# hzxie/GaussianCity

Hardware: AMD Instinct MI355X
Metric: rendered frames/sec (fwd) @ 5000000 Gaussians, 1920x1080 (higher is better)
Workload: dtype f32; 1 GPU; C3: s_city 5000000 Gaussians, 1920x1080, SH degree 3, forward, 24-pose orbit; exp=gcr-fp32-v2 (bit-exact vs oracle), tile_sort=lists beyond 1024 entries sorted lazily, as far as the blend walks (default), cull=stateless: every frame reads means, scales, rotations (default)

## Files before the change

### gaussiancity_amd/csrc/gcr_api.hip

```cpp
#include <atomic>
#include <chrono>
#include <condition_variable>
#include <cstdio>
#include <cstring>
#include <deque>
#include <map>
#include <mutex>
#include <string>
#include <thread>

#include <pthread.h>

#include "gcr_internal.h"
#define GC_ERR_HIP GCR_ERR_DEVICE
#include "gc_host.h"

namespace {

std::atomic<int> g_timing{0};
std::atomic<int> g_force_radix{0};
std::atomic<int> g_force_global_cursor{0};
std::atomic<int> g_lazy_sort{1};
std::atomic<int> g_sort_in_blend{0};
std::atomic<int> g_split_preprocess{0};
std::atomic<int> g_deterministic{0};
std::atomic<int> g_bwd_wave_units{0};
std::atomic<int> g_rescue_hold{0};
std::atomic<int> g_gate_polls{400000};
std::atomic<int> g_band_sort_min{GCR_BAND_SORT_MIN_DEFAULT};
std::atomic<int> g_bwd_piece{160};
std::atomic<int> g_stream_policy{-1};
std::atomic<int> g_sync_culls{0};
struct SyncCullGuard {
  const int others;
  SyncCullGuard() : others(g_sync_culls.fetch_add(1)) {}
  ~SyncCullGuard() { g_sync_culls.fetch_sub(1); }
  SyncCullGuard(const SyncCullGuard&) = delete;
  SyncCullGuard& operator=(const SyncCullGuard&) = delete;
};
#ifdef GCR_EXPERIMENTS
std::atomic<int> g_k7_skip_flush{0};
std::atomic<int> g_k6_debug{0};
std::atomic<unsigned long long*> g_clock_buf{nullptr};
#endif

struct Opts {
  int lazy_sort, sort_in_blend, bwd_piece, deterministic, split_preprocess, force_radix, force_global_cursor, bwd_wave_units;
  int band_sort_min;
  int stream_policy;
};

int opt_raw(int v) { return v; }
int opt_bool(int v) { return v != 0; }
int opt_piece(int v) { return v < GCR_PIECE_MIN ? GCR_PIECE_MIN : (v > GCR_PIECE_MAX ? GCR_PIECE_MAX : v); }
struct OptionRow {
  const char* name;
  std::atomic<int>* global;
  int (*normalize)(int);
  int Opts::*resolved;
  int32_t gcr_options::*per_call;
};
const OptionRow g_options[] = {
    {"timing", &g_timing, opt_raw, nullptr, nullptr},
    {"force_radix", &g_force_radix, opt_raw, &Opts::force_radix, &gcr_options::force_radix},
    {"force_global_cursor", &g_force_global_cursor, opt_raw, &Opts::force_global_cursor, &gcr_options::force_global_cursor},
    {"split_preprocess", &g_split_preprocess, opt_raw, &Opts::split_preprocess, &gcr_options::split_preprocess},
    {"sort_in_blend", &g_sort_in_blend, opt_raw, &Opts::sort_in_blend, &gcr_options::sort_in_blend},
    {"lazy_sort", &g_lazy_sort, opt_bool, &Opts::lazy_sort, &gcr_options::lazy_sort},
    {"deterministic_backward", &g_deterministic, opt_bool, &Opts::deterministic, &gcr_options::deterministic_backward},
    {"bwd_wave_units", &g_bwd_wave_units, opt_bool, &Opts::bwd_wave_units, &gcr_options::bwd_wave_units},
    {"bwd_piece", &g_bwd_piece, opt_piece, &Opts::bwd_piece, &gcr_options::bwd_piece},
    {"band_sort_min", &g_band_sort_min, [](int v) { return v < 0 ? -1 : v; }, &Opts::band_sort_min, nullptr},
    {"stream_policy", &g_stream_policy, [](int v) { return v < 0 ? -1 : (v != 0); }, &Opts::stream_policy, nullptr},
    {"rescue_hold", &g_rescue_hold, opt_bool, nullptr, nullptr},
    {"gate_polls", &g_gate_polls, [](int v) { return v < 1 ? 1 : v; }, nullptr, nullptr},
#ifdef GCR_EXPERIMENTS
    {"k7_skip_flush", &g_k7_skip_flush, opt_raw, nullptr, nullptr},
    {"k6_debug", &g_k6_debug, opt_raw, nullptr, nullptr},
#endif
};
const OptionRow* find_option(const char* name) {
  if (name)
    for (const OptionRow& o : g_options)
      if (!strcmp(name, o.name)) return &o;
  return nullptr;
}
Opts resolve_options(const gcr_options* o) {
  Opts r{};
  for (const OptionRow& row : g_options) {
    if (!row.resolved) continue;
    int v = row.global->load();
    if (o != nullptr && row.per_call != nullptr && o->*row.per_call >= 0)
      v = row.normalize == opt_piece ? opt_piece(o->*row.per_call) : opt_bool(o->*row.per_call);
    r.*row.resolved = v;
  }
  return r;
}

enum Stage { ST_PRE = 0, ST_SCAN, ST_EMIT, ST_SORT, ST_RANGES, ST_BLEND_FWD, ST_BLEND_BWD, ST_PRE_BWD, ST_COUNT };

int check_num_rendered(unsigned long long R) {
  if (R == GCR_PREFILTER_MARK)
    return fail(GCR_ERR_INVALID_ARGUMENT, "Point is filtered although prefiltered is set. This shouldn't happen!");
  if (R > 0x7fffffffull)
    return fail(GCR_ERR_OVERFLOW, "num_rendered exceeds 2^31-1 (32-bit instance index, as in the reference)");
  return 0;
}

inline size_t align_up(size_t v, size_t a = 256) { return (v + a - 1) / a * a; }

inline void gcr_cpu_relax() {
#if defined(__x86_64__) || defined(__i386__)
  __builtin_ia32_pause();
#elif defined(__aarch64__)
  __asm__ __volatile__("yield");
#endif
}

constexpr int64_t GCR_SORT_IN_BLEND_MAX = 384;

thread_local StageSlot g_slots[ST_COUNT];
StageSlot* stage_slot(int stage) { return g_timing.load() ? &g_slots[stage] : nullptr; }

int debug_sync(const gcr_camera* cam, hipStream_t s, const char* where) {
  if (cam->debug) {
    hipError_t e = hipStreamSynchronize(s);
    if (e != hipSuccess) return fail_hip(e, where);
  }
  return 0;
}

gcr_layout compute_layout(int32_t P, int32_t W, int32_t H, int64_t R) {
  gcr_layout L;
  const size_t p = (size_t)(P > 0 ? P : 0);
  const size_t nblk = (p + 255) / 256;
  size_t o = 0;
  L.geom_rec = o;            o = align_up(o + p * sizeof(float4) * GCR_REC_QUADS);
  L.geom_cov3D = o;          o = align_up(o + p * GCR_COV3D_FLOATS * sizeof(float));
  L.geom_clamped = o;        o = align_up(o + p);
  L.geom_tiles_touched = o;  o = align_up(o + p * sizeof(uint32_t));
  L.geom_block_sums = o;     o = align_up(o + (nblk + 1) * sizeof(uint32_t));
  L.geom_vis_list = o;       o = align_up(o + p * sizeof(uint32_t));
  L.geom_vis_count = o;      o = align_up(o + (nblk + 1) * sizeof(uint32_t));
  L.geom_num_rendered = o;   o = align_up(o + 16 * sizeof(uint64_t));
  L.geom_block_tiles = o;    o = align_up(o + GCR_K1_MAX_BLOCKS * sizeof(uint64_t));
  L.geom_vis_rec = o;        o = align_up(o + p * sizeof(uint4));
  L.geom_total = o;

  const size_t npix = (size_t)(W > 0 ? W : 0) * (size_t)(H > 0 ? H : 0);
  const size_t gx = (size_t)(W + GCR_BLOCK_X - 1) / GCR_BLOCK_X, gy = (size_t)(H + GCR_BLOCK_Y - 1) / GCR_BLOCK_Y;
  const size_t T = gx * gy;
  o = 0;
  L.img_final_T = o;    o = align_up(o + npix * sizeof(float));
  L.img_n_contrib = o;  o = align_up(o + npix * sizeof(uint32_t));
  L.img_ranges = o;       o = align_up(o + T * 2 * sizeof(uint32_t));
  L.img_tile_cursor = o;  o = align_up(o + T * GCR_CURSOR_STRIDE * sizeof(uint32_t));
  {
    int G = 1;
    const int ng = gcr_tile_table_groups((int)T, GCR_K1_MAX_BLOCKS, &G);
    L.img_tile_table = o;   o = align_up(o + (size_t)ng * T * sizeof(uint32_t));
  }
  L.img_tile_lazy = o;    o = align_up(o + T * 4 * sizeof(uint32_t));
  L.img_total = o;

  const size_t r = (size_t)(R > 0 ? R : 0);
  const int end_bit = 32 + (int)gcr_higher_msb((uint32_t)T);
  L.bin_sorted = (size_t)(gcr_sort_passes(end_bit) & 1);
  o = 0;
  L.bin_vals[L.bin_sorted] = o;      o = align_up(o + r * sizeof(uint32_t));
  L.bin_vals[1 - L.bin_sorted] = o;  o = align_up(o + r * sizeof(uint32_t));
  L.bin_keys[0] = o;  o = align_up(o + r * sizeof(uint64_t));
  L.bin_keys[1] = o;  o = align_up(o + r * sizeof(uint64_t));
  L.bin_hist = o;     o = align_up(o + gcr_sort_hist_bytes((int64_t)r, end_bit));
  const size_t slots = r ? (size_t)gcr_piece_slots(r, T, GCR_PIECE_MIN) : 0;
  L.bin_lean_total = o;
  L.bin_work = o;       o = align_up(o + slots * 16);
  L.bin_mask = o;       o = align_up(o + r * sizeof(uint16_t));
  L.bin_ckpt = o;       o = align_up(o + slots * (size_t)GCR_CKPT_BYTES);
  L.bin_staged = o;     o = align_up(o + r * 48);
  L.bin_total = o;
  return L;
}

int check_inputs(const gcr_camera* cam, const gcr_gaussians* g, bool need_opacity = true) {
  if (!cam || !g) return fail(GCR_ERR_INVALID_ARGUMENT, "null camera/gaussians record");
  if (g->P < 0) return fail(GCR_ERR_INVALID_ARGUMENT, "P must be >= 0");
  if (g->P > 700000000)
    return fail(GCR_ERR_INVALID_ARGUMENT, "P above 700 000 000 is not supported");
  if (cam->img_w <= 0 || cam->img_h <= 0) return fail(GCR_ERR_INVALID_ARGUMENT, "image size must be positive");
  if (cam->img_w > 16 * 65535 || cam->img_h > 16 * 65535)
    return fail(GCR_ERR_INVALID_ARGUMENT, "image too large for 16-bit tile coordinates");
  if (!cam->bg || !cam->view_matrix || !cam->proj_matrix || !cam->campos)
    return fail(GCR_ERR_INVALID_ARGUMENT, "bg/view_matrix/proj_matrix/campos must be non-null");
  if (cam->out_u8 != 0 && cam->backward == 1)
    return fail(GCR_ERR_INVALID_ARGUMENT, "out_u8 (uint8 video frames) is for inference frames: gcr_camera.backward must be 0");
  if (cam->win_w != 0 || cam->win_h != 0) {
    if (cam->win_w <= 0 || cam->win_h <= 0 || cam->win_x < 0 || cam->win_y < 0 || cam->win_x + cam->win_w > cam->img_w ||
        cam->win_y + cam->win_h > cam->img_h)
      return fail(GCR_ERR_INVALID_ARGUMENT, "the output window must lie inside the image");
  }
  if (g->P == 0) return 0;
  if (!g->means3D) return fail(GCR_ERR_INVALID_ARGUMENT, "means3D must have dimensions (num_points, 3)");
  if (need_opacity && !g->opacities) return fail(GCR_ERR_INVALID_ARGUMENT, "opacities must be non-null");
  if ((g->shs == nullptr) == (g->colors_precomp == nullptr))
    return fail(GCR_ERR_INVALID_ARGUMENT, "provide exactly one of SHs or precomputed colors");
  const bool has_sr = g->scales != nullptr && g->rotations != nullptr;
  if (has_sr == (g->cov3D_precomp != nullptr) || ((g->scales != nullptr) != (g->rotations != nullptr)))
    return fail(GCR_ERR_INVALID_ARGUMENT,
                "provide exactly one of scale/rotation pair or precomputed 3D covariance");
  if (g->cull_cache && ((uintptr_t)g->cull_cache & 127u))
    return fail(GCR_ERR_INVALID_ARGUMENT, "cull_cache must be 128-byte aligned (gcr_cull_cache_bytes(P) bytes filled by gcr_build_cull_cache)");
  if (g->shs) {
    if (cam->sh_degree < 0 || cam->sh_degree > 3) return fail(GCR_ERR_INVALID_ARGUMENT, "sh_degree must be 0..3");
    if (g->M < (cam->sh_degree + 1) * (cam->sh_degree + 1))
      return fail(GCR_ERR_INVALID_ARGUMENT, "sh has fewer coefficients than sh_degree needs");
  }
  return 0;
}

void fill_cam(GcrCamVals& c, const gcr_camera* cam) {
  memset(&c, 0, sizeof(c));
  if (!cam->host_camera) return;
  c.by_value = 1;
  memcpy(c.view, cam->view_matrix, sizeof(c.view));
  memcpy(c.proj, cam->proj_matrix, sizeof(c.proj));
  memcpy(c.campos, cam->campos, sizeof(c.campos));
  memcpy(c.bg, cam->bg, sizeof(c.bg));
}
inline int stride_or(int32_t s, int dense) { return s > 0 ? (int)s : dense; }

struct FrameSetup {
  gcr_layout L;
  int64_t R_layout;
  int gx, gy, T;
  int nblocks, chunk;
  int NG, G;
  float4* rec;
  float* cov3D;
  uint32_t *tiles_touched, *block_sums, *vis_list, *vis_count;
  uint4 *vis_rec, *banded;
  unsigned long long *frame, *block_tiles;
  float* final_T;
  uint32_t *n_contrib, *ranges, *cursor, *table;
  uint4* lazy;
  char* bin;
  uint64_t* keys[2];
  uint32_t *vals[2], *list, *hist;
};
template <class T>
T* at(const void* base, size_t off) {
  return base ? (T*)((char*)base + off) : nullptr;
}
FrameSetup frame_setup(const Opts& op, int32_t P, const gcr_camera* cam, int64_t R_layout, const void* geom,
                       const void* img, const void* binning) {
  FrameSetup f;
  f.L = compute_layout(P, cam->img_w, cam->img_h, R_layout);
  const gcr_layout& L = f.L;
  f.R_layout = R_layout;
  f.gx = (cam->img_w + GCR_BLOCK_X - 1) / GCR_BLOCK_X;
  f.gy = (cam->img_h + GCR_BLOCK_Y - 1) / GCR_BLOCK_Y;
  f.T = f.gx * f.gy;
  gcr_preprocess_grid(P, gcr_preprocess_resident_blocks(), &f.nblocks, &f.chunk);
  f.G = 1;
  f.NG = op.force_global_cursor ? 0 : gcr_tile_table_groups(f.T, f.nblocks, &f.G);
  f.rec = at<float4>(geom, L.geom_rec);
  f.cov3D = at<float>(geom, L.geom_cov3D);
  f.tiles_touched = at<uint32_t>(geom, L.geom_tiles_touched);
  f.block_sums = at<uint32_t>(geom, L.geom_block_sums);
  f.vis_list = at<uint32_t>(geom, L.geom_vis_list);
  f.vis_count = at<uint32_t>(geom, L.geom_vis_count);
  f.vis_rec = at<uint4>(geom, L.geom_vis_rec);
  f.frame = at<unsigned long long>(geom, L.geom_num_rendered);
  f.block_tiles = at<unsigned long long>(geom, L.geom_block_tiles);
  f.banded = gcr_band_sort_possible(f.T) ? at<uint4>(geom, L.geom_tiles_touched) : nullptr;
  f.final_T = at<float>(img, L.img_final_T);
  f.n_contrib = at<uint32_t>(img, L.img_n_contrib);
  f.ranges = at<uint32_t>(img, L.img_ranges);
  f.cursor = at<uint32_t>(img, L.img_tile_cursor);
  f.table = at<uint32_t>(img, L.img_tile_table);
  f.lazy = at<uint4>(img, L.img_tile_lazy);
  f.bin = at<char>(binning, 0);
  for (int k = 0; k < 2; k++) {
    f.keys[k] = at<uint64_t>(binning, L.bin_keys[k]);
    f.vals[k] = at<uint32_t>(binning, L.bin_vals[k]);
  }
  f.list = f.vals[L.bin_sorted];
  f.hist = at<uint32_t>(binning, L.bin_hist);
  return f;
}

int check_buffers(const FrameSetup& f, const gcr_camera* cam, size_t geom_bytes, size_t img_bytes, const void* binning,
                  size_t binning_bytes, const char* binning_msg) {
  if (geom_bytes < f.L.geom_total) return fail(GCR_ERR_BUFFER_TOO_SMALL, "geometry buffer too small");
  if (img_bytes < f.L.img_total) return fail(GCR_ERR_BUFFER_TOO_SMALL, "image buffer too small");
  if (f.R_layout > 0 && (!binning || binning_bytes < (cam->backward == 1 ? f.L.bin_total : f.L.bin_lean_total)))
    return fail(GCR_ERR_BUFFER_TOO_SMALL, binning_msg);
  return 0;
}

template <class A>
void set_gaussian_args(A& a, const gcr_gaussians* g) {
  a.P = g->P;
  a.means3D = g->means3D; a.scales = g->scales; a.rotations = g->rotations;
  a.s_mean = stride_or(g->stride_means3D, 3);
  a.s_scale = stride_or(g->stride_scales, 3);
  a.s_rot = stride_or(g->stride_rotations, 4);
}
template <class A>
void set_camera_args(A& a, const gcr_camera* cam, const gcr_gaussians* g) {
  set_gaussian_args(a, g);
  a.D = cam->sh_degree; a.M = g->M; a.W = cam->img_w; a.H = cam->img_h;
  a.tanfovx = cam->tanfovx; a.tanfovy = cam->tanfovy;
  a.focal_y = cam->img_h / (2.0f * cam->tanfovy);
  a.focal_x = cam->img_w / (2.0f * cam->tanfovx);
  a.scale_modifier = cam->scale_modifier;
  a.shs = g->shs;
  a.view = cam->view_matrix; a.proj = cam->proj_matrix; a.campos = cam->campos;
  fill_cam(a.cam, cam);
}

GcrBlendArgs blend_args(const FrameSetup& f, const gcr_camera* cam, const uint32_t* list) {
  GcrBlendArgs b;
  memset(&b, 0, sizeof(b));
  b.ranges = f.ranges;
  b.list = list;
  b.rec = f.rec;
  b.W = cam->img_w; b.H = cam->img_h; b.gx = f.gx; b.gy = f.gy;
  b.bg = cam->bg;
  b.flip_x = cam->flip_x != 0; b.flip_y = cam->flip_y != 0;
  b.win_x = cam->win_x; b.win_y = cam->win_y; b.win_w = cam->win_w; b.win_h = cam->win_h;
  b.out_u8 = cam->out_u8 != 0 && cam->backward != 1;
  b.image_only = cam->backward == GCR_BACKWARD_IMAGE_ONLY;
  fill_cam(b.cam, cam);
  b.final_T = f.final_T;
  b.n_contrib = f.n_contrib;
  return b;
}

}

extern "C" {

#ifdef GCR_EXPERIMENTS
void gcr_debug_set_clock_buffer(void* dev_ptr) { g_clock_buf.store((unsigned long long*)dev_ptr); }
#endif

int gcr_abi_version(void) { return GCR_ABI_VERSION; }
int gcr_grad_record_floats(void) { return g_deterministic.load() ? GCR_GRAD_REC_FLOATS_DET : GCR_GRAD_REC_FLOATS; }
int gcr_grad_record_floats_opt(const gcr_options* options) {
  return resolve_options(options).deterministic ? GCR_GRAD_REC_FLOATS_DET : GCR_GRAD_REC_FLOATS;
}
const char* gcr_last_error(void) { return g_err.c_str(); }

size_t gcr_geometry_bytes(int32_t P) { return compute_layout(P, 16, 16, 0).geom_total; }
size_t gcr_image_bytes(int32_t W, int32_t H) { return compute_layout(0, W, H, 0).img_total; }
size_t gcr_binning_bytes(int64_t R, int32_t W, int32_t H) { return compute_layout(0, W, H, R).bin_total; }
size_t gcr_binning_bytes_lean(int64_t R, int32_t W, int32_t H) { return compute_layout(0, W, H, R).bin_lean_total; }
int gcr_get_layout(int32_t P, int32_t W, int32_t H, int64_t R, gcr_layout* out) {
  if (!out) return fail(GCR_ERR_INVALID_ARGUMENT, "null layout");
  *out = compute_layout(P, W, H, R);
  return 0;
}

int gcr_set_option(const char* name, int value) {
  const OptionRow* o = find_option(name);
  return o ? o->global->exchange(o->normalize(value)) : -1;
}

int gcr_get_option(const char* name) {
  const OptionRow* o = find_option(name);
  return o ? o->global->load() : INT32_MIN;
}

int gcr_get_stage_ms(float* ms_out, int capacity) { return stage_report(g_slots, ST_COUNT, ms_out, capacity); }

static inline bool band_sort_slot_free(const Opts& op) {
  return !op.split_preprocess && !op.force_radix && !op.force_global_cursor;
}

static int enqueue_preprocess(const Opts& op, const gcr_camera* cam, const gcr_gaussians* g, const FrameSetup& f,
                              int32_t* radii, unsigned long long cap_instances, unsigned long long cap_list, hipStream_t s,
                              unsigned long long* host_R = nullptr, unsigned int seq = 0, bool nt_stream = false) {
  GcrPreprocessArgs a;
  set_camera_args(a, cam, g);
  a.gx = f.gx; a.gy = f.gy;
  a.opacities = g->opacities; a.cov3D_precomp = g->cov3D_precomp; a.colors_precomp = g->colors_precomp;
  a.s_opac = stride_or(g->stride_opacities, 1);
  a.s_col = stride_or(g->stride_colors, 3);
  a.prefiltered = cam->prefiltered != 0;
  a.cull_cache = op.split_preprocess ? nullptr : reinterpret_cast<const float4*>(g->cull_cache);
  a.cull_shape = a.cull_cache ? reinterpret_cast<const float4*>((const char*)g->cull_cache + gcr_cull_cache_offset_b(g->P)) : nullptr;
  a.nt_stream = nt_stream ? 1 : 0;
  a.radii = radii;
  a.rec = f.rec;
  a.cov3D = f.cov3D;
  a.tile_count = f.cursor;
  a.vis_list = f.vis_list;
  a.vis_count = f.vis_count;
  a.vis_rec = f.vis_rec;
  a.cand_list = f.tiles_touched;
  a.cand_count = f.block_sums;
  a.nblocks = f.nblocks; a.chunk = f.chunk;
  a.block_tiles = f.block_tiles;
  const int T = f.T;
  if (f.NG > 0) a.tile_count = nullptr;
  {
    StageTimer t(s, stage_slot(ST_PRE));
    if (f.NG == 0)
      HIP_TRY(hipMemsetAsync(a.tile_count, 0, sizeof(uint32_t) * GCR_CURSOR_STRIDE * (size_t)T, s), "tile count memset");
    HIP_TRY(gcr_launch_preprocess(a, op.split_preprocess != 0, s), "preprocess");
  }
  if (int rc = debug_sync(cam, s, "preprocess")) return rc;
  StageTimer t(s, stage_slot(ST_SCAN));
  if (f.NG > 0) {
    const bool band = f.banded && band_sort_slot_free(op) && op.band_sort_min >= 0 &&
                      (op.band_sort_min == 0 || (cap_instances != ~0ull && cap_instances >= (unsigned long long)op.band_sort_min));
    HIP_TRY(gcr_launch_tile_count(T, f.gx, f.NG, f.G, f.nblocks, f.chunk, f.vis_rec, f.vis_count, f.table, f.cursor,
                                  f.cursor + (size_t)T, f.cursor + 2 * (size_t)T, f.frame, f.block_tiles, host_R, seq,
                                  band ? f.banded : nullptr, g->P / 4, s),
            "tile count");
  } else {
    HIP_TRY(gcr_launch_scan_tiles(f.cursor, GCR_CURSOR_STRIDE, f.ranges, T, f.frame, cap_instances, cap_list, host_R, seq,
                                  f.block_tiles, f.nblocks, s),
            "tile scan");
  }
  return 0;
}

static void set_piece_args(const Opts& op, GcrBlendArgs& b, bool want_state, const FrameSetup& f) {
  const gcr_layout& L = f.L;
  char* bb = want_state && f.R_layout > 0 ? f.bin : nullptr;
  b.piece = want_state ? op.bwd_piece : GCR_PIECE_MAX;
#ifdef GCR_EXPERIMENTS
  if (!want_state)
    if (const char* e = getenv("GCR_INFER_PIECE")) b.piece = atoi(e) < GCR_PIECE_MIN ? GCR_PIECE_MIN : (atoi(e) > GCR_PIECE_MAX ? GCR_PIECE_MAX : atoi(e));
#endif
  b.ckpt = bb ? (float4*)(bb + L.bin_ckpt) : nullptr;
  b.work = bb ? (uint4*)(bb + L.bin_work) : nullptr;
  b.mask_out = bb ? (uint16_t*)(bb + L.bin_mask) : nullptr;
  b.staged_out = bb ? (float4*)(bb + L.bin_staged) : nullptr;
  b.staged_off = L.bin_staged;
  b.ckpt_off = L.bin_ckpt;
  b.work_off = L.bin_work;
  b.mask_off = L.bin_mask;
  b.carve_bytes = L.bin_total;
  b.frame_out = f.frame;
#ifdef GCR_EXPERIMENTS
  if (const char* e = getenv("GCR_K6_NOEXTRAS")) {
    if (strchr(e, 'w')) { b.ckpt = nullptr; b.work = nullptr; }
    if (strchr(e, 'm')) { b.mask_out = nullptr; b.staged_out = nullptr; }
  }
#endif
}

static int enqueue_render_lds(const Opts& op, const gcr_camera* cam, const gcr_gaussians* g, const FrameSetup& f,
                              int64_t list_length_hint, bool speculative, unsigned long long cap_instances,
                              unsigned long long cap_list, float* out_color, hipStream_t s,
                              unsigned long long* host_longest = nullptr, unsigned long long* gate_words = nullptr,
                              unsigned int gate_seq = 0, bool nt_out = false) {
  const int64_t R_layout = f.R_layout;
  uint64_t* pairs = f.keys[0];
  const unsigned long long* frame_guard = speculative ? f.frame : nullptr;
  {
    StageTimer t(s, stage_slot(ST_EMIT));
    if (f.NG > 0) {
      HIP_TRY(gcr_launch_tile_scatter(f.T, f.gx, f.NG, f.G, f.nblocks, f.chunk, f.vis_rec, f.vis_count, f.table, f.cursor,
                                      f.cursor + (size_t)f.T, f.cursor + 2 * (size_t)f.T, f.ranges, pairs, f.frame,
                                      cap_instances, cap_list, host_longest, f.banded, g->P / 4, s),
              "tile scatter");
    } else if (R_layout > 0) {
      HIP_TRY(gcr_launch_scatter_instances(f.nblocks, f.chunk, f.vis_list, f.vis_count, f.rec, f.gx, f.cursor, pairs,
                                           f.ranges, f.T, frame_guard, s),
              "scatter instances");
    }
  }
  if (int rc = debug_sync(cam, s, "scatter instances")) return rc;
  const bool sort_in_blend = R_layout > 0 && list_length_hint <= GCR_SORT_IN_BLEND_MAX && op.sort_in_blend != 0;
  uint4* lazy = (R_layout > 0 && !sort_in_blend && op.lazy_sort != 0) ? f.lazy : nullptr;
  if (R_layout > 0 && !sort_in_blend) {
    StageTimer t(s, stage_slot(ST_SORT));
    HIP_TRY(gcr_launch_tile_sort(f.ranges, f.T, pairs, f.keys[1], f.list, list_length_hint + list_length_hint / 2 + 64,
                                 frame_guard, lazy, s),
            "tile sort");
  }
  if (int rc = debug_sync(cam, s, "tile sort")) return rc;
  GcrBlendArgs b = blend_args(f, cam, f.list);
  b.nt_out = nt_out && cam->backward != 1;
  b.out_color = out_color;
  b.frame = frame_guard;
  b.pairs = pairs;
  b.list_out = f.list;
  b.lazy = lazy;
  set_piece_args(op, b, cam->backward == 1, f);
  b.gate_words = gate_words;
  b.gate_seq = gate_seq;
  b.gate_polls = (unsigned int)g_gate_polls.load();
#ifdef GCR_EXPERIMENTS
  b.debug_flags = g_k6_debug.load();
  b.clock_buf = g_clock_buf.load();
#endif
#ifdef GCR_EXPERIMENTS
  static const bool chain = getenv("GCR_CHAIN_BLEND") != nullptr && atoi(getenv("GCR_CHAIN_BLEND")) != 0;
  static std::mutex chain_mu;
  static hipEvent_t chain_ev[64] = {};
  static unsigned chain_n = 0;
  if (chain) {
    std::lock_guard<std::mutex> lk(chain_mu);
    if (chain_n > 0) (void)hipStreamWaitEvent(s, chain_ev[(chain_n - 1) % 64], 0);
  }
#endif
  {
    StageTimer t(s, stage_slot(ST_BLEND_FWD));
    HIP_TRY(gcr_launch_blend_fwd(b, sort_in_blend, s), "blend forward");
  }
#ifdef GCR_EXPERIMENTS
  if (chain) {
    std::lock_guard<std::mutex> lk(chain_mu);
    hipEvent_t& e = chain_ev[chain_n % 64];
    if (!e) (void)hipEventCreateWithFlags(&e, hipEventDisableTiming);
    (void)hipEventRecord(e, s);
    chain_n++;
  }
#endif
  return debug_sync(cam, s, "blend forward");
}

static unsigned long long* host_words_alloc(size_t n) {
  unsigned long long* p = nullptr;
  if (n == 0 || hipHostMalloc((void**)&p, n * sizeof(unsigned long long),
                              hipHostMallocCoherent | hipHostMallocMapped | hipHostMallocPortable) != hipSuccess)
    return nullptr;
  for (size_t i = 0; i < n; i++) p[i] = 0ull;
  return p;
}
struct FrameReadback {
  unsigned long long* pinned = nullptr;
  unsigned int seq = 0;
  int ensure() {
    if (!pinned) {
      pinned = host_words_alloc(8);
      if (!pinned) return fail(GCR_ERR_DEVICE, "hipHostMalloc for the frame read-back failed");
    }
    return 0;
  }
};
thread_local FrameReadback g_readback;

static std::mutex g_words_mu;
static std::map<unsigned long long*, size_t> g_words_blocks;
static void rescue_forget_words(const unsigned long long* base, size_t n);

unsigned long long* gcr_host_words_alloc(size_t n_words) {
  unsigned long long* p = host_words_alloc(n_words);
  if (p) {
    std::lock_guard<std::mutex> lk(g_words_mu);
    g_words_blocks[p] = n_words;
  }
  return p;
}
void gcr_host_words_free(unsigned long long* words) {
  if (!words) return;
  size_t n = 0;
  {
    std::lock_guard<std::mutex> lk(g_words_mu);
    auto it = g_words_blocks.find(words);
    if (it != g_words_blocks.end()) {
      n = it->second;
      g_words_blocks.erase(it);
    }
  }
  if (n) rescue_forget_words(words, n);
  (void)hipHostFree(words);
}

int gcr_forward_preprocess(const gcr_camera* cam, const gcr_gaussians* g, void* geom,
                           size_t geom_bytes, void* img, size_t img_bytes, int32_t* radii,
                           gcr_frame_info* info_host, void* hip_stream) {
  if (int rc = check_inputs(cam, g)) return rc;
  if (!info_host) return fail(GCR_ERR_INVALID_ARGUMENT, "info_host is null");
  info_host->num_rendered = 0;
  info_host->max_tile_instances = 0;
  if (g->P == 0) return 0;
  if (!geom || !radii || !img) return fail(GCR_ERR_INVALID_ARGUMENT, "geom/img/radii must be non-null");
  const Opts op = resolve_options(cam->options);
  const FrameSetup f = frame_setup(op, g->P, cam, 0, geom, img, nullptr);
  if (int rc = check_buffers(f, cam, geom_bytes, img_bytes, nullptr, 0, nullptr)) return rc;
  hipStream_t s = (hipStream_t)hip_stream;
  const SyncCullGuard sync_cull;
  const bool nt = op.stream_policy > 0 || (op.stream_policy < 0 && sync_cull.others == 0);
  if (int rc = enqueue_preprocess(op, cam, g, f, radii, ~0ull, ~0ull, s, nullptr, 0, nt)) return rc;
  unsigned long long r[2] = {0, 0};
  HIP_TRY(hipMemcpyAsync(r, f.frame, sizeof(r), hipMemcpyDeviceToHost, s), "num_rendered copy");
  HIP_TRY(hipStreamSynchronize(s), "num_rendered sync");
  if (int rc = check_num_rendered(r[0])) return rc;
  info_host->num_rendered = (int64_t)r[0];
  info_host->max_tile_instances = (int64_t)r[1];
  return 0;
}

int gcr_forward(const gcr_camera* cam, const gcr_gaussians* g, void* geom, size_t geom_bytes, void* binning,
                size_t binning_bytes, int64_t binning_capacity, int64_t tile_list_capacity, void* img,
                size_t img_bytes, int32_t* radii, float* out_color, gcr_frame_info* info_host, void* hip_stream) {
  if (int rc = check_inputs(cam, g)) return rc;
  if (!info_host) return fail(GCR_ERR_INVALID_ARGUMENT, "info_host is null");
  info_host->num_rendered = 0;
  info_host->max_tile_instances = 0;
  if (g->P == 0) return 0;
  if (!out_color) return fail(GCR_ERR_INVALID_ARGUMENT, "out_color is null");
  if (binning_capacity < 0 || binning_capacity > 0x7fffffffll)
    return fail(GCR_ERR_INVALID_ARGUMENT, "binning_capacity out of range");
  if (!geom || !radii || !img) return fail(GCR_ERR_INVALID_ARGUMENT, "geom/img/radii must be non-null");
  const Opts op = resolve_options(cam->options);
  const FrameSetup f = frame_setup(op, g->P, cam, binning_capacity, geom, img, binning);
  if (int rc = check_buffers(f, cam, geom_bytes, img_bytes, binning, binning_bytes,
                               "binning buffer smaller than gcr_binning_bytes(binning_capacity)"))
    return rc;
  if (int rc = g_readback.ensure()) return rc;
  hipStream_t s = (hipStream_t)hip_stream;
  const bool speculate = binning_capacity > 0 && !op.force_radix && !cam->debug;
  const int64_t list_hint = tile_list_capacity > 0 ? tile_list_capacity : (int64_t)gcr_tile_sort_capacity();
  FrameReadback& rb = g_readback;
  const unsigned int seq = ++rb.seq ? rb.seq : ++rb.seq;
  const SyncCullGuard sync_cull;
  const bool nt = op.stream_policy > 0 || (op.stream_policy < 0 && sync_cull.others == 0);
  if (int rc = enqueue_preprocess(op, cam, g, f, radii, speculate ? (unsigned long long)binning_capacity : 0ull, ~0ull, s,
                                  rb.pinned, seq, nt))
    return rc;
  if (speculate) {
    if (int rc = enqueue_render_lds(op, cam, g, f, list_hint, true, (unsigned long long)binning_capacity, ~0ull, out_color,
                                    s, rb.pinned + 1, nullptr, 0, nt))
      return rc;
  }
  volatile unsigned long long* word = rb.pinned;
  unsigned long long v = *word;
  for (unsigned long spins = 0; (unsigned int)(v >> 32) != seq; v = *word) {
    gcr_cpu_relax();
    if ((++spins & 0xffffu) == 0) {
      const hipError_t q = hipStreamQuery(s);
      if (q != hipSuccess && q != hipErrorNotReady) return fail_hip(q, "frame info wait");
      if (q == hipSuccess && (unsigned int)(*word >> 32) != seq)
        return fail(GCR_ERR_DEVICE, "the stream finished without publishing num_rendered");
    }
  }
  const unsigned long long R = v & 0xffffffffull;
  const bool go = R <= (unsigned long long)binning_capacity;
  if (int rc = check_num_rendered(R)) return rc;
  info_host->num_rendered = (int64_t)R;
  if (speculate && go) {
    const unsigned long long seen = ((volatile unsigned long long*)rb.pinned)[1];
    info_host->max_tile_instances = seen ? (int64_t)seen : tile_list_capacity;
    return 0;
  }
  unsigned long long mx = 0;
  HIP_TRY(hipMemcpyAsync(&mx, f.frame + 1, sizeof(mx), hipMemcpyDeviceToHost, s), "longest list copy");
  HIP_TRY(hipStreamSynchronize(s), "longest list sync");
  info_host->max_tile_instances = (int64_t)mx;
  return 1;
}

struct AsyncFrame {
  unsigned long long* words;
  unsigned int seq;
  int device;
  gcr_camera cam;
  gcr_options opt;
  bool has_opt;
  float camvals[38];
  gcr_gaussians g;
  void* geom;
  size_t geom_bytes;
  void* img;
  size_t img_bytes;
  float* out_color;
  int64_t capacity;
  std::chrono::steady_clock::time_point born;
};

class RescueService {
  std::mutex mu_;
  std::condition_variable cv_;
  std::deque<AsyncFrame> frames_;
  bool started_ = false;
  hipStream_t streams_[64] = {};
  void* scratch_[64] = {};
  size_t scratch_bytes_[64] = {};
  std::atomic<long> rescued_{0};
  std::atomic<long> dropped_{0};
  const unsigned long long* rescuing_ = nullptr;
  std::condition_variable idle_cv_;

  static void publish(unsigned long long* w, int idx, unsigned int seq) {
    std::atomic_thread_fence(std::memory_order_seq_cst);
    ((volatile unsigned long long*)w)[idx] = (unsigned long long)seq;
    std::atomic_thread_fence(std::memory_order_seq_cst);
  }

  void rescue(AsyncFrame& f) {
    volatile unsigned long long* w = f.words;
    publish(f.words, 7, f.seq);
    if ((unsigned int)w[4] == f.seq) {
      publish(f.words, 5, f.seq);
      publish(f.words, 2, f.seq);
      dropped_.fetch_add(1);
      return;
    }
    const unsigned long long R = w[0] & 0xffffffffull;
    bool ok = false;
    void* stale = nullptr;
    do {
      if (check_num_rendered(R)) break;
      if (hipSetDevice(f.device) != hipSuccess) break;
      const int d = f.device & 63;
      if (!streams_[d]) {
        int lo = 0, hi = 0;
        if (hipDeviceGetStreamPriorityRange(&lo, &hi) != hipSuccess) lo = hi = 0;
        if (hipStreamCreateWithPriority(&streams_[d], hipStreamNonBlocking, hi) != hipSuccess &&
            hipStreamCreateWithFlags(&streams_[d], hipStreamNonBlocking) != hipSuccess)
          break;
      }
      hipStream_t s = streams_[d];
      gcr_camera cam = f.cam;
      if (cam.backward == 1) cam.backward = 0;
      cam.options = f.has_opt ? &f.opt : nullptr;
      if (cam.host_camera) {
        cam.view_matrix = f.camvals;
        cam.proj_matrix = f.camvals + 16;
        cam.campos = f.camvals + 32;
        cam.bg = f.camvals + 35;
      }
      const FrameSetup fs = frame_setup(resolve_options(cam.options), f.g.P, &cam, 0, f.geom, f.img, nullptr);
      gcr_frame_info info;
      info.num_rendered = (int64_t)R;
      unsigned long long longest = 0;
      if (hipMemcpyAsync(&longest, fs.frame + 1, 8, hipMemcpyDeviceToHost, s) != hipSuccess) break;
      if (hipStreamSynchronize(s) != hipSuccess) break;
      info.max_tile_instances = (int64_t)longest;
      const size_t bytes = gcr_binning_bytes_lean((int64_t)R, cam.img_w, cam.img_h);
      if (scratch_bytes_[d] < bytes) {
        stale = scratch_[d];
        scratch_[d] = nullptr;
        scratch_bytes_[d] = 0;
        if (hipMalloc(&scratch_[d], bytes + bytes / 2) != hipSuccess) {
          scratch_[d] = nullptr;
          break;
        }
        scratch_bytes_[d] = bytes + bytes / 2;
      }
      if (gcr_forward_render(&cam, &f.g, f.geom, f.geom_bytes, scratch_[d], scratch_bytes_[d], f.img, f.img_bytes, &info,
                             f.out_color, s) < 0)
        break;
      if (hipStreamSynchronize(s) != hipSuccess) break;
      ok = true;
    } while (false);
    if (!ok) publish(f.words, 5, f.seq);
    publish(f.words, 6, f.seq);
    publish(f.words, 2, f.seq);
    rescued_.fetch_add(1);
    if (stale) (void)hipFree(stale);
  }

  void run() {
    for (;;) {
      std::unique_lock<std::mutex> lk(mu_);
      cv_.wait(lk, [&] { return !frames_.empty(); });
      const auto now = std::chrono::steady_clock::now();
      const bool hold = g_rescue_hold.load() != 0;
      for (auto it = frames_.begin(); it != frames_.end();) {
        volatile unsigned long long* w = it->words;
        const unsigned long long v = w[0];
        if ((unsigned int)(v >> 32) == it->seq) {
          if ((v & 0xffffffffull) <= (unsigned long long)it->capacity) {
            it = frames_.erase(it);
            continue;
          }
          if ((unsigned int)w[4] == it->seq) {
            dropped_.fetch_add(1);
            it = frames_.erase(it);
            continue;
          }
          if (!hold && (unsigned int)w[3] == it->seq) {
            AsyncFrame f = *it;
            frames_.erase(it);
            rescuing_ = f.words;
            lk.unlock();
            rescue(f);
            lk.lock();
            rescuing_ = nullptr;
            idle_cv_.notify_all();
            break;
          }
        }
        if (now - it->born > std::chrono::seconds(120)) {
          it = frames_.erase(it);
          continue;
        }
        ++it;
      }
      lk.unlock();
      std::this_thread::sleep_for(std::chrono::microseconds(100));
    }
  }

 public:
  void add(const AsyncFrame& f) {
    std::lock_guard<std::mutex> lk(mu_);
    for (auto it = frames_.begin(); it != frames_.end();) it = it->words == f.words ? frames_.erase(it) : it + 1;
    const bool was_empty = frames_.empty();
    frames_.push_back(f);
    if (!started_) {
      started_ = true;
      std::thread([this] { run(); }).detach();
    }
    if (was_empty) cv_.notify_one();
  }
  void forget(const unsigned long long* base, size_t n) {
    std::unique_lock<std::mutex> lk(mu_);
    for (auto it = frames_.begin(); it != frames_.end();) it = (it->words >= base && it->words < base + n) ? frames_.erase(it) : it + 1;
    idle_cv_.wait(lk, [&] { return !(rescuing_ != nullptr && rescuing_ >= base && rescuing_ < base + n); });
  }
  void remove(const unsigned long long* words, unsigned int seq) {
    std::lock_guard<std::mutex> lk(mu_);
    for (auto it = frames_.begin(); it != frames_.end();) it = (it->words == words && it->seq == seq) ? frames_.erase(it) : it + 1;
  }
  long rescued() const { return rescued_.load(); }
  long dropped() const { return dropped_.load(); }
  void reset_after_fork() {
    new (&mu_) std::mutex();
    new (&cv_) std::condition_variable();
    new (&idle_cv_) std::condition_variable();
    rescuing_ = nullptr;
    new (&frames_) std::deque<AsyncFrame>();
    started_ = false;
    for (int i = 0; i < 64; i++) {
      streams_[i] = nullptr;
      scratch_[i] = nullptr;
      scratch_bytes_[i] = 0;
    }
  }
};
static RescueService& rescue_service() {
  static RescueService* r = [] {
    RescueService* p = new RescueService();
    (void)pthread_atfork(nullptr, nullptr, [] { rescue_service().reset_after_fork(); });
    return p;
  }();
  return *r;
}

static void rescue_forget_words(const unsigned long long* base, size_t n) { rescue_service().forget(base, n); }

long gcr_rescue_count(void) { return rescue_service().rescued(); }
long gcr_rescue_dropped_count(void) { return rescue_service().dropped(); }

int gcr_forward_async(const gcr_camera* cam, const gcr_gaussians* g, void* geom, size_t geom_bytes, void* binning,
                      size_t binning_bytes, int64_t binning_capacity, int64_t tile_list_capacity, void* img,
                      size_t img_bytes, int32_t* radii, float* out_color, unsigned long long* words_host, uint32_t seq,
                      void* hip_stream) {
  if (int rc = check_inputs(cam, g)) return rc;
  if (!words_host || seq == 0u) return fail(GCR_ERR_INVALID_ARGUMENT, "words_host must be non-null and seq non-zero");
  if (g->P == 0) {
    ((volatile unsigned long long*)words_host)[1] = 0ull;
    ((volatile unsigned long long*)words_host)[0] = (unsigned long long)seq << 32;
    return 0;
  }
  if (!out_color) return fail(GCR_ERR_INVALID_ARGUMENT, "out_color is null");
  const Opts op = resolve_options(cam->options);
  if (binning_capacity <= 0 || binning_capacity > 0x7fffffffll || op.force_radix || cam->debug)
    return fail(GCR_ERR_INVALID_ARGUMENT,
                "gcr_forward_async needs a capacity guess > 0 and neither force_radix nor debug: use gcr_forward");
  if (!geom || !radii || !img) return fail(GCR_ERR_INVALID_ARGUMENT, "geom/img/radii must be non-null");
  const FrameSetup fr = frame_setup(op, g->P, cam, binning_capacity, geom, img, binning);
  if (int rc = check_buffers(fr, cam, geom_bytes, img_bytes, binning, binning_bytes,
                               "binning buffer smaller than gcr_binning_bytes(binning_capacity)"))
    return rc;
  hipStream_t s = (hipStream_t)hip_stream;
  const int64_t list_hint = tile_list_capacity > 0 ? tile_list_capacity : (int64_t)gcr_tile_sort_capacity();
  if (int rc = enqueue_preprocess(op, cam, g, fr, radii, (unsigned long long)binning_capacity, ~0ull, s, words_host, seq,
                                  op.stream_policy > 0))
    return rc;
  AsyncFrame f;
  memset((void*)&f, 0, sizeof(f));
  f.words = words_host;
  f.seq = seq;
  if (hipGetDevice(&f.device) != hipSuccess) f.device = 0;
  f.cam = *cam;
  f.has_opt = cam->options != nullptr;
  if (f.has_opt) f.opt = *cam->options;
  f.cam.options = nullptr;
  if (cam->host_camera) {
    memcpy(f.camvals, cam->view_matrix, 16 * sizeof(float));
    memcpy(f.camvals + 16, cam->proj_matrix, 16 * sizeof(float));
    memcpy(f.camvals + 32, cam->campos, 3 * sizeof(float));
    memcpy(f.camvals + 35, cam->bg, 3 * sizeof(float));
  }
  f.g = *g;
  f.geom = geom;
  f.geom_bytes = geom_bytes;
  f.img = img;
  f.img_bytes = img_bytes;
  f.out_color = out_color;
  f.capacity = binning_capacity;
  f.born = std::chrono::steady_clock::now();
  rescue_service().add(f);
  const int rc = enqueue_render_lds(op, cam, g, fr, list_hint, true, (unsigned long long)binning_capacity, ~0ull, out_color, s,
                                    words_host + 1, words_host, seq, op.stream_policy > 0);
  if (rc < 0) rescue_service().remove(words_host, seq);
  return rc;
}

static int ticket_state(const unsigned long long* words_host, uint32_t seq, int64_t capacity, gcr_frame_info* info) {
  volatile const unsigned long long* w = words_host;
  const unsigned long long v = w[0];
  if ((unsigned int)(v >> 32) != seq) return 1;
  const unsigned long long R = v & 0xffffffffull;
  if (int rc = check_num_rendered(R)) return rc;
  if (R > (unsigned long long)capacity) {
    if ((unsigned int)w[5] == seq) return fail(GCR_ERR_DEVICE, "the overflow rescue of an asynchronous frame failed");
    if ((unsigned int)w[2] != seq) {
      if ((unsigned int)w[4] == seq && (unsigned int)w[7] != seq)
        return fail(GCR_ERR_DEVICE, "an asynchronous frame overflowed its binning buffer and was not rescued in time");
      return 1;
    }
  }
  if (info) {
    info->num_rendered = (int64_t)R;
    info->max_tile_instances = (int64_t)w[1];
  }
  return 0;
}

int gcr_ticket_poll(const unsigned long long* words_host, uint32_t seq, int64_t binning_capacity,
                    gcr_frame_info* info_host) {
  if (!words_host || seq == 0u) return fail(GCR_ERR_INVALID_ARGUMENT, "words_host must be non-null and seq non-zero");
  return ticket_state(words_host, seq, binning_capacity, info_host);
}

int gcr_ticket_wait(const unsigned long long* words_host, uint32_t seq, int64_t binning_capacity, void* hip_stream,
                    gcr_frame_info* info_host) {
  if (!words_host || seq == 0u) return fail(GCR_ERR_INVALID_ARGUMENT, "words_host must be non-null and seq non-zero");
  hipStream_t s = (hipStream_t)hip_stream;
  for (unsigned long spins = 0;; ) {
    const int st = ticket_state(words_host, seq, binning_capacity, info_host);
    if (st != 1) return st;
    gcr_cpu_relax();
    if ((++spins & 0xfffffu) == 0 && hip_stream != nullptr) {
      const hipError_t q = hipStreamQuery(s);
      if (q != hipSuccess && q != hipErrorNotReady) return fail_hip(q, "ticket wait");
      if (q == hipSuccess && ticket_state(words_host, seq, binning_capacity, info_host) == 1)
        return fail(GCR_ERR_DEVICE, "the stream finished without publishing num_rendered");
    }
  }
}

int gcr_forward_render(const gcr_camera* cam, const gcr_gaussians* g, void* geom, size_t geom_bytes,
                       void* binning, size_t binning_bytes, void* img, size_t img_bytes,
                       const gcr_frame_info* info, float* out_color, void* hip_stream) {
  if (int rc = check_inputs(cam, g, false)) return rc;
  if (g->P == 0) return 0;
  if (!geom || !img || !info) return fail(GCR_ERR_INVALID_ARGUMENT, "geom/img/info must be non-null");
  if (!out_color && cam->backward != 1)
    return fail(GCR_ERR_INVALID_ARGUMENT, "out_color may only be NULL for a state-only pass (gcr_camera.backward == 1)");
  const int64_t R = info->num_rendered;
  if (R < 0 || R > 0x7fffffffll) return fail(GCR_ERR_INVALID_ARGUMENT, "R out of range");
  if (R > 0 && !binning) return fail(GCR_ERR_INVALID_ARGUMENT, "binning buffer is null");
  const Opts op = resolve_options(cam->options);
  const FrameSetup f = frame_setup(op, g->P, cam, R, geom, img, binning);
  if (int rc = check_buffers(f, cam, geom_bytes, img_bytes, binning, binning_bytes, "binning buffer too small")) return rc;
  hipStream_t s = (hipStream_t)hip_stream;
  if (R == 0 || !op.force_radix)
    return enqueue_render_lds(op, cam, g, f, info->max_tile_instances, false, ~0ull, ~0ull, out_color, s, nullptr, nullptr, 0,
                              op.stream_policy > 0);

  int half = (int)f.L.bin_sorted;
  {
    StageTimer t(s, stage_slot(ST_EMIT));
    HIP_TRY(gcr_launch_tiles_touched(g->P, f.nblocks, f.chunk, f.vis_list, f.vis_count, f.rec, f.tiles_touched, f.block_sums, s),
            "tiles touched");
    HIP_TRY(gcr_launch_scan_block_sums(f.block_sums, (g->P + 255) / 256, (unsigned long long*)f.hist, s), "scan");
    HIP_TRY(gcr_launch_emit(g->P, f.tiles_touched, f.block_sums, f.rec, f.gx, f.keys[0], f.vals[0], s), "emit");
  }
  if (int rc = debug_sync(cam, s, "emit")) return rc;
  {
    StageTimer t(s, stage_slot(ST_SORT));
    const int end_bit = 32 + (int)gcr_higher_msb((uint32_t)f.T);
    HIP_TRY(gcr_launch_sort(f.keys[0], f.vals[0], f.keys[1], f.vals[1], R, end_bit, f.hist, &half, s), "sort");
  }
  if (int rc = debug_sync(cam, s, "sort")) return rc;
  {
    StageTimer t(s, stage_slot(ST_RANGES));
    HIP_TRY(gcr_launch_tile_ranges(f.keys[half], R, f.ranges, f.T, s), "tile ranges");
  }
  if (int rc = debug_sync(cam, s, "tile ranges")) return rc;
  GcrBlendArgs b = blend_args(f, cam, f.vals[half]);
  b.out_color = out_color;
  set_piece_args(op, b, cam->backward == 1, f);
  {
    StageTimer t(s, stage_slot(ST_BLEND_FWD));
    HIP_TRY(gcr_launch_blend_fwd(b, false, s), "blend forward");
  }
  return debug_sync(cam, s, "blend forward");
}

int gcr_backward(const gcr_camera* cam, const gcr_gaussians* g, const int32_t* radii, const void* geom,
                 size_t geom_bytes, const void* binning, size_t binning_bytes, const void* img,
                 size_t img_bytes, int64_t R, const float* dL_dpix, const gcr_grads* gr,
                 void* hip_stream) {
  if (int rc = check_inputs(cam, g, false)) return rc;
  if (g->P == 0) return 0;
  if (!gr || !dL_dpix || !radii || !geom || !img)
    return fail(GCR_ERR_INVALID_ARGUMENT, "grads/dL_dpix/radii/geom/img must be non-null");
  if (!gr->dL_dmeans2D || !gr->dL_dconic || !gr->dL_dopacity || !gr->dL_dcolors || !gr->dL_dmeans3D ||
      !gr->dL_dcov3D || (g->shs && !gr->dL_dsh) || (g->scales && (!gr->dL_dscales || !gr->dL_drotations)))
    return fail(GCR_ERR_INVALID_ARGUMENT, "a required gradient output is null");
  if ((uintptr_t)gr->dL_dconic & 63u)
    return fail(GCR_ERR_INVALID_ARGUMENT, "dL_dconic (the gradient records) must be 64-byte aligned");
  if (g->scales && stride_or(gr->stride_rotations, 4) == 4 && ((uintptr_t)gr->dL_drotations & 15u))
    return fail(GCR_ERR_INVALID_ARGUMENT, "dL_drotations must be 16-byte aligned");
  if (g->rotations && stride_or(g->stride_rotations, 4) == 4 && ((uintptr_t)g->rotations & 15u))
    return fail(GCR_ERR_INVALID_ARGUMENT, "rotations must be 16-byte aligned when dense");
  const bool any_grad_stride = gr->stride_means3D > 0 || gr->stride_opacity > 0 || gr->stride_colors > 0 ||
                               gr->stride_scales > 0 || gr->stride_rotations > 0;
  if (any_grad_stride && (!gr->packed || gr->packed_floats <= 0))
    return fail(GCR_ERR_INVALID_ARGUMENT, "strided gradient outputs need the block they live in (gcr_grads.packed)");
  if (R < 0 || R > 0x7fffffffll) return fail(GCR_ERR_INVALID_ARGUMENT, "R out of range");
  if (cam->backward != 1)
    return fail(GCR_ERR_INVALID_ARGUMENT,
                "gcr_backward needs a frame rendered with gcr_camera.backward == 1 (pass the same value here); for a frame "
                "rendered without it call gcr_forward_render(out_color = NULL, backward = 1) first");
  const Opts op = resolve_options(cam->options);
  const FrameSetup f = frame_setup(op, g->P, cam, R, geom, img, binning);
  if (int rc = check_buffers(f, cam, geom_bytes, img_bytes, binning, binning_bytes, "binning buffer too small")) return rc;
  hipStream_t s = (hipStream_t)hip_stream;

  const int det = op.deterministic;

  GcrFillArgs fill;
  memset(&fill, 0, sizeof(fill));
  {
    const unsigned long long P = (unsigned long long)g->P;
    auto seg = [&](float* p, unsigned long long n) {
      if (p != nullptr && n != 0) {
        fill.ptr[fill.nseg] = p;
        fill.n[fill.nseg++] = n;
      }
    };
    seg(gr->dL_dmeans2D, 3 * P);
    seg(gr->stride_colors > 0 ? nullptr : gr->dL_dcolors, (unsigned long long)GCR_NUM_CHANNELS * P);
    seg(gr->stride_opacity > 0 ? nullptr : gr->dL_dopacity, P);
    seg(gr->stride_means3D > 0 ? nullptr : gr->dL_dmeans3D, 3 * P);
    seg(gr->dL_dcov3D, 6 * P);
    seg(gr->dL_dsh, g->shs ? 3ull * (unsigned long long)g->M * P : 0ull);
    seg(gr->stride_scales > 0 ? nullptr : gr->dL_dscales, 3 * P);
    seg(gr->stride_rotations > 0 ? nullptr : gr->dL_drotations, 4 * P);
    if (any_grad_stride) seg(gr->packed, (unsigned long long)gr->packed_floats);
    unsigned long long total = 0;
    for (int i = 0; i < fill.nseg; i++) total += fill.n[i];
    const unsigned long long want = (total + 1023ull) / 1024ull;
    unsigned long long cap = 256ull;
#ifdef GCR_EXPERIMENTS
    if (const char* e = getenv("GCR_FILL_BLOCKS")) cap = (unsigned long long)atoi(e);
#endif
    fill.blocks = (int)(want < cap ? (want ? want : 1ull) : cap);
  }

  if (R > 0) {
    StageTimer t(s, stage_slot(ST_BLEND_BWD));
    HIP_TRY(gcr_launch_zero_grad_records(f.nblocks, f.chunk, f.vis_list, f.vis_count, (float4*)gr->dL_dconic,
                                         (det ? GCR_GRAD_REC_FLOATS_DET : GCR_GRAD_REC_FLOATS) / 4, s),
            "zero gradient records");
    GcrBlendArgs b = blend_args(f, cam, f.list);
    b.fill = fill;
    b.dL_dpix = dL_dpix;
    b.grad_rec = gr->dL_dconic;
    b.deterministic = det;
    b.binning_base = f.bin;
    b.frame_in = f.frame;
    b.R = (unsigned long long)R;
    b.piece = op.bwd_piece;
    b.binning_bytes = (unsigned long long)binning_bytes;
#ifdef GCR_EXPERIMENTS
    b.debug_flags = g_k7_skip_flush.load();
    b.clock_buf = g_clock_buf.load();
#endif
    HIP_TRY(gcr_launch_blend_bwd(b, op.bwd_wave_units != 0, s), "blend backward");
  } else {
    HIP_TRY(gcr_launch_fill(fill, s), "gradient zero fill");
  }
  if (int rc = debug_sync(cam, s, "blend backward")) return rc;

  GcrPreprocessBwdArgs a;
  set_camera_args(a, cam, g);
  a.cov3D = g->cov3D_precomp ? g->cov3D_precomp : f.cov3D;
  a.s_cov3d = g->cov3D_precomp ? 6 : GCR_COV3D_FLOATS;
  a.radii = radii;
  a.vis_list = f.vis_list;
  a.vis_count = f.vis_count;
  a.nblocks = f.nblocks; a.chunk = f.chunk;
  a.frame = R > 0 ? f.frame : nullptr;
  a.binning_bytes = (unsigned long long)binning_bytes;
  a.grad_rec = (const float4*)gr->dL_dconic;
  a.rec = f.rec;
  a.deterministic = det;
  a.dL_dmean2D = gr->dL_dmeans2D; a.dL_dcolor = gr->dL_dcolors; a.dL_dopacity = gr->dL_dopacity;
  a.dL_dmean3D = gr->dL_dmeans3D; a.dL_dcov3D = gr->dL_dcov3D; a.dL_dsh = gr->dL_dsh;
  a.dL_dscale = gr->dL_dscales; a.dL_drot = gr->dL_drotations;
  a.g_mean = stride_or(gr->stride_means3D, 3);
  a.g_opac = stride_or(gr->stride_opacity, 1);
  a.g_col = stride_or(gr->stride_colors, 3);
  a.g_scale = stride_or(gr->stride_scales, 3);
  a.g_rot = stride_or(gr->stride_rotations, 4);
  {
    StageTimer t(s, stage_slot(ST_PRE_BWD));
    HIP_TRY(gcr_launch_preprocess_bwd(a, s), "preprocess backward");
  }
  return debug_sync(cam, s, "preprocess backward");
}

size_t gcr_cull_cache_bytes(int32_t P) { return P > 0 ? gcr_cull_cache_offset_b(P) + (size_t)P * 32 : 0; }

int gcr_build_cull_cache(const gcr_gaussians* g, float scale_modifier, void* cull_cache_out, void* hip_stream) {
  if (!g) return fail(GCR_ERR_INVALID_ARGUMENT, "null gaussians record");
  if (g->P < 0 || g->P > 700000000) return fail(GCR_ERR_INVALID_ARGUMENT, "P must be 0 .. 700 000 000");
  if (g->P == 0) return 0;
  if (!g->means3D) return fail(GCR_ERR_INVALID_ARGUMENT, "means3D must have dimensions (num_points, 3)");
  if (!g->opacities) return fail(GCR_ERR_INVALID_ARGUMENT, "opacities must be non-null");
  const bool has_sr = g->scales != nullptr && g->rotations != nullptr;
  if (has_sr == (g->cov3D_precomp != nullptr) || ((g->scales != nullptr) != (g->rotations != nullptr)))
    return fail(GCR_ERR_INVALID_ARGUMENT, "provide exactly one of scale/rotation pair or precomputed 3D covariance");
  if (!cull_cache_out || ((uintptr_t)cull_cache_out & 127u))
    return fail(GCR_ERR_INVALID_ARGUMENT, "cull_cache_out must be a 128-byte aligned buffer of gcr_cull_cache_bytes(P) bytes");
  GcrPreprocessArgs a;
  memset(&a, 0, sizeof(a));
  set_gaussian_args(a, g);
  a.scale_modifier = scale_modifier;
  a.cov3D_precomp = g->cov3D_precomp;
  a.opacities = g->opacities;
  a.s_opac = stride_or(g->stride_opacities, 1);
  HIP_TRY(gcr_launch_build_cull_cache(a, reinterpret_cast<float4*>(cull_cache_out),
                                      reinterpret_cast<float4*>((char*)cull_cache_out + gcr_cull_cache_offset_b(g->P)),
                                      (hipStream_t)hip_stream),
          "build cull cache");
  return 0;
}

int gcr_mark_visible(int32_t P, const float* means3D, const float* view_matrix,
                     const float* proj_matrix, uint8_t* present, void* hip_stream) {
  (void)proj_matrix;
  if (P < 0) return fail(GCR_ERR_INVALID_ARGUMENT, "P must be >= 0");
  if (P == 0) return 0;
  if (!means3D || !view_matrix || !present) return fail(GCR_ERR_INVALID_ARGUMENT, "null pointer");
  HIP_TRY(gcr_launch_mark_visible(P, means3D, view_matrix, present, (hipStream_t)hip_stream), "mark_visible");
  return 0;
}

int64_t gcr_rasterize_forward(gcr_resize_fn geometry_buffer, void* geometry_user,
                              gcr_resize_fn binning_buffer, void* binning_user,
                              gcr_resize_fn image_buffer, void* image_user, const gcr_camera* cam,
                              const gcr_gaussians* g, float* out_color, int32_t* radii,
                              void* hip_stream) {
  if (int rc = check_inputs(cam, g)) return rc;
  if (!geometry_buffer || !binning_buffer || !image_buffer)
    return fail(GCR_ERR_INVALID_ARGUMENT, "resize callbacks must be non-null");
  if (g->P == 0) return 0;
  const size_t gbytes = gcr_geometry_bytes(g->P);
  void* geom = geometry_buffer(geometry_user, gbytes);
  if (!geom) return fail(GCR_ERR_ALLOC, "geometry resize callback returned null");
  const size_t ibytes = gcr_image_bytes(cam->img_w, cam->img_h);
  void* img = image_buffer(image_user, ibytes);
  if (!img) return fail(GCR_ERR_ALLOC, "image resize callback returned null");
  gcr_camera cam1 = *cam;
  cam1.backward = 1;
  gcr_frame_info info;
  if (int rc = gcr_forward_preprocess(&cam1, g, geom, gbytes, img, ibytes, radii, &info, hip_stream)) return rc;
  const size_t bbytes = gcr_binning_bytes(info.num_rendered, cam->img_w, cam->img_h);
  void* bin = binning_buffer(binning_user, bbytes);
  if (!bin && info.num_rendered > 0) return fail(GCR_ERR_ALLOC, "binning resize callback returned null");
  if (int rc = gcr_forward_render(&cam1, g, geom, gbytes, bin, bbytes, img, ibytes, &info, out_color, hip_stream))
    return rc;
  return info.num_rendered;
}

}
```

### gaussiancity_amd/csrc/gcr_binning.hip

```cpp
#include <stdlib.h>
#include "gcr_device.h"
#include "gcr_internal.h"
#include "gcr_sort.h"

namespace {

constexpr int SORT_THREADS = 256;
constexpr int SORT_ITEMS = 16;
constexpr int SORT_TILE = SORT_THREADS * SORT_ITEMS;
constexpr int RADIX_BITS = 8;
constexpr int RADIX = 1 << RADIX_BITS;

__global__ __launch_bounds__(256) void k_emit(int P, const uint32_t* __restrict__ tiles_touched,
                                              const uint32_t* __restrict__ block_offsets,
                                              const float4* __restrict__ rec, int gx,
                                              uint64_t* __restrict__ keys,
                                              uint32_t* __restrict__ vals) {
  __shared__ uint32_t lds4[4];
  const int idx = blockIdx.x * 256 + threadIdx.x;
  const uint32_t t = idx < P ? tiles_touched[idx] : 0u;
  uint32_t total;
  uint32_t off = gcr_block_excl_scan_256(t, lds4, &total);
  if (t == 0) return;
  off += block_offsets[blockIdx.x];
  const float4 q2 = rec[(size_t)idx * GCR_REC_QUADS + 2];
  const uint32_t dbits = __float_as_uint(q2.y);
  const uint32_t rx = __float_as_uint(q2.z), ry = __float_as_uint(q2.w);
  const uint32_t minx = rx & 0xffffu, maxx = rx >> 16, miny = ry & 0xffffu, maxy = ry >> 16;
  for (uint32_t y = miny; y < maxy; y++)
    for (uint32_t x = minx; x < maxx; x++) {
      const uint64_t key = ((uint64_t)(y * (uint32_t)gx + x) << 32) | dbits;
      keys[off] = key;
      vals[off] = (uint32_t)idx;
      off++;
    }
}

constexpr int RANK_MERGE_MAX = 1024;
constexpr int TT_MAX_TBLOCKS = 640;

template <int THREADS>
struct TtPrefix {
  static constexpr int PER = (GCR_K1_MAX_BLOCKS + THREADS) / THREADS;
  uint32_t vc[PER];
  GCR_DEV void load(const uint32_t* __restrict__ vis_count, int nblocks, int tid) {
#pragma unroll
    for (int u = 0; u < PER; u++) {
      const int bi = tid * PER + u;
      vc[u] = bi < nblocks ? vis_count[bi] : 0u;
    }
  }
  GCR_DEV void scan(uint32_t* pre, uint32_t* wtot, int nblocks, int tid) const {
    const int lane = tid & 63, w = tid >> 6;
    uint32_t mine = 0;
#pragma unroll
    for (int u = 0; u < PER; u++) mine += vc[u];
    const uint32_t incl = gcr_wave_incl_scan_u32(mine, lane);
    __syncthreads();
    if (lane == 63) wtot[w] = incl;
    __syncthreads();
    uint32_t run = incl - mine;
#pragma unroll
    for (int k = 0; k < THREADS / 64; k++)
      if (k < w) run += wtot[k];
#pragma unroll
    for (int u = 0; u < PER; u++) {
      const int bi = tid * PER + u;
      if (bi <= nblocks) pre[bi] = run;
      run += vc[u];
    }
    __syncthreads();
  }
};
GCR_DEV uint32_t tt_position(const uint32_t* pre, int nblocks, int chunk, uint32_t f) {
  int lo = 0, hi = nblocks;
  while (hi - lo > 1) {
    const int mid = (lo + hi) >> 1;
    if (pre[mid] <= f)
      lo = mid;
    else
      hi = mid;
  }
  return (uint32_t)lo * (uint32_t)chunk + (f - pre[lo]);
}
GCR_DEV uint4 tt_survivor(const uint32_t* pre, int nblocks, const uint4* __restrict__ vis_rec, int chunk, uint32_t f) {
  return vis_rec[tt_position(pre, nblocks, chunk, f)];
}

template <bool SCATTER, int TT_THREADS>
__global__ __launch_bounds__(TT_THREADS) void k_tile_table(int T, int gx, int G, int nblocks_k1, int chunk,
                                                           const uint4* __restrict__ vis_rec,
                                                           const uint32_t* __restrict__ vis_count,
                                                           uint32_t* __restrict__ table,
                                                           const uint32_t* __restrict__ tile_total,
                                                           const uint32_t* __restrict__ tile_local,
                                                           const uint32_t* __restrict__ blk_total,
                                                           uint32_t* __restrict__ ranges,
                                                           uint64_t* __restrict__ pairs,
                                                           unsigned long long* __restrict__ frame,
                                                           unsigned long long cap_instances,
                                                           unsigned long long cap_list,
                                                           unsigned long long* __restrict__ host_word,
                                                           unsigned int seq,
                                                           const unsigned long long* __restrict__ block_tiles,
                                                           const uint4* __restrict__ banded, int banded_capacity) {
  extern __shared__ __attribute__((aligned(16))) unsigned char gcr_smem[];
  uint32_t* cnt = reinterpret_cast<uint32_t*>(gcr_smem);
  __shared__ uint32_t pre[GCR_K1_MAX_BLOCKS + 1];
  __shared__ uint32_t blk_base[TT_MAX_TBLOCKS];
  __shared__ uint32_t wtot[TT_THREADS / 64];
  const int tid = threadIdx.x, lane = tid & 63, w = tid >> 6;
#ifdef GCR_EXPERIMENTS
  const uint32_t my_row = G < 0 ? blockIdx.x : gcr_tt_row(blockIdx.x, gridDim.x);
#else
  const uint32_t my_row = gcr_tt_row(blockIdx.x, gridDim.x);
#endif
  uint32_t* __restrict__ row = table + (size_t)my_row * T;
  TtPrefix<TT_THREADS> blocks;
  blocks.load(vis_count, nblocks_k1, tid);
  if (!SCATTER) {
    if (blockIdx.x == 0) {
      unsigned long long part = 0ull, pf = 0ull;
      for (int b = tid; b < nblocks_k1; b += TT_THREADS) {
        const unsigned long long v = block_tiles[b];
        part += v & ~GCR_PREFILTER_FLAG;
        pf |= v & GCR_PREFILTER_FLAG;
      }
#pragma unroll
      for (int o = 32; o > 0; o >>= 1) part += __shfl_xor(part, o, 64);
      __shared__ unsigned long long wpart[TT_THREADS / 64];
      if (lane == 0) wpart[w] = part;
      const int prefilter_violation = __syncthreads_or(pf != 0ull ? 1 : 0);
      if (tid == 0) {
        unsigned long long total = 0ull;
#pragma unroll
        for (int k = 0; k < TT_THREADS / 64; k++) total += wpart[k];
        if (prefilter_violation) total = GCR_PREFILTER_MARK;
        frame[0] = total;
        frame[1] = 0ull;
        frame[2] = 0ull;
        frame[GCR_FRAME_PIECE] = 0ull;
        frame[GCR_FRAME_BANDED] = banded != nullptr ? 1ull : 0ull;
        if (host_word != nullptr)
          gcr_store_to_host(host_word, ((unsigned long long)seq << 32) | (total > 0xffffffffull ? 0xffffffffull : total));
      }
    }
    for (int t = tid; t < T; t += TT_THREADS) cnt[t] = 0u;
  } else {
    const bool go = frame[0] <= cap_instances && frame[1] <= cap_list;
    if (blockIdx.x == 0 && tid == 0) {
      frame[2] = go ? 1ull : 0ull;
      if (host_word != nullptr) gcr_store_to_host(host_word, frame[1]);
    }
    if (!go) return;
    const int ntb = (T + 63) / 64;
    uint32_t running = 0;
    for (int b0 = 0; b0 < ntb; b0 += TT_THREADS) {
      const int bi = b0 + tid;
      const uint32_t v = bi < ntb ? blk_total[bi] : 0u;
      const uint32_t incl = gcr_wave_incl_scan_u32(v, lane);
      if (lane == 63) wtot[w] = incl;
      __syncthreads();
      uint32_t before = 0, all = 0;
#pragma unroll
      for (int k = 0; k < TT_THREADS / 64; k++) {
        const uint32_t x = wtot[k];
        if (k < w) before += x;
        all += x;
      }
      if (bi < ntb) blk_base[bi] = running + before + incl - v;
      running += all;
      __syncthreads();
    }
    const int slice = (T + (int)gridDim.x - 1) / (int)gridDim.x;
    const int t_lo = blockIdx.x * slice, t_hi = min(T, t_lo + slice);
    for (int t = tid; t < T; t += TT_THREADS) {
      const uint32_t start = blk_base[t >> 6] + tile_local[t];
      cnt[t] = start + row[t];
      if (t >= t_lo && t < t_hi) {
        ranges[2 * t] = start;
        ranges[2 * t + 1] = start + tile_total[t];
      }
    }
  }
  (void)G;
  blocks.scan(pre, wtot, nblocks_k1, tid);
  const uint32_t survivors = pre[nblocks_k1];
  const uint32_t f_lo = (uint32_t)(((uint64_t)survivors * blockIdx.x) / gridDim.x);
  const uint32_t f_hi = (uint32_t)(((uint64_t)survivors * (blockIdx.x + 1u)) / gridDim.x);
  const bool use_band = banded != nullptr && (SCATTER ? frame[GCR_FRAME_BANDED] != 0ull : true);
  const bool band_recs = survivors <= (uint32_t)banded_capacity;
  const uint32_t* __restrict__ banded_pos = reinterpret_cast<const uint32_t*>(banded);
  for (uint32_t f = f_lo + (uint32_t)tid; f < f_hi; f += TT_THREADS) {
    const uint4 sv = !use_band ? tt_survivor(pre, nblocks_k1, vis_rec, chunk, f)
                               : (band_recs ? banded[f] : vis_rec[banded_pos[f]]);
    const uint32_t rx = sv.z, ry = sv.w;
    const uint32_t minx = rx & 0xffffu, maxx = rx >> 16, miny = ry & 0xffffu, maxy = ry >> 16;
    const uint64_t key = ((uint64_t)sv.y << 32) | sv.x;
    for (uint32_t y = miny; y < maxy; y++)
      for (uint32_t x = minx; x < maxx; x++) {
        const uint32_t t = y * (uint32_t)gx + x;
        if (SCATTER) {
          const uint32_t pos = atomicAdd(&cnt[t], 1u);
          pairs[pos] = key;
        } else {
          atomicAdd(&cnt[t], 1u);
        }
      }
  }
  if (!SCATTER) {
    __syncthreads();
    for (int t = tid; t < T; t += TT_THREADS) row[t] = cnt[t];
  }
}

constexpr int GCR_BANDS = 256;
constexpr int BAND_CUTS = 128;
GCR_DEV uint32_t band_of(uint32_t rx, uint32_t ry, uint32_t gx, uint32_t band_mul) {
  const uint32_t t0 = (ry & 0xffffu) * gx + (rx & 0xffffu);
  const uint32_t b = (uint32_t)(((uint64_t)t0 * band_mul) >> 32);
  return b < (uint32_t)GCR_BANDS ? b : (uint32_t)GCR_BANDS - 1u;
}

constexpr int BAND_THREADS = 1024;
constexpr int BAND_ILP = 4;
template <bool PERMUTE>
__global__ __launch_bounds__(BAND_THREADS) void k_band(int gx, uint32_t band_mul, int nblocks_k1, int chunk,
                                                       const uint4* __restrict__ vis_rec,
                                                       const uint32_t* __restrict__ vis_count,
                                                       uint32_t* __restrict__ hist, uint4* __restrict__ banded,
                                                       int banded_capacity) {
  __shared__ uint32_t pre[GCR_K1_MAX_BLOCKS + 1];
  __shared__ uint32_t wtot[BAND_THREADS / 64];
  __shared__ uint32_t cur[GCR_BANDS];
  __shared__ uint32_t part[2][BAND_THREADS / GCR_BANDS][GCR_BANDS];
  const int tid = threadIdx.x, lane = tid & 63, w = tid >> 6;
  TtPrefix<BAND_THREADS> blocks;
  blocks.load(vis_count, nblocks_k1, tid);
  if (PERMUTE) {
    constexpr int Q = BAND_THREADS / GCR_BANDS, ROWS = BAND_CUTS / Q;
    const int b = tid & (GCR_BANDS - 1), q = tid / GCR_BANDS;
    uint32_t total = 0, before = 0;
#pragma unroll 16
    for (int r = 0; r < ROWS; r++) {
      const int g = q * ROWS + r;
      const uint32_t v = hist[(size_t)g * GCR_BANDS + b];
      total += v;
      before += g < (int)blockIdx.x ? v : 0u;
    }
    part[0][q][b] = total;
    part[1][q][b] = before;
    __syncthreads();
    if (tid < GCR_BANDS) {
      total = 0;
      before = 0;
#pragma unroll
      for (int k = 0; k < Q; k++) {
        total += part[0][k][tid];
        before += part[1][k][tid];
      }
      const uint32_t incl = gcr_wave_incl_scan_u32(total, lane);
      if (lane == 63) wtot[w] = incl;
      part[0][0][tid] = incl - total + before;
    }
    __syncthreads();
    if (tid < GCR_BANDS) {
      uint32_t start = part[0][0][tid];
#pragma unroll
      for (int k = 0; k < GCR_BANDS / 64; k++)
        if (k < w) start += wtot[k];
      cur[tid] = start;
    }
  } else {
    if (tid < GCR_BANDS) cur[tid] = 0u;
  }
  blocks.scan(pre, wtot, nblocks_k1, tid);
  const uint32_t survivors = pre[nblocks_k1];
  const uint32_t f_lo = (uint32_t)(((uint64_t)survivors * blockIdx.x) / gridDim.x);
  const uint32_t f_hi = (uint32_t)(((uint64_t)survivors * (blockIdx.x + 1u)) / gridDim.x);
  const bool band_recs = survivors <= (uint32_t)banded_capacity;
  uint32_t* __restrict__ banded_pos = reinterpret_cast<uint32_t*>(banded);
  for (uint32_t f0 = f_lo + (uint32_t)tid; f0 < f_hi; f0 += BAND_THREADS * BAND_ILP) {
    uint32_t pos[BAND_ILP];
    uint4 sv[BAND_ILP];
#pragma unroll
    for (int u = 0; u < BAND_ILP; u++) {
      const uint32_t f = f0 + (uint32_t)u * BAND_THREADS;
      pos[u] = f < f_hi ? tt_position(pre, nblocks_k1, chunk, f) : 0xffffffffu;
    }
#pragma unroll
    for (int u = 0; u < BAND_ILP; u++)
      if (pos[u] != 0xffffffffu) sv[u] = vis_rec[pos[u]];
#pragma unroll
    for (int u = 0; u < BAND_ILP; u++)
      if (pos[u] != 0xffffffffu) {
        const uint32_t b = band_of(sv[u].z, sv[u].w, (uint32_t)gx, band_mul);
        if (PERMUTE) {
          const uint32_t slot = atomicAdd(&cur[b], 1u);
          if (band_recs)
            banded[slot] = sv[u];
          else
            banded_pos[slot] = pos[u];
        } else {
          atomicAdd(&cur[b], 1u);
        }
      }
  }
  if (!PERMUTE) {
    __syncthreads();
    if (tid < GCR_BANDS) hist[(size_t)blockIdx.x * GCR_BANDS + tid] = cur[tid];
  }
}

__global__ __launch_bounds__(1024) void k_table_colscan(uint32_t* __restrict__ table, int NG, int T,
                                                        uint32_t* __restrict__ tile_total,
                                                        uint32_t* __restrict__ tile_local,
                                                        uint32_t* __restrict__ blk_total,
                                                        unsigned long long* __restrict__ frame) {
  __shared__ uint32_t part[16][64];
  const int lane = threadIdx.x & 63, grp = threadIdx.x >> 6;
  const int t = blockIdx.x * 64 + lane;
  const int rpg = (NG + 15) / 16;
  const int r0 = grp * rpg;
  uint32_t v[32];
  uint32_t sum = 0;
#pragma unroll
  for (int r = 0; r < 32; r++) {
    const int g = r0 + r;
    v[r] = (r < rpg && g < NG && t < T) ? table[(size_t)g * T + t] : 0u;
  }
#pragma unroll
  for (int r = 0; r < 32; r++) sum += v[r];
  part[grp][lane] = sum;
  __syncthreads();
  uint32_t before = 0, all = 0;
#pragma unroll
  for (int k = 0; k < 16; k++) {
    const uint32_t p = part[k][lane];
    if (k < grp) before += p;
    all += p;
  }
  if (t < T) {
    uint32_t run = before;
#pragma unroll
    for (int r = 0; r < 32; r++) {
      const int g = r0 + r;
      if (r < rpg && g < NG) {
        table[(size_t)g * T + t] = run;
        run += v[r];
      }
    }
  }
  if (grp == 0) {
    const uint32_t mine = t < T ? all : 0u;
    const uint32_t incl = gcr_wave_incl_scan_u32(mine, lane);
    const uint32_t mx = gcr_wave_max_u32(mine);
    if (t < T) {
      tile_total[t] = mine;
      tile_local[t] = incl - mine;
    }
    if (lane == 63) {
      blk_total[blockIdx.x] = incl;
      if (mx) atomicMax(&frame[1], (unsigned long long)mx);
    }
  }
}

__global__ __launch_bounds__(256) void k_scatter_instances(int chunk, const uint32_t* __restrict__ vis_list,
                                                           const uint32_t* __restrict__ vis_count,
                                                           const float4* __restrict__ rec, int gx,
                                                           uint32_t* __restrict__ cursor,
                                                           uint64_t* __restrict__ pairs,
                                                           const unsigned long long* __restrict__ frame) {
  if (frame != nullptr && frame[2] == 0ull) return;
  const uint32_t nvis = vis_count[blockIdx.x];
  const uint32_t* __restrict__ my_list = vis_list + (size_t)blockIdx.x * chunk;
  for (uint32_t it = threadIdx.x; it < nvis; it += 256) {
    const int idx = (int)my_list[it];
    const float4 q2 = rec[(size_t)idx * GCR_REC_QUADS + 2];
    const uint64_t key = ((uint64_t)__float_as_uint(q2.y) << 32) | (uint32_t)idx;
    const uint32_t rx = __float_as_uint(q2.z), ry = __float_as_uint(q2.w);
    const uint32_t minx = rx & 0xffffu, maxx = rx >> 16, miny = ry & 0xffffu, maxy = ry >> 16;
    const uint32_t w = maxx - minx, n = w * (maxy - miny);
    for (uint32_t k0 = 0; k0 < n; k0 += 8) {
      uint32_t pos[8];
#pragma unroll
      for (uint32_t u = 0; u < 8; u++) {
        const uint32_t k = k0 + u;
        if (k < n) {
          const uint32_t t = (miny + k / w) * (uint32_t)gx + minx + k % w;
          pos[u] = atomicAdd(&cursor[(size_t)t * GCR_CURSOR_STRIDE], 1u);
        }
      }
#pragma unroll
      for (uint32_t u = 0; u < 8; u++)
        if (k0 + u < n) pairs[pos[u]] = key;
    }
  }
}

__global__ __launch_bounds__(256) void k_tile_sort(const uint32_t* __restrict__ ranges,
                                                   uint64_t* __restrict__ pairs, uint64_t* __restrict__ pairs_spare,
                                                   uint32_t* __restrict__ list,
                                                   const unsigned long long* __restrict__ frame, int lds_capacity,
                                                   uint4* __restrict__ lazy) {
  extern __shared__ __attribute__((aligned(16))) unsigned char gcr_smem[];
  uint64_t* s = reinterpret_cast<uint64_t*>(gcr_smem);
  if (frame != nullptr && frame[2] == 0ull) return;
  const int tid = threadIdx.x;
  const uint32_t r0 = ranges[2 * blockIdx.x], r1 = ranges[2 * blockIdx.x + 1];
  const int n = (int)(r1 - r0);
  if (lazy != nullptr) {
    if (n > GCR_LAZY_MIN) {
      uint32_t n_sorted = 0;
      uint64_t L = 0;
      gcr_lazy_extend<GCR_LAZY_CAP_K4>(s, pairs + r0, (uint32_t)n, n_sorted, L, list + r0, tid);
      if (tid == 0) lazy[blockIdx.x] = make_uint4(n_sorted, 0u, (uint32_t)L, (uint32_t)(L >> 32));
      return;
    }
    if (tid == 0) lazy[blockIdx.x] = make_uint4((uint32_t)max(n, 0), 0u, ~0u, ~0u);
  }
  if (n <= 0) return;
  if (n > lds_capacity) {
    gcr_tile_sort_long(s, (uint32_t)lds_capacity, pairs + r0, pairs_spare + r0, list + r0, (uint32_t)n, tid);
    return;
  }
  if (n == 1) {
    if (tid == 0) list[r0] = (uint32_t)pairs[r0];
    return;
  }
  if (n <= RANK_MERGE_MAX) {
    const int nchunks = (n + 63) >> 6, npad = nchunks << 6;
    uint64_t* sb = s + npad;
    for (int i = tid; i < npad; i += 256) s[i] = i < n ? pairs[r0 + i] : ~0ull;
    __syncthreads();
    const ulonglong2* s2 = reinterpret_cast<const ulonglong2*>(s);
    uint64_t mine[RANK_MERGE_MAX / 256];
    uint32_t rank[RANK_MERGE_MAX / 256];
#pragma unroll
    for (int e = 0; e < RANK_MERGE_MAX / 256; e++) {
      const int i = tid + e * 256;
      if (i < npad) {
        const int c = i >> 6;
        const uint64_t key = s[i];
        uint32_t r = 0;
#pragma unroll 8
        for (int j = 0; j < 32; j++) {
          const ulonglong2 kk = s2[c * 32 + j];
          r += (kk.x < key ? 1u : 0u) + (kk.y < key ? 1u : 0u);
        }
        mine[e] = key;
        rank[e] = r;
        if (i < n) sb[c * 64 + r] = key;
      }
    }
    __syncthreads();
    const int last_real = n - (nchunks - 1) * 64;
#pragma unroll
    for (int e = 0; e < RANK_MERGE_MAX / 256; e++) {
      const int i = tid + e * 256;
      if (i < n) {
        const int c = i >> 6;
        const uint64_t key = mine[e];
        uint32_t pos = rank[e];
        for (int c2 = 0; c2 < nchunks; c2++) {
          if (c2 == c) continue;
          const uint64_t* chunk = sb + c2 * 64;
          const int len = c2 == nchunks - 1 ? last_real : 64;
          int lo = 0, hi = len;
#pragma unroll
          for (int step = 0; step < 7; step++) {
            if (lo < hi) {
              const int mid = (lo + hi) >> 1;
              if (chunk[mid] < key)
                lo = mid + 1;
              else
                hi = mid;
            }
          }
          pos += (uint32_t)lo;
        }
        list[r0 + pos] = (uint32_t)key;
      }
    }
    return;
  }
  int N2 = 2;
  while (N2 < n) N2 <<= 1;
  for (int i = tid; i < N2; i += 256) s[i] = i < n ? pairs[r0 + i] : ~0ull;
  __syncthreads();
  gcr_bitonic_sort_lds(s, N2, tid);
  for (int i = tid; i < n; i += 256) list[r0 + i] = (uint32_t)s[i];
}


__global__ __launch_bounds__(SORT_THREADS) void k_radix_hist(const uint64_t* __restrict__ keys,
                                                             int64_t R, int shift, int nb,
                                                             uint32_t* __restrict__ table,
                                                             uint32_t* __restrict__ ghist) {
  __shared__ uint32_t h[RADIX];
  const int tid = threadIdx.x;
  h[tid] = 0;
  __syncthreads();
  const int64_t base = (int64_t)blockIdx.x * SORT_TILE;
#pragma unroll 4
  for (int i = 0; i < SORT_ITEMS; i++) {
    const int64_t idx = base + (int64_t)i * SORT_THREADS + tid;
    if (idx < R) atomicAdd(&h[(uint32_t)(keys[idx] >> shift) & (RADIX - 1)], 1u);
  }
  __syncthreads();
  const uint32_t c = h[tid];
  table[(size_t)tid * nb + blockIdx.x] = c;
  if (c) atomicAdd(&ghist[tid], c);
}

__global__ __launch_bounds__(256) void k_radix_scan(uint32_t* __restrict__ table, int nb) {
  __shared__ uint32_t lds4[4];
  uint32_t* row = table + (size_t)blockIdx.x * nb;
  uint32_t running = 0;
  for (int base = 0; base < nb; base += 256) {
    const int i = base + threadIdx.x;
    const uint32_t v = i < nb ? row[i] : 0u;
    uint32_t total;
    const uint32_t ex = gcr_block_excl_scan_256(v, lds4, &total);
    if (i < nb) row[i] = running + ex;
    running += total;
  }
}

__global__ __launch_bounds__(SORT_THREADS) void k_radix_scatter(
    const uint64_t* __restrict__ kin, const uint32_t* __restrict__ vin, uint64_t* __restrict__ kout,
    uint32_t* __restrict__ vout, int64_t R, int shift, int nb, const uint32_t* __restrict__ table,
    const uint32_t* __restrict__ ghist) {
  __shared__ uint32_t cnt[4][RADIX];
  __shared__ uint32_t dbase[RADIX];
  __shared__ uint32_t lds4[4];
  const int tid = threadIdx.x, lane = tid & 63, w = tid >> 6;
#pragma unroll
  for (int i = 0; i < 4; i++) cnt[i][tid] = 0;
  {
    uint32_t total;
    const uint32_t gb = gcr_block_excl_scan_256(ghist[tid], lds4, &total);
    dbase[tid] = gb + table[(size_t)tid * nb + blockIdx.x];
  }
  __syncthreads();

  const int64_t wbase = (int64_t)blockIdx.x * SORT_TILE + (int64_t)w * (64 * SORT_ITEMS);
  uint64_t key[SORT_ITEMS];
  uint32_t lrank[SORT_ITEMS];
  const uint64_t lt_mask = (1ull << lane) - 1ull;
#pragma unroll
  for (int i = 0; i < SORT_ITEMS; i++) {
    const int64_t idx = wbase + i * 64 + lane;
    const bool valid = idx < R;
    key[i] = valid ? kin[idx] : ~0ull;
    const uint32_t d = (uint32_t)(key[i] >> shift) & (RADIX - 1);
    uint64_t m = __ballot(valid);
#pragma unroll
    for (int b = 0; b < RADIX_BITS; b++) {
      const bool bit = (d >> b) & 1u;
      const uint64_t bb = __ballot(bit);
      m &= bit ? bb : ~bb;
    }
    const uint32_t rank_in = (uint32_t)__popcll(m & lt_mask);
    const uint32_t old = cnt[w][d];
    __builtin_amdgcn_wave_barrier();
    if (valid && rank_in == 0) cnt[w][d] = old + (uint32_t)__popcll(m);
    __builtin_amdgcn_wave_barrier();
    lrank[i] = old + rank_in;
  }
  __syncthreads();
  {
    uint32_t run = 0;
#pragma unroll
    for (int i = 0; i < 4; i++) {
      const uint32_t t = cnt[i][tid];
      cnt[i][tid] = run;
      run += t;
    }
  }
  __syncthreads();
#pragma unroll
  for (int i = 0; i < SORT_ITEMS; i++) {
    const int64_t idx = wbase + i * 64 + lane;
    if (idx < R) {
      const uint32_t d = (uint32_t)(key[i] >> shift) & (RADIX - 1);
      const uint32_t pos = dbase[d] + cnt[w][d] + lrank[i];
      kout[pos] = key[i];
      vout[pos] = vin[idx];
    }
  }
}

__global__ __launch_bounds__(256) void k_tile_ranges(const uint64_t* __restrict__ keys, int64_t R,
                                                     uint32_t* __restrict__ ranges) {
  const int64_t idx = (int64_t)blockIdx.x * 256 + threadIdx.x;
  if (idx >= R) return;
  const uint32_t currtile = (uint32_t)(keys[idx] >> 32);
  if (idx == 0)
    ranges[2 * currtile + 0] = 0;
  else {
    const uint32_t prevtile = (uint32_t)(keys[idx - 1] >> 32);
    if (currtile != prevtile) {
      ranges[2 * prevtile + 1] = (uint32_t)idx;
      ranges[2 * currtile + 0] = (uint32_t)idx;
    }
  }
  if (idx == R - 1) ranges[2 * currtile + 1] = (uint32_t)R;
}

__global__ __launch_bounds__(256) void k_ranges_make_contiguous(uint32_t* __restrict__ ranges, int T) {
  __shared__ uint32_t wmax[4];
  __shared__ uint32_t carry_s;
  const int tid = threadIdx.x, lane = tid & 63, w = tid >> 6;
  if (tid == 0) carry_s = 0u;
  __syncthreads();
  for (int t0 = 0; t0 < T; t0 += 256) {
    const int t = t0 + tid;
    const uint32_t r0 = t < T ? ranges[2 * t] : 0u, r1 = t < T ? ranges[2 * t + 1] : 0u;
    uint32_t v = r1;
#pragma unroll
    for (int o = 1; o < 64; o <<= 1) {
      const uint32_t u = __shfl_up(v, o, 64);
      if (lane >= o) v = u > v ? u : v;
    }
    if (lane == 63) wmax[w] = v;
    __syncthreads();
    uint32_t before = carry_s;
#pragma unroll
    for (int k = 0; k < 4; k++)
      if (k < w) before = wmax[k] > before ? wmax[k] : before;
    const uint32_t incl = v > before ? v : before;
    uint32_t prev = __shfl_up(incl, 1, 64);
    if (lane == 0) prev = before;
    if (t < T && r0 == r1) {
      ranges[2 * t] = prev;
      ranges[2 * t + 1] = prev;
    }
    __syncthreads();
    if (tid == 255) carry_s = incl;
    __syncthreads();
  }
}

}

hipError_t gcr_launch_emit(int P, const uint32_t* tiles_touched, const uint32_t* block_offsets,
                           const float4* rec, int gx, uint64_t* keys, uint32_t* vals,
                           hipStream_t s) {
  if (P <= 0) return hipSuccess;
  k_emit<<<(P + 255) / 256, 256, 0, s>>>(P, tiles_touched, block_offsets, rec, gx, keys, vals);
  return hipGetLastError();
}

bool gcr_band_sort_possible(int T) { return T >= GCR_BANDS; }

int gcr_tile_table_groups(int T, int nblocks_k1, int* G_out) {
  const size_t lds = (size_t)T * sizeof(uint32_t);
  if (lds > 148 * 1024 || (T + 63) / 64 > TT_MAX_TBLOCKS) return 0;
  int ng = 128;
#ifdef GCR_EXPERIMENTS
  if (const char* e = getenv("GCR_TT_GROUPS")) ng = atoi(e);
#endif
  if (ng > nblocks_k1) ng = nblocks_k1;
  if (ng < 1) ng = 1;
  int G = (nblocks_k1 + ng - 1) / ng;
  *G_out = G;
  return (nblocks_k1 + G - 1) / G;
}

static hipError_t tile_table_attr() {
  static hipError_t done = [] {
    const void* fns[4] = {(const void*)k_tile_table<false, 512>, (const void*)k_tile_table<true, 512>,
                          (const void*)k_tile_table<false, 1024>, (const void*)k_tile_table<true, 1024>};
    for (const void* f : fns) {
      const hipError_t e = hipFuncSetAttribute(f, hipFuncAttributeMaxDynamicSharedMemorySize, 148 * 1024);
      if (e != hipSuccess) return e;
    }
    return hipSuccess;
  }();
  return done;
}
static inline bool tile_table_wide(int) { return true; }
static inline int tile_table_G(int G) {
#ifdef GCR_EXPERIMENTS
  static const bool numeric = getenv("GCR_TT_ROWS_NUMERIC") != nullptr && atoi(getenv("GCR_TT_ROWS_NUMERIC")) != 0;
  if (numeric) return -1;
#endif
  return G;
}

hipError_t gcr_launch_tile_count(int T, int gx, int NG, int G, int nblocks_k1, int chunk, const uint4* vis_rec,
                                 const uint32_t* vis_count, uint32_t* table,
                                 uint32_t* tile_total, uint32_t* tile_local, uint32_t* blk_total,
                                 unsigned long long* frame, const unsigned long long* block_tiles,
                                 unsigned long long* host_R, unsigned int seq, uint4* banded, int banded_capacity,
                                 hipStream_t s) {
  hipError_t e = tile_table_attr();
  if (e != hipSuccess) return e;
  if (banded != nullptr) {
    const uint32_t band_mul = (uint32_t)((((uint64_t)GCR_BANDS << 32) + (uint64_t)T - 1) / (uint64_t)T);
    k_band<false><<<BAND_CUTS, BAND_THREADS, 0, s>>>(gx, band_mul, nblocks_k1, chunk, vis_rec, vis_count, table, nullptr,
                                                      banded_capacity);
    k_band<true><<<BAND_CUTS, BAND_THREADS, 0, s>>>(gx, band_mul, nblocks_k1, chunk, vis_rec, vis_count, table, banded,
                                                     banded_capacity);
  }
  if (tile_table_wide(T))
    k_tile_table<false, 1024><<<NG, 1024, (size_t)T * sizeof(uint32_t), s>>>(
        T, gx, tile_table_G(G), nblocks_k1, chunk, vis_rec, vis_count, table, nullptr, nullptr, nullptr, nullptr, nullptr,
        frame, 0ull, 0ull, host_R, seq, block_tiles, banded, banded_capacity);
  else
    k_tile_table<false, 512><<<NG, 512, (size_t)T * sizeof(uint32_t), s>>>(
        T, gx, tile_table_G(G), nblocks_k1, chunk, vis_rec, vis_count, table, nullptr, nullptr, nullptr, nullptr, nullptr,
        frame, 0ull, 0ull, host_R, seq, block_tiles, banded, banded_capacity);
  k_table_colscan<<<(T + 63) / 64, 1024, 0, s>>>(table, NG, T, tile_total, tile_local, blk_total, frame);
  return hipGetLastError();
}

hipError_t gcr_launch_tile_scatter(int T, int gx, int NG, int G, int nblocks_k1, int chunk, const uint4* vis_rec,
                                   const uint32_t* vis_count, uint32_t* table,
                                   const uint32_t* tile_total, const uint32_t* tile_local,
                                   const uint32_t* blk_total, uint32_t* ranges, uint64_t* pairs,
                                   unsigned long long* frame, unsigned long long cap_instances,
                                   unsigned long long cap_list, unsigned long long* host_longest,
                                   const uint4* banded, int banded_capacity, hipStream_t s) {
  hipError_t e = tile_table_attr();
  if (e != hipSuccess) return e;
  if (tile_table_wide(T))
    k_tile_table<true, 1024><<<NG, 1024, (size_t)T * sizeof(uint32_t), s>>>(
        T, gx, tile_table_G(G), nblocks_k1, chunk, vis_rec, vis_count, table, tile_total, tile_local, blk_total, ranges, pairs,
        frame, cap_instances, cap_list, host_longest, 0u, nullptr, banded, banded_capacity);
  else
    k_tile_table<true, 512><<<NG, 512, (size_t)T * sizeof(uint32_t), s>>>(
        T, gx, tile_table_G(G), nblocks_k1, chunk, vis_rec, vis_count, table, tile_total, tile_local, blk_total, ranges, pairs,
        frame, cap_instances, cap_list, host_longest, 0u, nullptr, banded, banded_capacity);
  return hipGetLastError();
}

__global__ __launch_bounds__(256) void k_restore_cursors(const uint32_t* __restrict__ ranges,
                                                         uint32_t* __restrict__ cursor, int T) {
  const int t = blockIdx.x * 256 + threadIdx.x;
  if (t < T) cursor[(size_t)t * GCR_CURSOR_STRIDE] = ranges[2 * t];
}

hipError_t gcr_launch_scatter_instances(int nblocks, int chunk, const uint32_t* vis_list,
                                        const uint32_t* vis_count, const float4* rec, int gx,
                                        uint32_t* tile_cursor, uint64_t* pairs, const uint32_t* ranges, int T,
                                        const unsigned long long* frame, hipStream_t s) {
  if (nblocks <= 0) return hipSuccess;
  if (frame == nullptr)
    k_restore_cursors<<<(T + 255) / 256, 256, 0, s>>>(ranges, tile_cursor, T);
  k_scatter_instances<<<nblocks, 256, 0, s>>>(chunk, vis_list, vis_count, rec, gx, tile_cursor, pairs, frame);
  return hipGetLastError();
}

__global__ __launch_bounds__(256) void k_fill_tiles_touched(int chunk, const uint32_t* __restrict__ vis_list,
                                                            const uint32_t* __restrict__ vis_count,
                                                            const float4* __restrict__ rec,
                                                            uint32_t* __restrict__ tiles_touched) {
  const uint32_t nvis = vis_count[blockIdx.x];
  const uint32_t* __restrict__ my_list = vis_list + (size_t)blockIdx.x * chunk;
  for (uint32_t it = threadIdx.x; it < nvis; it += 256) {
    const uint32_t idx = my_list[it];
    const float4 q2 = rec[(size_t)idx * GCR_REC_QUADS + 2];
    const uint32_t rx = __float_as_uint(q2.z), ry = __float_as_uint(q2.w);
    tiles_touched[idx] = ((rx >> 16) - (rx & 0xffffu)) * ((ry >> 16) - (ry & 0xffffu));
  }
}

__global__ __launch_bounds__(256) void k_block_sums(int P, const uint32_t* __restrict__ tiles_touched,
                                                    uint32_t* __restrict__ block_sums) {
  __shared__ uint32_t wsum[4];
  const int idx = blockIdx.x * 256 + threadIdx.x;
  const uint32_t t = idx < P ? tiles_touched[idx] : 0u;
  const uint32_t ws = gcr_wave_sum_u32(t);
  if ((threadIdx.x & 63) == 0) wsum[threadIdx.x >> 6] = ws;
  __syncthreads();
  if (threadIdx.x == 0) block_sums[blockIdx.x] = wsum[0] + wsum[1] + wsum[2] + wsum[3];
}

hipError_t gcr_launch_tiles_touched(int P, int nblocks, int chunk, const uint32_t* vis_list,
                                    const uint32_t* vis_count, const float4* rec, uint32_t* tiles_touched,
                                    uint32_t* block_sums, hipStream_t s) {
  if (P <= 0) return hipSuccess;
  hipError_t e = hipMemsetAsync(tiles_touched, 0, sizeof(uint32_t) * (size_t)P, s);
  if (e != hipSuccess) return e;
  k_fill_tiles_touched<<<nblocks, 256, 0, s>>>(chunk, vis_list, vis_count, rec, tiles_touched);
  k_block_sums<<<(P + 255) / 256, 256, 0, s>>>(P, tiles_touched, block_sums);
  return hipGetLastError();
}

int gcr_tile_sort_capacity(void) { return 4096; }

hipError_t gcr_launch_tile_sort(const uint32_t* ranges, int T, uint64_t* pairs, uint64_t* pairs_spare,
                                uint32_t* list, int64_t list_length_hint, const unsigned long long* frame,
                                uint4* lazy, hipStream_t s) {
  if (T <= 0) return hipSuccess;
  static_assert(GCR_LAZY_MIN == RANK_MERGE_MAX, "lists the lazy path leaves to this kernel take the rank + merge path");
  const int cap = lazy != nullptr ? GCR_LAZY_MIN : gcr_tile_sort_capacity();
  size_t n2 = 64;
  while ((int64_t)n2 < list_length_hint && n2 < (size_t)cap) n2 <<= 1;
  size_t lds = n2 <= (size_t)RANK_MERGE_MAX ? 2 * n2 * sizeof(uint64_t) : n2 * sizeof(uint64_t);
  if (lazy != nullptr && lds < gcr_lazy_lds_keys(GCR_LAZY_CAP_K4) * sizeof(uint64_t))
    lds = gcr_lazy_lds_keys(GCR_LAZY_CAP_K4) * sizeof(uint64_t);
  k_tile_sort<<<T, 256, lds, s>>>(ranges, pairs, pairs_spare, list, frame, (int)n2, lazy);
  return hipGetLastError();
}

int gcr_sort_passes(int end_bit) { return (end_bit + RADIX_BITS - 1) / RADIX_BITS; }

static inline int sort_num_blocks(int64_t R) { return (int)((R + SORT_TILE - 1) / SORT_TILE); }

size_t gcr_sort_hist_bytes(int64_t R, int end_bit) {
  const size_t nb = (size_t)(R > 0 ? sort_num_blocks(R) : 1);
  return sizeof(uint32_t) * (RADIX * nb + (size_t)RADIX * gcr_sort_passes(end_bit));
}

hipError_t gcr_launch_sort(uint64_t* k0, uint32_t* v0, uint64_t* k1, uint32_t* v1, int64_t R,
                           int end_bit, uint32_t* hist, int* sorted_half, hipStream_t s) {
  const int passes = gcr_sort_passes(end_bit);
  *sorted_half = passes & 1;
  if (R <= 0) return hipSuccess;
  const int nb = sort_num_blocks(R);
  uint32_t* table = hist;
  uint32_t* ghist = hist + (size_t)RADIX * nb;
  hipError_t e = hipMemsetAsync(ghist, 0, sizeof(uint32_t) * RADIX * passes, s);
  if (e != hipSuccess) return e;
  uint64_t* kin = k0;
  uint32_t* vin = v0;
  uint64_t* kout = k1;
  uint32_t* vout = v1;
  for (int p = 0; p < passes; p++) {
    const int shift = p * RADIX_BITS;
    uint32_t* gh = ghist + (size_t)p * RADIX;
    k_radix_hist<<<nb, SORT_THREADS, 0, s>>>(kin, R, shift, nb, table, gh);
    k_radix_scan<<<RADIX, 256, 0, s>>>(table, nb);
    k_radix_scatter<<<nb, SORT_THREADS, 0, s>>>(kin, vin, kout, vout, R, shift, nb, table, gh);
    uint64_t* tk = kin; kin = kout; kout = tk;
    uint32_t* tv = vin; vin = vout; vout = tv;
  }
  return hipGetLastError();
}

hipError_t gcr_launch_tile_ranges(const uint64_t* keys, int64_t R, uint32_t* ranges, int T,
                                  hipStream_t s) {
  hipError_t e = hipMemsetAsync(ranges, 0, sizeof(uint32_t) * 2 * (size_t)T, s);
  if (e != hipSuccess) return e;
  if (R <= 0) return hipSuccess;
  k_tile_ranges<<<(unsigned)((R + 255) / 256), 256, 0, s>>>(keys, R, ranges);
  k_ranges_make_contiguous<<<1, 256, 0, s>>>(ranges, T);
  return hipGetLastError();
}
```

### gaussiancity_amd/csrc/gcr_blend.hip

```cpp
#include "gcr_cull.h"
#include "gcr_device.h"
#include "gcr_internal.h"
#include "gcr_sort.h"

namespace {

constexpr int CHUNK = 256;
constexpr uint32_t ENTRY_BYTES = 48;
constexpr int K6_SENT_SLOT = 223;
constexpr int K6_LIST_STRIDE = 232;
static_assert(GCR_PIECE_MAX <= K6_SENT_SLOT, "a K6 chunk must leave slot 255 to the sentinel");
constexpr uint32_t NO_ENTRY = 0xFFFFFFFFu;

struct __attribute__((aligned(16))) StagedEntry {
  float4 a, b, c;
};
static_assert(sizeof(StagedEntry) == ENTRY_BYTES, "StagedEntry must be 48 bytes");

GCR_DEV float gcr_alpha_skip_bound(float opacity) {
  if (!(opacity > 0.0f)) return __builtin_inff();
  return gcr_max(-87.0f, -__builtin_logf(255.0f * opacity) - 1.0e-3f);
}

GCR_DEV float blend_exp(float x) { return gcr_expf_noguard(x); }

struct LaneGeom {
  int lane, w, row, pxi, pyi;
  int bit[4];
};
GCR_DEV LaneGeom lane_geom(int tid, int tx, int ty) {
  LaneGeom g;
  g.lane = tid & 63;
  g.w = tid >> 6;
  g.row = g.lane >> 4;
  const int li = g.lane & 15;
  const int bx = (g.w & 1) * 2 + (g.row & 1), by = (g.w >> 1) * 2 + (g.row >> 1);
  g.pxi = tx * GCR_TILE_X + bx * 4 + (li & 3);
  g.pyi = ty * GCR_TILE_Y + by * 4 + (li >> 2);
#pragma unroll
  for (int rr = 0; rr < 4; rr++) g.bit[rr] = ((g.w >> 1) * 2 + (rr >> 1)) * 4 + (g.w & 1) * 2 + (rr & 1);
  return g;
}

struct LaneGeom6 {
  int lane, w, sub, pxi, pyi;
};
GCR_DEV LaneGeom6 lane_geom6(int tid, int tx, int ty) {
  LaneGeom6 g;
  g.lane = tid & 63;
  g.w = tid >> 6;
  g.sub = g.lane >> 3;
  const int li = g.lane & 7;
  g.pxi = tx * GCR_TILE_X + (g.w & 1) * 8 + (g.sub & 3) * 2 + (li & 1);
  g.pyi = ty * GCR_TILE_Y + (g.w >> 1) * 8 + (g.sub >> 2) * 4 + (li >> 1);
  return g;
}
GCR_DEV uint32_t lane6_to_k7_thread(uint32_t tid) {
  const uint32_t lane = tid & 63u, sub = lane >> 3, li = lane & 7u;
  const uint32_t row4 = (sub >> 2) * 2u + ((sub & 3u) >> 1);
  const uint32_t li4 = (li >> 1) * 4u + (sub & 1u) * 2u + (li & 1u);
  return (tid & ~63u) + row4 * 16u + li4;
}

GCR_DEV long long gcr_out_index(const GcrBlendArgs& a, int px, int py, size_t* plane) {
  const int ox = a.flip_x ? a.W - 1 - px : px, oy = a.flip_y ? a.H - 1 - py : py;
  if (a.win_w == 0) {
    *plane = (size_t)a.H * a.W;
    return (long long)a.W * oy + ox;
  }
  *plane = (size_t)a.win_h * a.win_w;
  const int wx = ox - a.win_x, wy = oy - a.win_y;
  return (wx >= 0 && wx < a.win_w && wy >= 0 && wy < a.win_h) ? (long long)a.win_w * wy + wx : -1ll;
}
GCR_DEV bool gcr_tile_in_window(const GcrBlendArgs& a, int tx, int ty) {
  if (a.win_w == 0) return true;
  int x0 = tx * GCR_TILE_X, x1 = min(a.W, x0 + GCR_TILE_X) - 1, y0 = ty * GCR_TILE_Y, y1 = min(a.H, y0 + GCR_TILE_Y) - 1;
  if (a.flip_x) { const int t = a.W - 1 - x1; x1 = a.W - 1 - x0; x0 = t; }
  if (a.flip_y) { const int t = a.H - 1 - y1; y1 = a.H - 1 - y0; y0 = t; }
  return x1 >= a.win_x && x0 < a.win_x + a.win_w && y1 >= a.win_y && y0 < a.win_y + a.win_h;
}

GCR_DEV uint8_t gcr_video_byte(float c) {
  float t = c < -1.0f ? -1.0f : (c > 1.0f ? 1.0f : c);
  t = t / 2.0f;
  t = t + 0.5f;
  t = t * 255.0f;
  return (uint8_t)(t == t ? (int)t : 0);
}

GCR_DEV uint32_t slot_of_offset(uint32_t off) { return (off * 1366u) >> 16; }

struct K7Behind {
  float T, s0, s1, s2;
};
GCR_DEV K7Behind k7_behind(const float4* __restrict__ ckpt, uint32_t sbase, uint32_t kpiece, uint32_t npieces, uint32_t cs,
                           uint32_t last_contributor, uint32_t thread) {
  K7Behind r = {0.0f, 0.0f, 0.0f, 0.0f};
  if (kpiece + 1u >= npieces) return r;
  r.T = ckpt[(size_t)(sbase + kpiece) * 256u + thread].x;
  const uint32_t my_last = last_contributor > 0u ? (last_contributor - 1u) / cs : 0u;
  for (uint32_t m = npieces - 1u; m > kpiece; m--) {
    const float4 d = ckpt[(size_t)(sbase + m) * 256u + thread];
    const bool mine = m <= my_last;
    r.s0 += mine ? d.y : 0.0f;
    r.s1 += mine ? d.z : 0.0f;
    r.s2 += mine ? d.w : 0.0f;
  }
  return r;
}

#ifndef GCR_K6_SKIP_BRANCH
#define GCR_K6_SKIP_BRANCH 0
#endif
#if GCR_K6_SKIP_BRANCH
#define GCR_K6_WAVE_SKIP(x) (__ballot(x) != 0ull)
#else
#define GCR_K6_WAVE_SKIP(x) true
#endif
#ifndef GCR_K7_ADD_SENTINEL
#define GCR_K7_ADD_SENTINEL 0
#endif
#ifdef GCR_EXPERIMENTS
#define GCR_K6_STEP_ON !(a.debug_flags & 1)
#define GCR_K6_LOOP_ON !(a.debug_flags & 2)
#else
#define GCR_K6_STEP_ON true
#define GCR_K6_LOOP_ON true
#endif
__device__ __noinline__ uint32_t k6_lazy_extend(uint64_t* s, const uint64_t* keys, uint32_t n, uint32_t* out, uint4* state) {
  const int tid = threadIdx.x;
  uint32_t* w = reinterpret_cast<uint32_t*>(state);
  uint32_t ns = __hip_atomic_load(w, __ATOMIC_RELAXED, __HIP_MEMORY_SCOPE_AGENT);
  uint64_t l = (uint64_t)__hip_atomic_load(w + 2, __ATOMIC_RELAXED, __HIP_MEMORY_SCOPE_AGENT) |
               ((uint64_t)__hip_atomic_load(w + 3, __ATOMIC_RELAXED, __HIP_MEMORY_SCOPE_AGENT) << 32);
  gcr_lazy_extend<GCR_LAZY_CAP_K6>(s, keys, n, ns, l, out, tid);
  if (tid == 0) {
    __hip_atomic_store(w, ns, __ATOMIC_RELAXED, __HIP_MEMORY_SCOPE_AGENT);
    __hip_atomic_store(w + 2, (uint32_t)l, __ATOMIC_RELAXED, __HIP_MEMORY_SCOPE_AGENT);
    __hip_atomic_store(w + 3, (uint32_t)(l >> 32), __ATOMIC_RELAXED, __HIP_MEMORY_SCOPE_AGENT);
  }
  __syncthreads();
  return ns;
}

__device__ __noinline__ void k6_frame_gate(unsigned long long* words, unsigned int seq, unsigned int max_polls) {
  gcr_store_to_host(words + 3, (unsigned long long)seq);
  for (unsigned int i = 0; i < max_polls; i++) {
    const unsigned long long v = __hip_atomic_load(words + 2, __ATOMIC_RELAXED, __HIP_MEMORY_SCOPE_SYSTEM);
    if ((unsigned int)v == seq) return;
    __builtin_amdgcn_s_sleep(127);
    __builtin_amdgcn_s_sleep(127);
  }
  gcr_store_to_host(words + 4, (unsigned long long)seq);
  asm volatile("s_waitcnt vmcnt(0)" ::: "memory");
  const unsigned long long st = __hip_atomic_load(words + 7, __ATOMIC_RELAXED, __HIP_MEMORY_SCOPE_SYSTEM);
  if ((unsigned int)st != seq) return;
  for (unsigned long long i = 0; i < 16ull * max_polls; i++) {
    const unsigned long long v = __hip_atomic_load(words + 2, __ATOMIC_RELAXED, __HIP_MEMORY_SCOPE_SYSTEM);
    if ((unsigned int)v == seq) return;
    __builtin_amdgcn_s_sleep(127);
    __builtin_amdgcn_s_sleep(127);
  }
}

template <bool SORT, bool STATE, bool PIXSTATE>
__global__ __launch_bounds__(256) __attribute__((amdgpu_waves_per_eu(8, 8))) void k_blend_fwd(const GcrBlendArgs a) {
  __shared__ StagedEntry sE[K6_SENT_SLOT + 1];
  __shared__ uint32_t sMask[CHUNK];
  __shared__ __attribute__((aligned(16))) uint8_t sList[4][8][K6_LIST_STRIDE];

  if (a.frame != nullptr && a.frame[2] == 0ull) {
    if (a.gate_words != nullptr && blockIdx.x == 0 && threadIdx.x == 0) k6_frame_gate(a.gate_words, a.gate_seq, a.gate_polls);
    return;
  }
  const int tile = blockIdx.x;
  const int tx = tile % a.gx, ty = tile / a.gx;
  const int tid = threadIdx.x;
  const float tile_x0 = (float)(tx * GCR_TILE_X), tile_y0 = (float)(ty * GCR_TILE_Y);
  const uint32_t r0 = a.ranges[2 * tile], r1 = a.ranges[2 * tile + 1];
  if (!gcr_tile_in_window(a, tx, ty)) {
    if (STATE && a.work != nullptr) {
      const uint32_t P0 = (uint32_t)a.piece, sb = r0 / P0 + (uint32_t)tile, ns = r1 / P0 + 1u - r0 / P0;
      for (uint32_t k = tid; k < ns; k += 256u) a.work[sb + k] = make_uint4(GCR_NO_TILE, 0u, 0u, 0u);
      if (tile == 0 && tid == 0) {
        a.frame_out[GCR_FRAME_PIECE] = P0;
        a.frame_out[GCR_FRAME_CKPT_OFF] = a.ckpt_off;
        a.frame_out[GCR_FRAME_WORK_OFF] = a.work_off;
        a.frame_out[GCR_FRAME_MASK_OFF] = a.mask_off;
        a.frame_out[GCR_FRAME_STAGED_OFF] = a.staged_off;
        a.frame_out[GCR_FRAME_CARVE] = a.carve_bytes;
      }
    }
    return;
  }
  const int total = (int)(r1 - r0);
  const char* const sEb = reinterpret_cast<const char*>(sE);
#ifdef GCR_EXPERIMENTS
  if (a.clock_buf != nullptr && tid == 0) {
    unsigned long long* o = a.clock_buf + (size_t)tile * 16;
    o[0] = (unsigned long long)__builtin_amdgcn_s_getreg(63492) | ((unsigned long long)__builtin_amdgcn_s_getreg(63508) << 32);
    o[1] = __builtin_readcyclecounter();
    o[3] = (unsigned long long)total;
    o[10] = __builtin_readcyclecounter();
  }
#endif
  if (tid == 0) {
    sE[K6_SENT_SLOT].a = make_float4(0.0f, 0.0f, 0.0f, 0.0f);
    sE[K6_SENT_SLOT].b = make_float4(0.0f, 0.0f, 0.0f, 0.0f);
    sE[K6_SENT_SLOT].c = make_float4(0.0f, __builtin_inff(), 0.0f, 0.0f);
  }
  static_assert(gcr_lazy_lds_keys(GCR_LAZY_CAP_K6) * 8 <= K6_SENT_SLOT * (int)ENTRY_BYTES, "the lazy sort's scratch must end below the sentinel");

  float Tw;
  {
    const LaneGeom6 g0 = lane_geom6(tid, tx, ty);
    Tw = (g0.pxi < a.W && g0.pyi < a.H) ? 1.0f : -1.0f;
  }
  float C0 = 0.0f, C1 = 0.0f, C2 = 0.0f;
  float D0 = 0.0f, D1 = 0.0f, D2 = 0.0f;
  uint32_t last_contributor = 0;
  const uint32_t piece_P = (uint32_t)a.piece;
  const int cs = (int)gcr_piece_size((uint32_t)total, piece_P);
  const uint32_t sbase = r0 / piece_P + (uint32_t)tile;
  uint32_t entered = 0;

  uint32_t lz_sorted = (uint32_t)max(total, 0);
  if (!SORT && a.lazy != nullptr) lz_sorted = a.lazy[tile].x;

  uint32_t sorted_id = 0;
  if (SORT && total > 0) {
    const uint64_t* __restrict__ seg = a.pairs + r0;
    uint32_t* __restrict__ out = a.list_out + r0;
    if (total <= K6_SENT_SLOT) {
      uint64_t* sKey = reinterpret_cast<uint64_t*>(sE);
      const uint64_t mine = tid < total ? seg[tid] : ~0ull;
      sKey[tid] = mine;
      __syncthreads();
      const ulonglong2* k2 = reinterpret_cast<const ulonglong2*>(sKey);
      uint32_t rank = 0;
      for (int j = 0; j < (total + 1) / 2; j++) {
        const ulonglong2 kk = k2[j];
        rank += (kk.x < mine ? 1u : 0u) + (kk.y < mine ? 1u : 0u);
      }
      __syncthreads();
      if (tid < total) {
        sMask[rank] = (uint32_t)mine;
        out[rank] = (uint32_t)mine;
      }
      __syncthreads();
      sorted_id = tid < total ? sMask[tid] : 0u;
      __syncthreads();
    } else {
      for (int i = tid; i < total; i += 256) {
        const uint64_t mine = seg[i];
        uint32_t rank = 0;
        for (int j = 0; j < total; j++) rank += seg[j] < mine ? 1u : 0u;
        out[rank] = (uint32_t)mine;
      }
      __syncthreads();
    }
  }

#define GCR_BLEND_STEP(QA, QB, QC, OFF)                                                      \
  {                                                                                          \
    const float dx = QA.x - pixx, dy = QA.y - pixy;                                          \
    const float power = __builtin_fmaf(QA.w * dx, dy, __builtin_fmaf(QB.x * dy, dy, (QA.z * dx) * dx)); \
    const bool in_range = !(power > 0.0f) && !(power < QC.y);                                \
    if (GCR_K6_WAVE_SKIP(in_range) && GCR_K6_STEP_ON) {                     \
        \
      const float araw = __builtin_fminf(0.99f, QB.y * blend_exp(power));          \
      const bool valid = in_range && !(araw < 1.0f / 255.0f);                                \
      const float a_eff = valid ? araw : 0.0f;                                               \
      const float test_T = Tw * (1 - a_eff);                                                 \
      const bool keep = !(test_T < 0.0001f);                                                 \
      const float wgt = keep ? a_eff : 0.0f;                                                 \
      C0 = __builtin_fmaf(QB.z * wgt, Tw, C0);                                               \
      C1 = __builtin_fmaf(QB.w * wgt, Tw, C1);                                               \
      C2 = __builtin_fmaf(QC.x * wgt, Tw, C2);                                               \
      if (STATE) {     \
        D0 = __builtin_fmaf(QB.z * wgt, Tw, D0);                                             \
        D1 = __builtin_fmaf(QB.w * wgt, Tw, D1);                                             \
        D2 = __builtin_fmaf(QC.x * wgt, Tw, D2);                                             \
      }                                                                                      \
      if (PIXSTATE) last_off = (keep && valid) ? (OFF) : last_off;                           \
      Tw = keep ? test_T : -__builtin_fabsf(Tw);                                             \
    }                                                                                        \
  }
#define GCR_BLEND_LOAD(QA, QB, QC, OFF)                            \
  QA = *reinterpret_cast<const float4*>(sEb + (OFF));             \
  QB = *reinterpret_cast<const float4*>(sEb + (OFF) + 16);         \
  QC = *reinterpret_cast<const float2*>(sEb + (OFF) + 32);

  int base = 0;
  bool finished = false;
  while (base < total && !finished && GCR_K6_LOOP_ON) {
  if (!SORT) {
    const uint32_t need = (uint32_t)(base + min(cs, total - base));
    while (lz_sorted < need) {
      const uint32_t ns = k6_lazy_extend(reinterpret_cast<uint64_t*>(sE), a.pairs + r0, (uint32_t)total,
                                         a.list_out + r0, a.lazy + tile);
      lz_sorted = (uint32_t)__builtin_amdgcn_readfirstlane((int)ns);
    }
  }
  int tid_op = threadIdx.x;
  asm volatile("" : "+v"(tid_op));
  const LaneGeom6 g = lane_geom6(tid_op, tx, ty);
  const int lane = g.lane;
  const float pixx = (float)g.pxi, pixy = (float)g.pyi;
  const int w_u = __builtin_amdgcn_readfirstlane(g.w);
  const int mask_sh = (w_u >> 1) * 16 + (w_u & 1) * 4;
  uint8_t* const lw = &sList[w_u][0][0];
  for (; base < total; base += cs) {
    if (__syncthreads_count(!(Tw > 0.0f)) == 256) {
      finished = true;
      break;
    }
    if (!SORT && lz_sorted < (uint32_t)(base + min(cs, total - base))) break;
    if (STATE && entered > 0u && a.ckpt != nullptr) {
      uint32_t t_op = threadIdx.x;
      asm volatile("" : "+v"(t_op));
      a.ckpt[(size_t)(sbase + entered - 1u) * 256u + lane6_to_k7_thread(t_op)] = make_float4(__builtin_fabsf(Tw), D0, D1, D2);
      D0 = D1 = D2 = 0.0f;
    }
    entered++;
    const int n = min(cs, total - base);
    uint32_t my_mask = 0;
    if (tid < n) {
      const uint32_t id = !SORT ? a.list[r0 + base + tid]
                                : ((total <= K6_SENT_SLOT && cs == total) ? sorted_id : a.list_out[r0 + base + tid]);
      const float4* __restrict__ rec = a.rec + (size_t)id * GCR_REC_QUADS;
#ifdef GCR_EXPERIMENTS
      if (a.clock_buf != nullptr && tid == 0 && base == 0) {
        asm volatile("s_waitcnt vmcnt(0)" ::: "memory");
        a.clock_buf[(size_t)tile * 16 + 8] = __builtin_readcyclecounter();
      }
#endif
      const float4 q0 = rec[0], q1 = rec[1], q2 = rec[2];
#ifdef GCR_EXPERIMENTS
      if (a.clock_buf != nullptr && tid == 0 && base == 0) {
        asm volatile("s_waitcnt vmcnt(0)" ::: "memory");
        a.clock_buf[(size_t)tile * 16 + 9] = __builtin_readcyclecounter();
      }
#endif
      const float pmin = gcr_alpha_skip_bound(q1.y);
      my_mask = gcr_block_mask_2x4(q0.x, q0.y, q0.z, q0.w, q1.x, pmin, tile_x0, tile_y0);
      const float4 sa = make_float4(q0.x, q0.y, -0.5f * q0.z, -q0.w), sb = make_float4(-0.5f * q1.x, q1.y, q1.z, q1.w);
      const float4 sc = make_float4(q2.x, pmin, 0.0f, 0.0f);
      sE[tid].a = sa;
      sE[tid].b = sb;
      sE[tid].c = sc;
      if (STATE && a.staged_out != nullptr) {
        float4* __restrict__ so = a.staged_out + (size_t)(r0 + (uint32_t)base + (uint32_t)tid) * 3;
        so[0] = sa;
        so[1] = sb;
        so[2] = sc;
      }
    }
    sMask[tid] = my_mask;
    if (STATE && tid < n && a.mask_out != nullptr)
      a.mask_out[r0 + base + tid] = (uint16_t)gcr_block_mask_4x4_of_2x4(my_mask);
    __syncthreads();
#ifdef GCR_EXPERIMENTS
    if (a.clock_buf != nullptr && tid == 0 && base == 0) a.clock_buf[(size_t)tile * 16 + 4] = __builtin_readcyclecounter();
#endif
    if (__ballot(Tw > 0.0f) == 0ull) continue;
    {
      constexpr int NQ = 8 * K6_LIST_STRIDE / 16;
      static_assert(8 * K6_LIST_STRIDE % 16 == 0 && NQ > 64 && NQ <= 128, "list fill: two stores per lane");
      uint4* const f = reinterpret_cast<uint4*>(lw);
      const uint32_t sb = 0x01010101u * (uint32_t)K6_SENT_SLOT;
      const uint4 ff = make_uint4(sb, sb, sb, sb);
      f[lane] = ff;
      if (64 + lane < NQ) f[64 + lane] = ff;
    }
    int cnt[8] = {0, 0, 0, 0, 0, 0, 0, 0};
#pragma unroll
    for (int k = 0; k < 4; k++) {
      if (k * 64 < n) {
        const int jj = k * 64 + lane;
        const uint32_t m = sMask[jj] >> mask_sh;
#pragma unroll
        for (int s = 0; s < 8; s++) {
          uint32_t bit = m & (1u << (s < 4 ? s : s + 4));
          asm volatile("" : "+v"(bit));
          const bool rel = bit != 0u;
          const uint64_t bal = __ballot(rel);
          const uint32_t before = __builtin_amdgcn_mbcnt_hi((uint32_t)(bal >> 32), __builtin_amdgcn_mbcnt_lo((uint32_t)bal, 0u));
          if (rel) lw[s * K6_LIST_STRIDE + cnt[s] + (int)before] = (uint8_t)jj;
          cnt[s] += __popcll(bal);
        }
      }
    }
    const int maxcnt = __builtin_amdgcn_readfirstlane(
        max(max(max(cnt[0], cnt[1]), max(cnt[2], cnt[3])), max(max(cnt[4], cnt[5]), max(cnt[6], cnt[7]))));
    __builtin_amdgcn_wave_barrier();
#ifdef GCR_EXPERIMENTS
    if (a.clock_buf != nullptr && tid == 0 && base == 0) {
      a.clock_buf[(size_t)tile * 16 + 5] = __builtin_readcyclecounter();
      a.clock_buf[(size_t)tile * 16 + 7] = (unsigned long long)maxcnt;
    }
#endif
    const uint8_t* lp = &sList[w_u][g.sub][0];
    float4 qa0, qb0, qa1, qb1;
    float2 qc0, qc1;
    uint32_t e0 = (uint32_t)lp[0] * ENTRY_BYTES, e1 = (uint32_t)lp[1] * ENTRY_BYTES;
    uint32_t last_off = NO_ENTRY;
    GCR_BLEND_LOAD(qa0, qb0, qc0, e0)
    for (int i = 0; i < maxcnt; i += 2, lp += 2) {
      GCR_BLEND_LOAD(qa1, qb1, qc1, e1)
      const uint32_t cur0 = e0;
      e0 = (uint32_t)lp[2] * ENTRY_BYTES;
      GCR_BLEND_STEP(qa0, qb0, qc0, cur0)
      if (i + 1 >= maxcnt) break;
      GCR_BLEND_LOAD(qa0, qb0, qc0, e0)
      const uint32_t cur1 = e1;
      e1 = (uint32_t)lp[3] * ENTRY_BYTES;
      GCR_BLEND_STEP(qa1, qb1, qc1, cur1)
      if (__ballot(Tw > 0.0f) == 0ull) break;
    }
#ifdef GCR_EXPERIMENTS
    if (a.clock_buf != nullptr && tid == 0 && base == 0) a.clock_buf[(size_t)tile * 16 + 6] = __builtin_readcyclecounter();
#endif
    if (PIXSTATE && last_off != NO_ENTRY) last_contributor = (uint32_t)base + slot_of_offset(last_off) + 1u;
  }
  }
#undef GCR_BLEND_STEP
#undef GCR_BLEND_LOAD
  int tid_end = threadIdx.x;
  asm volatile("" : "+v"(tid_end));
  const LaneGeom6 g = lane_geom6(tid_end, tx, ty);
  static_assert(PIXSTATE || !STATE, "the backward reads final_T / n_contrib");
  if (g.pxi < a.W && g.pyi < a.H) {
    const float Tout = __builtin_fabsf(Tw);
    const size_t pix_id = (size_t)a.W * g.pyi + g.pxi;
    const bool nt_out = !STATE && a.nt_out != 0;
    if (!PIXSTATE) {
    } else if (nt_out) {
      __builtin_nontemporal_store(Tout, a.final_T + pix_id);
      __builtin_nontemporal_store(last_contributor, a.n_contrib + pix_id);
    } else {
      a.final_T[pix_id] = Tout;
      a.n_contrib[pix_id] = last_contributor;
    }
    size_t oplane = 0;
    int px_op = g.pxi, py_op = g.pyi;
    asm volatile("" : "+v"(px_op), "+v"(py_op));
    const long long out_id = (!STATE || a.out_color != nullptr) ? gcr_out_index(a, px_op, py_op, &oplane) : -1;
    if (out_id >= 0) {
      const float c0 = C0 + Tout * GCR_CAM(a, bg, a.bg, 0);
      const float c1 = C1 + Tout * GCR_CAM(a, bg, a.bg, 1);
      const float c2 = C2 + Tout * GCR_CAM(a, bg, a.bg, 2);
      if (!STATE && a.out_u8) {
        uint8_t* o = reinterpret_cast<uint8_t*>(a.out_color) + 3 * (size_t)out_id;
        o[0] = gcr_video_byte(c0);
        o[1] = gcr_video_byte(c1);
        o[2] = gcr_video_byte(c2);
      } else if (nt_out) {
        __builtin_nontemporal_store(c0, a.out_color + out_id);
        __builtin_nontemporal_store(c1, a.out_color + oplane + out_id);
        __builtin_nontemporal_store(c2, a.out_color + 2 * oplane + out_id);
      } else {
        a.out_color[out_id] = c0;
        a.out_color[oplane + out_id] = c1;
        a.out_color[2 * oplane + out_id] = c2;
      }
    }
  }
#ifdef GCR_EXPERIMENTS
  if (a.clock_buf != nullptr && tid == 0) a.clock_buf[(size_t)tile * 16 + 2] = __builtin_readcyclecounter();
#endif
  if (STATE && a.work != nullptr) {
    if (entered >= 2u)
      a.ckpt[(size_t)(sbase + entered - 1u) * 256u + lane6_to_k7_thread((uint32_t)tid)] =
          make_float4(__builtin_fabsf(Tw), D0, D1, D2);
    const uint32_t nslots = r1 / piece_P + 1u - r0 / piece_P;
    for (uint32_t k = tid; k < nslots; k += 256u)
      a.work[sbase + k] = k < entered ? make_uint4((uint32_t)tile, r0, (uint32_t)total, k) : make_uint4(GCR_NO_TILE, 0u, 0u, 0u);
  }
  if (STATE && a.work != nullptr && tile == 0 && tid == 0) {
    a.frame_out[GCR_FRAME_PIECE] = piece_P;
    a.frame_out[GCR_FRAME_CKPT_OFF] = a.ckpt_off;
    a.frame_out[GCR_FRAME_WORK_OFF] = a.work_off;
    a.frame_out[GCR_FRAME_MASK_OFF] = a.mask_off;
    a.frame_out[GCR_FRAME_STAGED_OFF] = a.staged_off;
    a.frame_out[GCR_FRAME_CARVE] = a.carve_bytes;
  }
}

#ifdef GCR_EXPERIMENTS
#define GCR_K7_NCLK 8
#define GCR_K7_CLK(i) \
  if (clk_on) clk[i] = __builtin_readcyclecounter();
#define GCR_FLUSH_ON !(a.debug_flags & 1)
#define GCR_LDS_ADD_ON !(a.debug_flags & 4)
#define GCR_STEP_ON !(a.debug_flags & 16)
#define GCR_K7_IEEE_DIV (a.debug_flags & 64)
#define GCR_PASSES_ON !(a.debug_flags & 32)
#else
#define GCR_K7_IEEE_DIV false
#define GCR_STEP_ON true
#define GCR_PASSES_ON true
#define GCR_K7_CLK(i)
#define GCR_FLUSH_ON true
#define GCR_LDS_ADD_ON true
#endif

constexpr int WPASS = 64;
constexpr int WLIST_STRIDE = WPASS + 8;
constexpr uint32_t WSENT_OFF = WPASS * ENTRY_BYTES;

#ifndef GCR_K7_RS_ASM
#define GCR_K7_RS_ASM 1
#endif
#if GCR_K7_RS_ASM
#define GCR_K7_ROW_SLOT gcr_row_reduce_scatter9_b_slot(lane)
#define GCR_K7_ROW_SUMS                                                                                        \
  float rs_r;                                                                                                  \
  const float rs_8 = gcr_row_reduce_scatter9_b(v[0], v[1], v[2], v[3], v[4], v[5], v[6], v[7], v[8], rs_r);    \
  const float rsum = acc_slot == 8 ? rs_8 : rs_r;
#else
#define GCR_K7_ROW_SLOT ((lane & 15) <= 8 ? (lane & 15) : -1)
#define GCR_K7_ROW_SUMS const float rsum = gcr_row_reduce_scatter9(v, lane);
#endif
#define GCR_BWD_STEP(QA, QB, QC)                                                               \
  {                                                                                            \
    const float dx = QA.x - pixx, dy = QA.y - pixy;                                            \
    const float power_raw = __builtin_fmaf(QA.w * dx, dy, __builtin_fmaf(QB.x * dy, dy, (QA.z * dx) * dx)); \
    const bool in_range = __float_as_uint(QC.z) < last_contributor && !(power_raw > 0.0f) &&   \
                          !(power_raw < QC.y);                                                 \
    if (GCR_K7_WAVE_SKIP(in_range) && GCR_STEP_ON) {    \
      const float power = in_range ? power_raw : 0.0f;                                         \
      const float G = blend_exp(power);                                                        \
      const float alpha = __builtin_fminf(0.99f, QB.y * G);                                    \
      const bool use = in_range && !(alpha < 1.0f / 255.0f);                                   \
      const float a_eff = use ? alpha : 0.0f;                                                  \
      const float om = 1.f - a_eff;                                                            \
      const float rc0 = __builtin_amdgcn_rcpf(om);                                             \
      const float rcp = __builtin_fmaf(rc0, __builtin_fmaf(-om, rc0, 1.0f), rc0);              \
      T = GCR_K7_IEEE_DIV ? T / om : T * rcp;                                                  \
      const float dchannel_dcolor = a_eff * T;                                                 \
      const float oml = 1.f - last_alpha;                                                      \
      acc0 = __builtin_fmaf(last_alpha, lc0, oml * acc0);                                      \
      acc1 = __builtin_fmaf(last_alpha, lc1, oml * acc1);                                      \
      acc2 = __builtin_fmaf(last_alpha, lc2, oml * acc2);                                      \
      lc0 = QB.z;                                                                              \
      lc1 = QB.w;                                                                              \
      lc2 = QC.x;                                                                              \
      last_alpha = a_eff;                                                                      \
      float dL_dalpha = (lc0 - acc0) * dLp0;                                                   \
      dL_dalpha = __builtin_fmaf(lc1 - acc1, dLp1, dL_dalpha);                                 \
      dL_dalpha = __builtin_fmaf(lc2 - acc2, dLp2, dL_dalpha);                                 \
      dL_dalpha = GCR_K7_IEEE_DIV ? dL_dalpha * T + nbg / om : __builtin_fmaf(nbg, rcp, dL_dalpha * T); \
      dL_dalpha = use ? dL_dalpha : 0.0f;                                                      \
      const float u = G * dL_dalpha;                                                           \
      const float ux = u * dx, uy = u * dy;                                                    \
      float v[9];                                                                              \
      v[0] = dchannel_dcolor * dLp0;                                                           \
      v[1] = dchannel_dcolor * dLp1;                                                           \
      v[2] = dchannel_dcolor * dLp2;                                                           \
      v[3] = ux;                                                                               \
      v[4] = uy;                                                                               \
      v[5] = ux * dx;                                                                          \
      v[6] = ux * dy;                                                                          \
      v[7] = uy * dy;                                                                          \
      v[8] = u;                                                                                \
       \
       \
      GCR_K7_ROW_SUMS                                                                          \
      if (acc_slot >= 0 && GCR_LDS_ADD_ON && (GCR_K7_ADD_SENTINEL || __float_as_uint(QC.z) != NO_ENTRY))                 \
        atomicAdd(reinterpret_cast<double*>(acc_base + __float_as_uint(QC.w)), (double)rsum);                             \
    }                                                                                          \
  }
#ifndef GCR_K7_SKIP_BRANCH
#define GCR_K7_SKIP_BRANCH 0
#endif
#ifndef GCR_K7_XCD_MAP
#define GCR_K7_XCD_MAP 1
#endif
#if GCR_K7_SKIP_BRANCH
#define GCR_K7_WAVE_SKIP(x) (__ballot(x) != 0ull)
#else
#define GCR_K7_WAVE_SKIP(x) true
#endif
#ifdef GCR_EXPERIMENTS
#define GCR_BWD_LOAD(QA, QB, QC, OFF)                              \
  QA = *reinterpret_cast<const float4*>(sEb + (OFF));             \
  if (!(a.debug_flags & 8)) {                                      \
    QB = *reinterpret_cast<const float4*>(sEb + (OFF) + 16);       \
    QC = *reinterpret_cast<const float4*>(sEb + (OFF) + 32);       \
  } else {                                                         \
    QB = make_float4(QA.z, 0.5f, QA.x, QA.y);                      \
    QC = make_float4(QA.w, -5.0f, __uint_as_float(0u), __uint_as_float(0u)); \
  }
#else
#define GCR_BWD_LOAD(QA, QB, QC, OFF)                              \
  QA = *reinterpret_cast<const float4*>(sEb + (OFF));             \
  QB = *reinterpret_cast<const float4*>(sEb + (OFF) + 16);         \
  QC = *reinterpret_cast<const float4*>(sEb + (OFF) + 32);
#endif



#ifdef GCR_K7_WAVES_PER_EU
#define GCR_K7_OCC __attribute__((amdgpu_waves_per_eu(GCR_K7_WAVES_PER_EU, 8)))
#else
#define GCR_K7_OCC
#endif
__global__ __launch_bounds__(64) GCR_K7_OCC void k_blend_bwd(const GcrBlendArgs a) {
  __shared__ StagedEntry sE[WPASS + 1];
  __shared__ uint32_t sId[WPASS];
  __shared__ uint16_t sList[4][WLIST_STRIDE];
  __shared__ uint16_t sRel[WPASS];
  __shared__ double sAcc[WPASS * 9];

  const int lane = threadIdx.x;
  if ((int)blockIdx.x < a.fill.blocks) {
    for (int sgi = 0; sgi < a.fill.nseg; sgi++)
      gcr_fill_zero_segment<64>(a.fill.ptr[sgi], a.fill.n[sgi], (int)blockIdx.x, a.fill.blocks, lane);
    return;
  }
#ifdef GCR_EXPERIMENTS
  bool clk_on = a.clock_buf != nullptr;
  unsigned long long clk[GCR_K7_NCLK] = {};
#endif
  GCR_K7_CLK(0)
  if (!gcr_frame_has_state(a.frame_in, a.binning_bytes)) return;
  const uint32_t piece_P = (uint32_t)a.frame_in[GCR_FRAME_PIECE];
  const unsigned long long nunits = 4ull * gcr_piece_slots(a.R, (unsigned long long)(a.gx * a.gy), piece_P);
  const float4* __restrict__ ckpt = reinterpret_cast<const float4*>(a.binning_base + a.frame_in[GCR_FRAME_CKPT_OFF]);
  const uint4* __restrict__ work = reinterpret_cast<const uint4*>(a.binning_base + a.frame_in[GCR_FRAME_WORK_OFF]);
  const uint16_t* __restrict__ masks = reinterpret_cast<const uint16_t*>(a.binning_base + a.frame_in[GCR_FRAME_MASK_OFF]);
  const float4* __restrict__ staged = reinterpret_cast<const float4*>(a.binning_base + a.frame_in[GCR_FRAME_STAGED_OFF]);
  const uint64_t lt_mask = (1ull << lane) - 1ull;
  const int acc_slot = GCR_K7_ROW_SLOT;
  const float bg0 = GCR_CAM(a, bg, a.bg, 0), bg1 = GCR_CAM(a, bg, a.bg, 1), bg2 = GCR_CAM(a, bg, a.bg, 2);
  const char* const sEb = reinterpret_cast<const char*>(sE);
  char* const acc_base = reinterpret_cast<char*>(&sAcc[acc_slot >= 0 ? acc_slot : 0]);
  if (lane == 0) {
    sE[WPASS].a = make_float4(0.0f, 0.0f, 0.0f, 0.0f);
    sE[WPASS].b = make_float4(0.0f, 0.0f, 0.0f, 0.0f);
    sE[WPASS].c = make_float4(0.0f, __builtin_inff(), __uint_as_float(NO_ENTRY), 0.0f);
  }
#pragma unroll
  for (int k = 0; k < 9; k++) sAcc[k * WPASS + lane] = 0.0;

  const unsigned long long nvirt = (nunits + 31ull) & ~31ull;
  for (unsigned long long v = (unsigned long long)blockIdx.x - (unsigned long long)a.fill.blocks; v < nvirt;
       v += (unsigned long long)gridDim.x - (unsigned long long)a.fill.blocks) {
#if GCR_K7_XCD_MAP
    const unsigned long long item = (v >> 5) * 8ull + (v & 7ull);
    const int q = (int)((v >> 3) & 3ull);
#else
    const unsigned long long item = v >> 2;
    const int q = (int)(v & 3ull);
#endif
    if (4ull * item >= nunits) continue;
    uint4 d = work[item];
    asm volatile("" : "+v"(d.x), "+v"(d.y), "+v"(d.z), "+v"(d.w));
    if (d.x == GCR_NO_TILE) continue;
    const int tile = (int)d.x;
    const uint32_t r0 = d.y, len = d.z, kpiece = d.w;
    const uint32_t npieces = gcr_piece_count(len, piece_P), cs = gcr_piece_size(len, piece_P);
    const uint32_t lo = kpiece * cs, hi = min(len, lo + cs);
    const uint32_t sbase = r0 / piece_P + (uint32_t)tile;
    const int tx = tile % a.gx, ty = tile / a.gx;
    const LaneGeom g = lane_geom(q * 64 + lane, tx, ty);
    const uint32_t quad_bits = (1u << g.bit[0]) | (1u << g.bit[1]) | (1u << g.bit[2]) | (1u << g.bit[3]);
    const bool inside = g.pxi < a.W && g.pyi < a.H;
    const float pixx = (float)g.pxi, pixy = (float)g.pyi;
    const size_t pix_id = (size_t)a.W * g.pyi + g.pxi;

    const float T_final = inside ? a.final_T[pix_id] : 0.0f;
    const uint32_t last_contributor = inside ? a.n_contrib[pix_id] : 0u;
    float dLp0 = 0.0f, dLp1 = 0.0f, dLp2 = 0.0f;
    if (inside) {
      size_t iplane;
      const long long in_id = gcr_out_index(a, g.pxi, g.pyi, &iplane);
      if (in_id >= 0) {
        dLp0 = a.dL_dpix[in_id];
        dLp1 = a.dL_dpix[iplane + in_id];
        dLp2 = a.dL_dpix[2 * iplane + in_id];
      }
    }
    const K7Behind ck = k7_behind(ckpt, sbase, kpiece, npieces, cs, last_contributor, (uint32_t)(q * 64 + lane));
    float bg_dot_dpixel = 0;
    bg_dot_dpixel += bg0 * dLp0;
    bg_dot_dpixel += bg1 * dLp1;
    bg_dot_dpixel += bg2 * dLp2;
    uint32_t row_max = last_contributor;
#pragma unroll
    for (int o = 8; o > 0; o >>= 1) {
      const uint32_t t = __shfl_xor(row_max, o, 64);
      row_max = t > row_max ? t : row_max;
    }
    uint32_t rmax[4];
#pragma unroll
    for (int rr = 0; rr < 4; rr++) rmax[rr] = __shfl(row_max, rr * 16, 64);
    const uint32_t wave_max = max(max(rmax[0], rmax[1]), max(rmax[2], rmax[3]));
    GCR_K7_CLK(1)
    if (wave_max <= lo || !GCR_PASSES_ON) continue;
    const int top = (int)min(hi, wave_max);

    float T = T_final;
    float acc0 = 0.0f, acc1 = 0.0f, acc2 = 0.0f;
    if (last_contributor > hi) {
      T = ck.T;
      acc0 = ck.s0 / ck.T;
      acc1 = ck.s1 / ck.T;
      acc2 = ck.s2 / ck.T;
    }
    const float nbg = -T_final * bg_dot_dpixel;
    float last_alpha = 0.0f, lc0 = 0.0f, lc1 = 0.0f, lc2 = 0.0f;

    const int npass = (top - (int)lo + WPASS - 1) / WPASS;
    uint32_t wm0, wm1, wm2, wm3, wi0, wi1, wi2, wi3;
#define GCR_K7_WINDOW(K, M, I)                                         \
  {                                                                    \
    const int e = top - 1 - (K) * WPASS - lane;                        \
    const bool hv = (K) < npass && e >= (int)lo;                       \
    M = hv ? (uint32_t)masks[r0 + (uint32_t)(hv ? e : 0)] : 0u;        \
    I = hv ? a.list[r0 + (uint32_t)(hv ? e : 0)] : 0u;                 \
  }
    GCR_K7_WINDOW(0, wm0, wi0)
    GCR_K7_WINDOW(1, wm1, wi1)
    GCR_K7_WINDOW(2, wm2, wi2)
    GCR_K7_WINDOW(3, wm3, wi3)
#undef GCR_K7_WINDOW
    bool rel_n = (wm0 & quad_bits) != 0u;
    float4 n0 = make_float4(0.0f, 0.0f, 0.0f, 0.0f), n1 = n0, n2 = n0;
    if (rel_n) {
      const float4* __restrict__ rec = staged + (size_t)(r0 + (uint32_t)(top - 1 - lane)) * 3;
      n0 = rec[0];
      n1 = rec[1];
      n2 = rec[2];
    }
    for (int k = 0; k < npass; k++) {
      const int e_l = top - 1 - k * WPASS - lane;
      const uint32_t m16 = wm0, id = wi0;
      const bool any_rel = rel_n;
      const float4 q0 = n0, q1 = n1, q2 = n2;
      wm0 = wm1; wm1 = wm2; wm2 = wm3; wm3 = 0u;
      wi0 = wi1; wi1 = wi2; wi2 = wi3; wi3 = 0u;
      rel_n = k + 1 < npass && (wm0 & quad_bits) != 0u;
      if (rel_n) {
        const float4* __restrict__ rec = staged + (size_t)(r0 + (uint32_t)(top - 1 - (k + 1) * WPASS - lane)) * 3;
        n0 = rec[0];
        n1 = rec[1];
        n2 = rec[2];
      }
      const uint64_t rel_bal = __ballot(any_rel);
      if (rel_bal == 0ull) continue;
      if (any_rel) {
        sE[lane].a = q0;
        sE[lane].b = q1;
        sE[lane].c = make_float4(q2.x, q2.y, __uint_as_float((uint32_t)e_l), __uint_as_float((uint32_t)lane * 72u));
        sId[lane] = id;
        sRel[__popcll(rel_bal & lt_mask)] = (uint16_t)lane;
      }
      const int nrel = __popcll(rel_bal);
      int maxcnt = 0;
      int cnt[4];
#pragma unroll
      for (int rr = 0; rr < 4; rr++) {
        const bool rel = ((m16 >> g.bit[rr]) & 1u) && (uint32_t)e_l < rmax[rr];
        const uint64_t bal = __ballot(rel);
        if (rel) sList[rr][__popcll(bal & lt_mask)] = (uint16_t)(lane * (int)ENTRY_BYTES);
        cnt[rr] = __popcll(bal);
        maxcnt = max(maxcnt, cnt[rr]);
      }
#pragma unroll
      for (int rr = 0; rr < 4; rr++)
        for (int s = cnt[rr] + lane; s < maxcnt + 3; s += 64) sList[rr][s] = (uint16_t)WSENT_OFF;
      __builtin_amdgcn_wave_barrier();
      GCR_K7_CLK(2)

      const uint16_t* lp = &sList[g.row][0];
      float4 qa0, qb0, qc0, qa1, qb1, qc1;
      uint32_t e0 = lp[0], e1 = lp[1];
      GCR_BWD_LOAD(qa0, qb0, qc0, e0)
      for (int i = 0; i < maxcnt; i += 2, lp += 2) {
        GCR_BWD_LOAD(qa1, qb1, qc1, e1)
        e0 = lp[2];
        GCR_BWD_STEP(qa0, qb0, qc0)
        if (i + 1 >= maxcnt) break;
        GCR_BWD_LOAD(qa0, qb0, qc0, e0)
        e1 = lp[3];
        GCR_BWD_STEP(qa1, qb1, qc1)
      }
      __builtin_amdgcn_wave_barrier();
      GCR_K7_CLK(3)
      {
        const int comp = lane & 15;
        const int rec_idx = comp < 3 ? comp : (comp == 8 ? 3 : comp + 1);
        if (comp < 9) {
          for (int i = lane >> 4; i < nrel; i += 4) {
            const int slot = (int)sRel[i];
            const float v = (float)sAcc[slot * 9 + comp];
            if (v != 0.0f) {
              sAcc[slot * 9 + comp] = 0.0;
              if (!GCR_FLUSH_ON) continue;
              if (!a.deterministic) {
                atomicAdd(&a.grad_rec[(size_t)sId[slot] * GCR_GRAD_REC_FLOATS + rec_idx], v);
              } else {
                const uint32_t gid = sId[slot];
                const float4 q2 = a.rec[(size_t)gid * GCR_REC_QUADS + 2];
                const int kc = gcr_det_frac_bits(sE[slot].a.x, sE[slot].a.y, __float_as_uint(q2.z), __float_as_uint(q2.w), 2);
                const int ko = gcr_det_frac_bits(sE[slot].a.x, sE[slot].a.y, __float_as_uint(q2.z), __float_as_uint(q2.w), 0);
                const int k1 = gcr_det_frac_bits(sE[slot].a.x, sE[slot].a.y, __float_as_uint(q2.z), __float_as_uint(q2.w), 1);
                const int cls = gcr_det_class(rec_idx);
                const int kf = cls == 2 ? kc : (cls == 1 ? k1 : ko);
                const float sc = __builtin_ldexpf(v, kf);
                const long long q = sc >= 9.2e18f ? 0x7fffffffffffffffll : (sc <= -9.2e18f ? -0x7fffffffffffffffll : __float2ll_rn(sc));
                unsigned long long* const r64 = reinterpret_cast<unsigned long long*>(a.grad_rec) + (size_t)gid * (GCR_GRAD_REC_FLOATS_DET / 2);
                atomicAdd(r64 + rec_idx, (unsigned long long)q);
                r64[GCR_DET_K_SLOT] = (unsigned long long)(kc + 64) | ((unsigned long long)(ko + 64) << 8) |
                                      ((unsigned long long)(k1 + 64) << 16);
              }
            }
          }
        }
      }
      __builtin_amdgcn_wave_barrier();
    }
#ifdef GCR_EXPERIMENTS
    if (clk_on) {
      clk[4] = __builtin_readcyclecounter();
      if (lane == 0) {
        unsigned long long* o = a.clock_buf + (size_t)blockIdx.x * (GCR_K7_NCLK + 2);
        o[0] = (unsigned long long)__builtin_amdgcn_s_getreg(63492) |
               ((unsigned long long)__builtin_amdgcn_s_getreg(63508) << 32);
        o[1] = (unsigned long long)(top - (int)lo);
        for (int i = 0; i < GCR_K7_NCLK; i++) o[2 + i] = clk[i];
      }
      clk_on = false;
    }
#endif
  }
}

#ifndef GCR_K7_IPASS
#define GCR_K7_IPASS GCR_PIECE_MAX
#endif
#ifdef GCR_K7_ITEM_WAVES
#define GCR_K7_ITEM_OCC __attribute__((amdgpu_waves_per_eu(GCR_K7_ITEM_WAVES, GCR_K7_ITEM_WAVES)))
#else
#define GCR_K7_ITEM_OCC
#endif
constexpr int IPASS = GCR_K7_IPASS;
constexpr int ILIST_STRIDE = IPASS + 9;
static_assert(IPASS < 256, "one thread per piece entry, byte list slots (slot IPASS = the sentinel)");

__global__ __launch_bounds__(256) GCR_K7_ITEM_OCC void k_blend_bwd_item(const GcrBlendArgs a) {
  __shared__ StagedEntry sE[IPASS + 1];
  __shared__ uint32_t sId[IPASS + 1];
  __shared__ uint16_t sMask[256];
  __shared__ uint8_t sList[4][4][ILIST_STRIDE];
  __shared__ double sAcc[IPASS * 9];

  const int tid = threadIdx.x;
  if ((int)blockIdx.x < a.fill.blocks) {
    for (int sgi = 0; sgi < a.fill.nseg; sgi++)
      gcr_fill_zero_segment<256>(a.fill.ptr[sgi], a.fill.n[sgi], (int)blockIdx.x, a.fill.blocks, tid);
    return;
  }
  if (!gcr_frame_has_state(a.frame_in, a.binning_bytes)) return;
  const uint32_t piece_P = (uint32_t)a.frame_in[GCR_FRAME_PIECE];
  const unsigned long long nitems = gcr_piece_slots(a.R, (unsigned long long)(a.gx * a.gy), piece_P);
  const float4* __restrict__ ckpt = reinterpret_cast<const float4*>(a.binning_base + a.frame_in[GCR_FRAME_CKPT_OFF]);
  const uint4* __restrict__ work = reinterpret_cast<const uint4*>(a.binning_base + a.frame_in[GCR_FRAME_WORK_OFF]);
  const uint16_t* __restrict__ masks = reinterpret_cast<const uint16_t*>(a.binning_base + a.frame_in[GCR_FRAME_MASK_OFF]);
  const float4* __restrict__ staged = reinterpret_cast<const float4*>(a.binning_base + a.frame_in[GCR_FRAME_STAGED_OFF]);
  const int lane = tid & 63;
  const int q = __builtin_amdgcn_readfirstlane(tid >> 6);
  const uint64_t lt_mask = (1ull << lane) - 1ull;
  const int acc_slot = GCR_K7_ROW_SLOT;
  const float bg0 = GCR_CAM(a, bg, a.bg, 0), bg1 = GCR_CAM(a, bg, a.bg, 1), bg2 = GCR_CAM(a, bg, a.bg, 2);
  const char* const sEb = reinterpret_cast<const char*>(sE);
  char* const acc_base = reinterpret_cast<char*>(&sAcc[acc_slot >= 0 ? acc_slot : 0]);
  if (tid == 0) {
    sE[IPASS].a = make_float4(0.0f, 0.0f, 0.0f, 0.0f);
    sE[IPASS].b = make_float4(0.0f, 0.0f, 0.0f, 0.0f);
    sE[IPASS].c = make_float4(0.0f, __builtin_inff(), __uint_as_float(NO_ENTRY), 0.0f);
  }

  bool first = true;
  for (unsigned long long item = (unsigned long long)blockIdx.x - (unsigned long long)a.fill.blocks; item < nitems;
       item += (unsigned long long)gridDim.x - (unsigned long long)a.fill.blocks) {
    uint4 d = work[item];
    asm volatile("" : "+v"(d.x), "+v"(d.y), "+v"(d.z), "+v"(d.w));
    if (d.x == GCR_NO_TILE) continue;
    if (!first) __syncthreads();
    first = false;
    const int tile = (int)d.x;
    const uint32_t r0 = d.y, len = d.z, kpiece = d.w;
    const uint32_t npieces = gcr_piece_count(len, piece_P), cs = gcr_piece_size(len, piece_P);
    const uint32_t lo = kpiece * cs, hi = min(len, lo + cs);
    const int n = __builtin_amdgcn_readfirstlane((int)min(hi - lo, (uint32_t)IPASS));
    const uint32_t sbase = r0 / piece_P + (uint32_t)tile;
    const int tx = tile % a.gx, ty = tile / a.gx;
    const LaneGeom g = lane_geom(tid, tx, ty);
    const bool inside = g.pxi < a.W && g.pyi < a.H;
    const float pixx = (float)g.pxi, pixy = (float)g.pyi;
    const size_t pix_id = (size_t)a.W * g.pyi + g.pxi;

    const bool hv = tid < n;
    const uint32_t e_t = hi - 1u - (uint32_t)(hv ? tid : 0);
    const uint32_t m16 = hv ? (uint32_t)masks[r0 + e_t] : 0u;
    const uint32_t id = hv ? a.list[r0 + e_t] : 0u;
    const float T_final = inside ? a.final_T[pix_id] : 0.0f;
    const uint32_t last_contributor = inside ? a.n_contrib[pix_id] : 0u;
    float dLp0 = 0.0f, dLp1 = 0.0f, dLp2 = 0.0f;
    if (inside) {
      size_t iplane;
      const long long in_id = gcr_out_index(a, g.pxi, g.pyi, &iplane);
      if (in_id >= 0) {
        dLp0 = a.dL_dpix[in_id];
        dLp1 = a.dL_dpix[iplane + in_id];
        dLp2 = a.dL_dpix[2 * iplane + in_id];
      }
    }
    const K7Behind ck = k7_behind(ckpt, sbase, kpiece, npieces, cs, last_contributor, (uint32_t)tid);
    for (int k = tid; k < n * 9; k += 256) sAcc[k] = 0.0;

    if (hv) {
      const float4* __restrict__ rec = staged + (size_t)(r0 + e_t) * 3;
      const float4 q0 = rec[0], q1 = rec[1], q2 = rec[2];
      if (m16 != 0u) {
        sE[tid].a = q0;
        sE[tid].b = q1;
        sE[tid].c = make_float4(q2.x, q2.y, __uint_as_float(e_t), __uint_as_float((uint32_t)tid * 72u));
        sId[tid] = id;
      }
    }
    sMask[tid] = (uint16_t)m16;

    float bg_dot_dpixel = 0;
    bg_dot_dpixel += bg0 * dLp0;
    bg_dot_dpixel += bg1 * dLp1;
    bg_dot_dpixel += bg2 * dLp2;
    uint32_t row_max = last_contributor;
#pragma unroll
    for (int o = 8; o > 0; o >>= 1) {
      const uint32_t t = __shfl_xor(row_max, o, 64);
      row_max = t > row_max ? t : row_max;
    }
    uint32_t rmax[4];
#pragma unroll
    for (int rr = 0; rr < 4; rr++) rmax[rr] = __shfl(row_max, rr * 16, 64);
    const uint32_t wave_max = max(max(rmax[0], rmax[1]), max(rmax[2], rmax[3]));

    float T = T_final;
    float acc0 = 0.0f, acc1 = 0.0f, acc2 = 0.0f;
    if (last_contributor > hi) {
      T = ck.T;
      acc0 = ck.s0 / ck.T;
      acc1 = ck.s1 / ck.T;
      acc2 = ck.s2 / ck.T;
    }
    const float nbg = -T_final * bg_dot_dpixel;
    float last_alpha = 0.0f, lc0 = 0.0f, lc1 = 0.0f, lc2 = 0.0f;
    __syncthreads();

    if (wave_max > lo && GCR_PASSES_ON) {
      uint8_t* const lw = &sList[q][0][0];
      int cnt[4] = {0, 0, 0, 0};
#pragma unroll
      for (int k = 0; k < 4; k++) {
        if (k * 64 < n) {
          const int j = k * 64 + lane;
          const uint32_t m = (uint32_t)sMask[j];
          const uint32_t e_j = hi - 1u - (uint32_t)j;
#pragma unroll
          for (int rr = 0; rr < 4; rr++) {
            const bool rel = ((m >> g.bit[rr]) & 1u) && e_j < rmax[rr];
            const uint64_t bal = __ballot(rel);
            if (rel) lw[rr * ILIST_STRIDE + cnt[rr] + __popcll(bal & lt_mask)] = (uint8_t)j;
            cnt[rr] += __popcll(bal);
          }
        }
      }
      const int maxcnt = __builtin_amdgcn_readfirstlane(max(max(cnt[0], cnt[1]), max(cnt[2], cnt[3])));
#pragma unroll
      for (int rr = 0; rr < 4; rr++)
        for (int s = cnt[rr] + lane; s < maxcnt + 3; s += 64) lw[rr * ILIST_STRIDE + s] = (uint8_t)IPASS;
      __builtin_amdgcn_wave_barrier();

      const uint8_t* lp = &sList[q][g.row][0];
      float4 qa0, qb0, qc0, qa1, qb1, qc1;
      uint32_t e0 = (uint32_t)lp[0] * ENTRY_BYTES, e1 = (uint32_t)lp[1] * ENTRY_BYTES;
      GCR_BWD_LOAD(qa0, qb0, qc0, e0)
      for (int i = 0; i < maxcnt; i += 2, lp += 2) {
        GCR_BWD_LOAD(qa1, qb1, qc1, e1)
        e0 = (uint32_t)lp[2] * ENTRY_BYTES;
        GCR_BWD_STEP(qa0, qb0, qc0)
        if (i + 1 >= maxcnt) break;
        GCR_BWD_LOAD(qa0, qb0, qc0, e0)
        e1 = (uint32_t)lp[3] * ENTRY_BYTES;
        GCR_BWD_STEP(qa1, qb1, qc1)
      }
    }
    __syncthreads();
    {
      const int comp = tid & 15;
      const int rec_idx = comp < 3 ? comp : (comp == 8 ? 3 : comp + 1);
      if (comp < 9 && GCR_FLUSH_ON) {
        for (int i = tid >> 4; i < n; i += 16) {
          const float v = (float)sAcc[i * 9 + comp];
          if (v != 0.0f) atomicAdd(&a.grad_rec[(size_t)sId[i] * GCR_GRAD_REC_FLOATS + rec_idx], v);
        }
      }
    }
  }
}

#undef GCR_BWD_STEP
#undef GCR_BWD_LOAD

}

template <bool SORT>
static void launch_blend_fwd_state(const GcrBlendArgs& a, int T, hipStream_t s) {
  size_t pad = 0;
#ifdef GCR_EXPERIMENTS
  if (const char* e = getenv("GCR_K6_LDS_PAD")) pad = (size_t)atoll(e);
#endif
  if (a.work != nullptr)
    k_blend_fwd<SORT, true, true><<<T, 256, pad, s>>>(a);
  else if (!SORT && a.image_only)
    k_blend_fwd<false, false, false><<<T, 256, pad, s>>>(a);
  else
    k_blend_fwd<SORT, false, true><<<T, 256, pad, s>>>(a);
}

hipError_t gcr_launch_blend_fwd(const GcrBlendArgs& a, bool sort_in_kernel, hipStream_t s) {
  const int T = a.gx * a.gy;
  if (T <= 0) return hipSuccess;
  if (sort_in_kernel)
    launch_blend_fwd_state<true>(a, T, s);
  else
    launch_blend_fwd_state<false>(a, T, s);
  return hipGetLastError();
}

hipError_t gcr_launch_blend_bwd(const GcrBlendArgs& a, bool wave_units, hipStream_t s) {
  const int T = a.gx * a.gy;
  if (T <= 0) return hipSuccess;
  unsigned long long items = gcr_piece_slots(a.R, (unsigned long long)T, (unsigned long long)a.piece);
  if (wave_units || a.deterministic) {
    unsigned long long units = (4ull * items + 31ull) & ~31ull;
#ifdef GCR_EXPERIMENTS
    if (const char* env = getenv("GCR_K7_BLOCKS")) units = (unsigned long long)atoll(env);
#endif
    const unsigned int grid = (unsigned int)(units > 0x3fffffe0ull ? 0x3fffffe0ull : units) + (unsigned int)a.fill.blocks;
    k_blend_bwd<<<grid, 64, 0, s>>>(a);
  } else {
    GcrBlendArgs b = a;
    b.fill.blocks = (a.fill.blocks + 3) / 4;
    const unsigned int grid = (unsigned int)(items > 0x3fffffffull ? 0x3fffffffull : items) + (unsigned int)b.fill.blocks;
    k_blend_bwd_item<<<grid, 256, 0, s>>>(b);
  }
  return hipGetLastError();
}
```

### gaussiancity_amd/csrc/gcr_internal.h

```cpp
#pragma once
#include <hip/hip_runtime.h>
#include <stdint.h>

#include "../../include/gcr.h"
#include "gcr_tt_row.h"

#define GCR_REC_QUADS 4
#define GCR_COV3D_FLOATS 8

#define GCR_CURSOR_STRIDE 32

struct GcrCamVals {
  int by_value;
  float view[16], proj[16], campos[3], bg[3];
};
#define GCR_CAM(A, FIELD, PTR, i) ((A).cam.by_value ? (A).cam.FIELD[i] : (PTR)[i])

struct GcrPreprocessArgs {
  int P, D, M, W, H, gx, gy;
  float tanfovx, tanfovy, focal_x, focal_y, scale_modifier;
  const float *means3D, *scales, *rotations, *opacities, *shs, *cov3D_precomp, *colors_precomp;
  const float *view, *proj, *campos;
  int32_t* radii;
  float4* rec;
  float* cov3D;
  uint32_t* tile_count;
  uint32_t* vis_list;
  uint32_t* vis_count;
  uint4* vis_rec;
  uint32_t* cand_list;
  uint32_t* cand_count;
  unsigned long long* block_tiles;
  int nblocks, chunk;
  int s_mean, s_opac, s_col, s_scale, s_rot;
  int prefiltered;
  const float4* cull_cache;
  const float4* cull_shape;
  int nt_stream;
  GcrCamVals cam;
};

#define GCR_PREFILTER_FLAG (1ull << 63)
#define GCR_PREFILTER_MARK 0xFFFFFFFEull

#define GCR_K1_MAX_BLOCKS 2048
int gcr_preprocess_resident_blocks();
static inline void gcr_preprocess_grid(int P, int max_blocks, int* nblocks, int* chunk) {
  int nb = (P + 255) / 256;
  if (nb > max_blocks) nb = max_blocks;
  if (nb < 1) nb = 1;
  long long c = ((long long)P + nb - 1) / nb;
  c = (c + 255) / 256 * 256;
  if (c < 256) c = 256;
  if (c < 512 && (long long)P >= 512ll * 512ll) c = 512;
  *chunk = (int)c;
  *nblocks = (int)(((long long)P + c - 1) / c);
  if (*nblocks < 1) *nblocks = 1;
}

struct GcrPreprocessBwdArgs {
  int P, D, M, W, H;
  float tanfovx, tanfovy, focal_x, focal_y, scale_modifier;
  const float *means3D, *scales, *rotations, *shs, *cov3D;
  const float *view, *proj, *campos;
  const int32_t* radii;
  int s_cov3d;
  const uint32_t *vis_list, *vis_count;
  int nblocks, chunk;
  const float4* grad_rec;
  const float4* rec;
  const unsigned long long* frame;
  unsigned long long binning_bytes;
  float *dL_dmean2D, *dL_dcolor, *dL_dopacity;
  float *dL_dmean3D, *dL_dcov3D, *dL_dsh, *dL_dscale, *dL_drot;
  int deterministic;
  int s_mean, s_scale, s_rot;
  int g_mean, g_opac, g_col, g_scale, g_rot;
  GcrCamVals cam;
};

#define GCR_GRAD_REC_FLOATS 16
#define GCR_GRAD_REC_FLOATS_DET 32
#define GCR_DET_K_SLOT 15
static inline __host__ __device__ int gcr_det_class(int rec_slot) { return rec_slot >= 6 ? 2 : (rec_slot >= 4 ? 1 : 0); }
static inline __host__ __device__ int gcr_det_frac_bits(float x, float y, uint32_t rect_x, uint32_t rect_y, int cls) {
  const float minx = 16.0f * (float)(rect_x & 0xffffu), maxx = 16.0f * (float)(rect_x >> 16);
  const float miny = 16.0f * (float)(rect_y & 0xffffu), maxy = 16.0f * (float)(rect_y >> 16);
  const float npix = (maxx - minx) * (maxy - miny);
  const float ax = x - minx, bx = x - maxx, ay = y - miny, by = y - maxy;
  const float dx2 = ax * ax > bx * bx ? ax * ax : bx * bx, dy2 = ay * ay > by * by ? ay * ay : by * by;
  float d2 = cls == 2 ? dx2 + dy2 : (cls == 1 ? __builtin_sqrtf(dx2 + dy2) : 64.0f);
  d2 = d2 > 64.0f ? d2 : 64.0f;
  float B = npix * d2 * 64.0f;
  B = B > 1.0f ? B : 1.0f;
  union { float f; uint32_t u; } c;
  c.f = B;
  const int e = (int)((c.u >> 23) & 0xffu) - 127 + 1;
  const int k = 61 - e;
  return k > 44 ? 44 : (k < -16 ? -16 : k);
}

#define GCR_FILL_SEGMENTS 8
struct GcrFillArgs {
  float* ptr[GCR_FILL_SEGMENTS];
  unsigned long long n[GCR_FILL_SEGMENTS];
  int nseg;
  int blocks;
};

#define GCR_PIECE_MIN 64
#define GCR_PIECE_MAX 223
#define GCR_NO_TILE 0xFFFFFFFFu
#define GCR_CKPT_BYTES 4096
static inline __host__ __device__ uint32_t gcr_piece_count(uint32_t len, uint32_t P) { return (len + P - 1u) / P; }
static inline __host__ __device__ uint32_t gcr_piece_size(uint32_t len, uint32_t P) {
  const uint32_t n = gcr_piece_count(len, P);
  return n ? (len + n - 1u) / n : 0u;
}
static inline __host__ __device__ unsigned long long gcr_piece_slots(unsigned long long R, unsigned long long T,
                                                                     unsigned long long P) {
  return R / P + T;
}
#define GCR_FRAME_PIECE 3
#define GCR_FRAME_CKPT_OFF 4
#define GCR_FRAME_WORK_OFF 5
#define GCR_FRAME_MASK_OFF 7
#define GCR_FRAME_CARVE 6
#define GCR_FRAME_STAGED_OFF 8
#define GCR_BAND_SORT_MIN_DEFAULT 6000000
#define GCR_FRAME_BANDED 9
static inline __host__ __device__ bool gcr_frame_has_state(const unsigned long long* frame, unsigned long long binning_bytes) {
  return frame[GCR_FRAME_PIECE] != 0ull && frame[GCR_FRAME_CARVE] <= binning_bytes;
}

struct GcrBlendArgs {
  const uint32_t* ranges;
  const uint32_t* list;
  const uint64_t* pairs;
  uint32_t* list_out;
  const float4* rec;
  int W, H, gx, gy;
  const float* bg;
  float* final_T;
  uint32_t* n_contrib;
  float* out_color;
  const unsigned long long* frame;
  const float* dL_dpix;
  float* grad_rec;
  GcrFillArgs fill;
  int deterministic;
  int win_x, win_y, win_w, win_h;
  int flip_x, flip_y;
  int out_u8;
  int nt_out;
  int image_only;
  GcrCamVals cam;
  int debug_flags;
  int piece;
  float4* ckpt;
  uint4* work;
  uint16_t* mask_out;
  unsigned long long mask_off;
  float4* staged_out;
  unsigned long long staged_off;
  unsigned long long* frame_out;
  unsigned long long ckpt_off, work_off;
  unsigned long long carve_bytes;
  unsigned long long* gate_words;
  unsigned int gate_seq, gate_polls;
  unsigned long long binning_bytes;
  const char* binning_base;
  const unsigned long long* frame_in;
  uint4* lazy;
  unsigned long long R;
#ifdef GCR_EXPERIMENTS
  unsigned long long* clock_buf;
#endif
};

hipError_t gcr_launch_mark_visible(int P, const float* means3D, const float* view, uint8_t* present,
                                   hipStream_t s);
hipError_t gcr_launch_preprocess(const GcrPreprocessArgs& a, bool split, hipStream_t s);
hipError_t gcr_launch_build_cull_cache(const GcrPreprocessArgs& a, float4* outA, float4* outB, hipStream_t s);
static inline size_t gcr_cull_cache_offset_b(int P) { return (((size_t)P * 16) + 127) & ~(size_t)127; }
hipError_t gcr_launch_zero_grad_records(int nblocks, int chunk, const uint32_t* vis_list, const uint32_t* vis_count,
                                        float4* grad_rec, int rec_quads, hipStream_t s);
hipError_t gcr_launch_fill(const GcrFillArgs& f, hipStream_t s);
hipError_t gcr_launch_scan_block_sums(uint32_t* block_sums, int n, unsigned long long* total,
                                      hipStream_t s);
hipError_t gcr_launch_tiles_touched(int P, int nblocks, int chunk, const uint32_t* vis_list,
                                    const uint32_t* vis_count, const float4* rec, uint32_t* tiles_touched,
                                    uint32_t* block_sums, hipStream_t s);
hipError_t gcr_launch_emit(int P, const uint32_t* tiles_touched, const uint32_t* block_offsets,
                           const float4* rec, int gx, uint64_t* keys, uint32_t* vals,
                           hipStream_t s);
hipError_t gcr_launch_scan_tiles(uint32_t* tile_cursor, int stride, uint32_t* ranges, int T,
                                 unsigned long long* frame, unsigned long long cap_instances,
                                 unsigned long long cap_list, unsigned long long* host_R, unsigned int seq,
                                 const unsigned long long* block_tiles, int nblocks_k1, hipStream_t s);
int gcr_tile_table_groups(int T, int nblocks_k1, int* G_out);
hipError_t gcr_launch_tile_count(int T, int gx, int NG, int G, int nblocks_k1, int chunk, const uint4* vis_rec,
                                 const uint32_t* vis_count, uint32_t* table,
                                 uint32_t* tile_total, uint32_t* tile_local, uint32_t* blk_total,
                                 unsigned long long* frame, const unsigned long long* block_tiles,
                                 unsigned long long* host_R, unsigned int seq, uint4* banded, int banded_capacity,
                                 hipStream_t s);
bool gcr_band_sort_possible(int T);
hipError_t gcr_launch_tile_scatter(int T, int gx, int NG, int G, int nblocks_k1, int chunk, const uint4* vis_rec,
                                   const uint32_t* vis_count, uint32_t* table,
                                   const uint32_t* tile_total, const uint32_t* tile_local,
                                   const uint32_t* blk_total, uint32_t* ranges, uint64_t* pairs,
                                   unsigned long long* frame, unsigned long long cap_instances,
                                   unsigned long long cap_list, unsigned long long* host_longest,
                                   const uint4* banded, int banded_capacity, hipStream_t s);
hipError_t gcr_launch_scatter_instances(int nblocks, int chunk, const uint32_t* vis_list,
                                        const uint32_t* vis_count, const float4* rec, int gx,
                                        uint32_t* tile_cursor, uint64_t* pairs, const uint32_t* ranges, int T,
                                        const unsigned long long* frame, hipStream_t s);
int gcr_tile_sort_capacity(void);
hipError_t gcr_launch_tile_sort(const uint32_t* ranges, int T, uint64_t* pairs, uint64_t* pairs_spare,
                                uint32_t* list, int64_t list_length_hint, const unsigned long long* frame,
                                uint4* lazy, hipStream_t s);
size_t gcr_sort_hist_bytes(int64_t R, int end_bit);
hipError_t gcr_launch_sort(uint64_t* k0, uint32_t* v0, uint64_t* k1, uint32_t* v1, int64_t R,
                           int end_bit, uint32_t* hist, int* sorted_half, hipStream_t s);
int gcr_sort_passes(int end_bit);
hipError_t gcr_launch_tile_ranges(const uint64_t* keys, int64_t R, uint32_t* ranges, int T,
                                  hipStream_t s);
hipError_t gcr_launch_blend_fwd(const GcrBlendArgs& a, bool sort_in_kernel, hipStream_t s);
hipError_t gcr_launch_blend_bwd(const GcrBlendArgs& a, bool wave_units, hipStream_t s);
hipError_t gcr_launch_preprocess_bwd(const GcrPreprocessBwdArgs& a, hipStream_t s);

static inline uint32_t gcr_higher_msb(uint32_t n) {
  uint32_t msb = sizeof(n) * 4;
  uint32_t step = msb;
  while (step > 1) {
    step /= 2;
    if (n >> msb)
      msb += step;
    else
      msb -= step;
  }
  if (n >> msb) msb++;
  return msb;
}
```

### gaussiancity_amd/csrc/gcr_sort.h

```cpp
#pragma once
#include "gcr_device.h"

GCR_DEV void gcr_bitonic_sort_lds(uint64_t* s, int N2, int tid) {
  const int half = N2 >> 1, wave_pairs = half >> 2;
  const int lane = tid & 63, w = tid >> 6;
  const int span = N2 >> 2;
  bool prev_local = false;
  for (int k = 2; k <= N2; k <<= 1) {
    for (int j = k >> 1; j > 0; j >>= 1) {
      const bool local = 2 * j <= span;
      if (!local && prev_local) __syncthreads();
      for (int t = lane; t < wave_pairs; t += 64) {
        const int i = w * wave_pairs + t;
        const int a = ((i & ~(j - 1)) << 1) | (i & (j - 1));
        const int b = a | j;
        const uint64_t x = s[a], y = s[b];
        const bool ascending = (a & k) == 0;
        if ((x > y) == ascending) {
          s[a] = y;
          s[b] = x;
        }
      }
      if (local)
        __builtin_amdgcn_wave_barrier();
      else
        __syncthreads();
      prev_local = local;
    }
  }
  __syncthreads();
}

GCR_DEV void gcr_tile_sort_long(uint64_t* s, uint32_t run0, uint64_t* __restrict__ A, uint64_t* __restrict__ B,
                                uint32_t* __restrict__ out, uint32_t n, int tid) {
  for (uint32_t c0 = 0; c0 < n; c0 += run0) {
    const uint32_t len = min(run0, n - c0);
    for (uint32_t i = tid; i < run0; i += 256) s[i] = i < len ? A[c0 + i] : ~0ull;
    __syncthreads();
    gcr_bitonic_sort_lds(s, (int)run0, tid);
    for (uint32_t i = tid; i < len; i += 256) A[c0 + i] = s[i];
    __syncthreads();
  }
  uint64_t* src = A;
  uint64_t* dst = B;
  __shared__ uint32_t win_ia[258];
  for (uint32_t run = run0; run < n; run <<= 1) {
    for (uint32_t p0 = 0; p0 < n; p0 += 2 * run) {
      const uint32_t la = min(run, n - p0);
      const uint32_t lb = p0 + run < n ? min(run, n - p0 - run) : 0u;
      const uint64_t* __restrict__ a = src + p0;
      const uint64_t* __restrict__ b = src + p0 + run;
      uint64_t* __restrict__ o = dst + p0;
      const uint32_t tot = la + lb;
      if (lb == 0u) {
        for (uint32_t i = tid; i < la; i += 256) o[i] = a[i];
        continue;
      }
      const uint32_t nwin = (tot + run0 - 1) / run0;
      for (uint32_t w0 = 0; w0 < nwin; w0 += 256) {
        const uint32_t wn = min(256u, nwin - w0);
        __syncthreads();
        for (uint32_t q = tid; q <= wn; q += 256) {
          const uint32_t d = min(tot, (w0 + q) * run0);
          uint32_t lo = d > lb ? d - lb : 0u, hi = min(d, la);
          while (lo < hi) {
            const uint32_t mid = (lo + hi) >> 1;
            if (a[mid] < b[d - 1 - mid])
              lo = mid + 1;
            else
              hi = mid;
          }
          win_ia[q] = lo;
        }
        __syncthreads();
        for (uint32_t w = 0; w < wn; w++) {
          const uint32_t d0 = (w0 + w) * run0, d1 = min(tot, d0 + run0);
          const uint32_t ia0 = win_ia[w], ia1 = win_ia[w + 1];
          const uint32_t ib0 = d0 - ia0, ib1 = d1 - ia1;
          const uint32_t na = ia1 - ia0, nb = ib1 - ib0;
          for (uint32_t i = tid; i < na; i += 256) s[i] = a[ia0 + i];
          for (uint32_t i = tid; i < nb; i += 256) s[na + i] = b[ib0 + i];
          __syncthreads();
          for (uint32_t i = tid; i < na + nb; i += 256) {
            const uint64_t key = s[i];
            const bool from_a = i < na;
            const uint64_t* other = from_a ? s + na : s;
            uint32_t lo = 0, hi = from_a ? nb : na;
            while (lo < hi) {
              const uint32_t mid = (lo + hi) >> 1;
              if (other[mid] < key)
                lo = mid + 1;
              else
                hi = mid;
            }
            o[d0 + (from_a ? i : i - na) + lo] = key;
          }
          __syncthreads();
        }
      }
    }
    __syncthreads();
    uint64_t* t = src;
    src = dst;
    dst = t;
  }
  for (uint32_t i = tid; i < n; i += 256) out[i] = (uint32_t)src[i];
}

constexpr int GCR_LAZY_MIN = 1024;
constexpr int GCR_LAZY_SAMPLES = 256;
constexpr int GCR_LAZY_CAP_K6 = 1024;
#ifndef GCR_LAZY_CAP_K4
#define GCR_LAZY_CAP_K4 1024
#endif
constexpr int gcr_lazy_lds_keys(int cap) { return cap + GCR_LAZY_SAMPLES + 3; }

template <int GCR_LAZY_CAP>
GCR_DEV void gcr_lazy_extend(uint64_t* s, const uint64_t* keys, uint32_t n, uint32_t& n_sorted, uint64_t& L,
                             uint32_t* out, int tid) {
  constexpr int GCR_LAZY_TARGET = GCR_LAZY_CAP * 3 / 4;
  uint64_t* samp = s + GCR_LAZY_CAP;
  uint32_t* cnt_w = reinterpret_cast<uint32_t*>(s + GCR_LAZY_CAP + GCR_LAZY_SAMPLES);
  unsigned long long* lo_w = reinterpret_cast<unsigned long long*>(s + GCR_LAZY_CAP + GCR_LAZY_SAMPLES + 1);
  unsigned long long* hi_w = lo_w + 1;
  const uint32_t rem = n - n_sorted;
  const int lane = tid & 63;
  const uint64_t lt_mask = (1ull << lane) - 1ull;
  uint32_t m = 0, j = 0;
  uint64_t U = ~0ull;
  __syncthreads();
  if (rem > (uint32_t)GCR_LAZY_CAP) {
    const uint64_t k = keys[((uint64_t)tid * n) >> 8];
    const bool cand = k >= L;
    const uint64_t mine = cand ? k : ~0ull;
    s[tid] = mine;
    m = (uint32_t)__syncthreads_count(cand);
    const ulonglong2* s2 = reinterpret_cast<const ulonglong2*>(s);
    uint32_t rank = 0;
#pragma unroll 2
    for (int q = 0; q < GCR_LAZY_SAMPLES / 2; q++) {
      const ulonglong2 kk = s2[q];
      rank += (kk.x < mine ? 1u : 0u) + (kk.y < mine ? 1u : 0u);
    }
    if (cand) samp[rank] = mine;
    j = (uint32_t)(((uint64_t)GCR_LAZY_TARGET * m) / rem);
    j = max(1u, min(j, m));
    __syncthreads();
    if (m > 0u && j < m) U = samp[j];
  }
  uint32_t cnt = 0;
  for (int guard = 0; guard < 160; guard++) {
    if (tid == 0) {
      *cnt_w = 0u;
      *lo_w = ~0ull;
      *hi_w = 0ull;
    }
    __syncthreads();
    uint64_t lo_k = ~0ull, hi_k = 0ull;
#pragma unroll 1
    for (uint32_t i0 = 0; i0 < n; i0 += 256u) {
      const uint32_t i = i0 + (uint32_t)tid;
      const uint64_t k = i < n ? keys[i] : ~0ull;
      const bool in = k >= L && k < U;
      const uint64_t bal = __ballot(in);
      if (bal != 0ull) {
        uint32_t base = 0;
        if (lane == 0) base = atomicAdd(cnt_w, (uint32_t)__popcll(bal));
        base = (uint32_t)__builtin_amdgcn_readfirstlane((int)base);
        if (in) {
          const uint32_t pos = base + (uint32_t)__popcll(bal & lt_mask);
          if (pos < (uint32_t)GCR_LAZY_CAP) s[pos] = k;
          lo_k = k < lo_k ? k : lo_k;
          hi_k = k > hi_k ? k : hi_k;
        }
      }
    }
    __syncthreads();
    cnt = *cnt_w;
    if (cnt <= (uint32_t)GCR_LAZY_CAP) break;
    if (j > 1u) {
      j = max(1u, min(j - 1u, (uint32_t)(((uint64_t)j * GCR_LAZY_TARGET) / cnt)));
      U = samp[j];
    } else {
      if (lo_k <= hi_k) {
        atomicMin(lo_w, (unsigned long long)lo_k);
        atomicMax(hi_w, (unsigned long long)hi_k);
      }
      __syncthreads();
      const uint64_t lo = *lo_w, hi = *hi_w;
      U = lo + ((hi - lo) >> 1) + 1ull;
      j = 0u;
    }
    __syncthreads();
  }
  if (cnt == 0u || cnt > (uint32_t)GCR_LAZY_CAP) {
    n_sorted = n;
    L = ~0ull;
    __syncthreads();
    return;
  }
  int N2 = 256;
  while (N2 < (int)cnt) N2 <<= 1;
  for (int i = (int)cnt + tid; i < N2; i += 256) s[i] = ~0ull;
  __syncthreads();
  gcr_bitonic_sort_lds(s, N2, tid);
  for (uint32_t i = tid; i < cnt; i += 256u) out[n_sorted + i] = (uint32_t)s[i];
  n_sorted += cnt;
  L = U;
  __syncthreads();
}
```

Measured before the change: 6074 frames/s.

## Scatter bare tile ids and rank-sort short tile lists inside the blend kernel

When no tile list exceeds 1024 entries and band sort is off, the tile scatter writes 32-bit Gaussian ids instead of 64-bit depth|id keys, and the separate tile-sort kernel is skipped. The forward blend kernel rebuilds the keys by reading depth from the per-Gaussian record and ranks them in LDS with a shared rank-merge helper. For single-chunk tiles it stages records straight into their ranked slots. This is meant to cut scatter traffic and one kernel launch plus its global round-trip. In exchange the blend pays for extra gathers and ranking work, and its LDS is unified into one block for the SORT variant.

```diff
diff --git a/gaussiancity_amd/csrc/gcr_api.hip b/gaussiancity_amd/csrc/gcr_api.hip
--- a/gaussiancity_amd/csrc/gcr_api.hip
+++ b/gaussiancity_amd/csrc/gcr_api.hip
@@ -22,6 +22,8 @@
 std::atomic<int> g_force_global_cursor{0};
 std::atomic<int> g_lazy_sort{1};
 std::atomic<int> g_sort_in_blend{0};
+std::atomic<int> g_blend_ranks{GCR_BLEND_RANKS_DEFAULT};
+std::atomic<int> g_last_tile_ids{0};
 std::atomic<int> g_split_preprocess{0};
 std::atomic<int> g_deterministic{0};
 std::atomic<int> g_bwd_wave_units{0};
@@ -45,7 +47,7 @@
 #endif
 
 struct Opts {
-  int lazy_sort, sort_in_blend, bwd_piece, deterministic, split_preprocess, force_radix, force_global_cursor, bwd_wave_units;
+  int lazy_sort, sort_in_blend, blend_ranks, bwd_piece, deterministic, split_preprocess, force_radix, force_global_cursor, bwd_wave_units;
   int band_sort_min;
   int stream_policy;
 };
@@ -67,6 +69,7 @@
     {"split_preprocess", &g_split_preprocess, opt_raw, &Opts::split_preprocess, &gcr_options::split_preprocess},
     {"sort_in_blend", &g_sort_in_blend, opt_raw, &Opts::sort_in_blend, &gcr_options::sort_in_blend},
     {"lazy_sort", &g_lazy_sort, opt_bool, &Opts::lazy_sort, &gcr_options::lazy_sort},
+    {"blend_ranks", &g_blend_ranks, opt_bool, &Opts::blend_ranks, nullptr},
     {"deterministic_backward", &g_deterministic, opt_bool, &Opts::deterministic, &gcr_options::deterministic_backward},
     {"bwd_wave_units", &g_bwd_wave_units, opt_bool, &Opts::bwd_wave_units, &gcr_options::bwd_wave_units},
     {"bwd_piece", &g_bwd_piece, opt_piece, &Opts::bwd_piece, &gcr_options::bwd_piece},
@@ -116,8 +119,6 @@
   __asm__ __volatile__("yield");
 #endif
 }
-
-constexpr int64_t GCR_SORT_IN_BLEND_MAX = 384;
 
 thread_local StageSlot g_slots[ST_COUNT];
 StageSlot* stage_slot(int stage) { return g_timing.load() ? &g_slots[stage] : nullptr; }
@@ -368,6 +369,7 @@
 }
 
 int gcr_get_option(const char* name) {
+  if (name && !strcmp(name, "last_tile_ids")) return g_last_tile_ids.load();
   const OptionRow* o = find_option(name);
   return o ? o->global->load() : INT32_MIN;
 }
@@ -376,6 +378,10 @@
 
 static inline bool band_sort_slot_free(const Opts& op) {
   return !op.split_preprocess && !op.force_radix && !op.force_global_cursor;
+}
+static inline bool band_sort_wanted(const Opts& op, const FrameSetup& f, unsigned long long cap_instances) {
+  return f.NG > 0 && f.banded && band_sort_slot_free(op) && op.band_sort_min >= 0 &&
+         (op.band_sort_min == 0 || (cap_instances != ~0ull && cap_instances >= (unsigned long long)op.band_sort_min));
 }
 
 static int enqueue_preprocess(const Opts& op, const gcr_camera* cam, const gcr_gaussians* g, const FrameSetup& f,
@@ -413,8 +419,7 @@
   if (int rc = debug_sync(cam, s, "preprocess")) return rc;
   StageTimer t(s, stage_slot(ST_SCAN));
   if (f.NG > 0) {
-    const bool band = f.banded && band_sort_slot_free(op) && op.band_sort_min >= 0 &&
-                      (op.band_sort_min == 0 || (cap_instances != ~0ull && cap_instances >= (unsigned long long)op.band_sort_min));
+    const bool band = band_sort_wanted(op, f, cap_instances);
     HIP_TRY(gcr_launch_tile_count(T, f.gx, f.NG, f.G, f.nblocks, f.chunk, f.vis_rec, f.vis_count, f.table, f.cursor,
                                   f.cursor + (size_t)T, f.cursor + 2 * (size_t)T, f.frame, f.block_tiles, host_R, seq,
                                   band ? f.banded : nullptr, g->P / 4, s),
@@ -461,12 +466,16 @@
   const int64_t R_layout = f.R_layout;
   uint64_t* pairs = f.keys[0];
   const unsigned long long* frame_guard = speculative ? f.frame : nullptr;
+  const bool tile_ids = R_layout > 0 && f.NG > 0 && (op.sort_in_blend != 0 || (op.blend_ranks != 0 && cam->backward != 1)) &&
+                        list_length_hint <= GCR_BLEND_RANKS_MAX && !op.force_radix && !op.force_global_cursor &&
+                        !band_sort_wanted(op, f, cap_instances);
+  g_last_tile_ids.store(tile_ids ? 1 : 0);
   {
     StageTimer t(s, stage_slot(ST_EMIT));
     if (f.NG > 0) {
       HIP_TRY(gcr_launch_tile_scatter(f.T, f.gx, f.NG, f.G, f.nblocks, f.chunk, f.vis_rec, f.vis_count, f.table, f.cursor,
                                       f.cursor + (size_t)f.T, f.cursor + 2 * (size_t)f.T, f.ranges, pairs, f.frame,
-                                      cap_instances, cap_list, host_longest, f.banded, g->P / 4, s),
+                                      cap_instances, cap_list, host_longest, f.banded, g->P / 4, tile_ids, s),
               "tile scatter");
     } else if (R_layout > 0) {
       HIP_TRY(gcr_launch_scatter_instances(f.nblocks, f.chunk, f.vis_list, f.vis_count, f.rec, f.gx, f.cursor, pairs,
@@ -475,9 +484,8 @@
     }
   }
   if (int rc = debug_sync(cam, s, "scatter instances")) return rc;
-  const bool sort_in_blend = R_layout > 0 && list_length_hint <= GCR_SORT_IN_BLEND_MAX && op.sort_in_blend != 0;
-  uint4* lazy = (R_layout > 0 && !sort_in_blend && op.lazy_sort != 0) ? f.lazy : nullptr;
-  if (R_layout > 0 && !sort_in_blend) {
+  uint4* lazy = (R_layout > 0 && op.lazy_sort != 0) ? f.lazy : nullptr;
+  if (R_layout > 0 && !tile_ids) {
     StageTimer t(s, stage_slot(ST_SORT));
     HIP_TRY(gcr_launch_tile_sort(f.ranges, f.T, pairs, f.keys[1], f.list, list_length_hint + list_length_hint / 2 + 64,
                                  frame_guard, lazy, s),
@@ -489,6 +497,7 @@
   b.out_color = out_color;
   b.frame = frame_guard;
   b.pairs = pairs;
+  b.key_scratch = f.keys[1];
   b.list_out = f.list;
   b.lazy = lazy;
   set_piece_args(op, b, cam->backward == 1, f);
@@ -511,7 +520,7 @@
 #endif
   {
     StageTimer t(s, stage_slot(ST_BLEND_FWD));
-    HIP_TRY(gcr_launch_blend_fwd(b, sort_in_blend, s), "blend forward");
+    HIP_TRY(gcr_launch_blend_fwd(b, tile_ids, s), "blend forward");
   }
 #ifdef GCR_EXPERIMENTS
   if (chain) {
@@ -994,6 +1003,7 @@
   GcrBlendArgs b = blend_args(f, cam, f.vals[half]);
   b.out_color = out_color;
   set_piece_args(op, b, cam->backward == 1, f);
+  g_last_tile_ids.store(0);
   {
     StageTimer t(s, stage_slot(ST_BLEND_FWD));
     HIP_TRY(gcr_launch_blend_fwd(b, false, s), "blend forward");
diff --git a/gaussiancity_amd/csrc/gcr_binning.hip b/gaussiancity_amd/csrc/gcr_binning.hip
--- a/gaussiancity_amd/csrc/gcr_binning.hip
+++ b/gaussiancity_amd/csrc/gcr_binning.hip
@@ -36,7 +36,7 @@
     }
 }
 
-constexpr int RANK_MERGE_MAX = 1024;
+constexpr int RANK_MERGE_MAX = GCR_RANK_MERGE_MAX;
 constexpr int TT_MAX_TBLOCKS = 640;
 
 template <int THREADS>
@@ -103,7 +103,8 @@
                                                            unsigned long long* __restrict__ host_word,
                                                            unsigned int seq,
                                                            const unsigned long long* __restrict__ block_tiles,
-                                                           const uint4* __restrict__ banded, int banded_capacity) {
+                                                           const uint4* __restrict__ banded, int banded_capacity,
+                                                           int tile_ids) {
   extern __shared__ __attribute__((aligned(16))) unsigned char gcr_smem[];
   uint32_t* cnt = reinterpret_cast<uint32_t*>(gcr_smem);
   __shared__ uint32_t pre[GCR_K1_MAX_BLOCKS + 1];
@@ -197,12 +198,16 @@
     const uint32_t rx = sv.z, ry = sv.w;
     const uint32_t minx = rx & 0xffffu, maxx = rx >> 16, miny = ry & 0xffffu, maxy = ry >> 16;
     const uint64_t key = ((uint64_t)sv.y << 32) | sv.x;
+    uint32_t* __restrict__ ids = reinterpret_cast<uint32_t*>(pairs);
     for (uint32_t y = miny; y < maxy; y++)
       for (uint32_t x = minx; x < maxx; x++) {
         const uint32_t t = y * (uint32_t)gx + x;
         if (SCATTER) {
           const uint32_t pos = atomicAdd(&cnt[t], 1u);
-          pairs[pos] = key;
+          if (tile_ids)
+            ids[pos] = sv.x;
+          else
+            pairs[pos] = key;
         } else {
           atomicAdd(&cnt[t], 1u);
         }
@@ -430,59 +435,17 @@
     return;
   }
   if (n <= RANK_MERGE_MAX) {
-    const int nchunks = (n + 63) >> 6, npad = nchunks << 6;
-    uint64_t* sb = s + npad;
-    for (int i = tid; i < npad; i += 256) s[i] = i < n ? pairs[r0 + i] : ~0ull;
-    __syncthreads();
-    const ulonglong2* s2 = reinterpret_cast<const ulonglong2*>(s);
     uint64_t mine[RANK_MERGE_MAX / 256];
-    uint32_t rank[RANK_MERGE_MAX / 256];
+    uint32_t pos[RANK_MERGE_MAX / 256];
 #pragma unroll
     for (int e = 0; e < RANK_MERGE_MAX / 256; e++) {
       const int i = tid + e * 256;
-      if (i < npad) {
-        const int c = i >> 6;
-        const uint64_t key = s[i];
-        uint32_t r = 0;
-#pragma unroll 8
-        for (int j = 0; j < 32; j++) {
-          const ulonglong2 kk = s2[c * 32 + j];
-          r += (kk.x < key ? 1u : 0u) + (kk.y < key ? 1u : 0u);
-        }
-        mine[e] = key;
-        rank[e] = r;
-        if (i < n) sb[c * 64 + r] = key;
-      }
-    }
-    __syncthreads();
-    const int last_real = n - (nchunks - 1) * 64;
-#pragma unroll
-    for (int e = 0; e < RANK_MERGE_MAX / 256; e++) {
-      const int i = tid + e * 256;
-      if (i < n) {
-        const int c = i >> 6;
-        const uint64_t key = mine[e];
-        uint32_t pos = rank[e];
-        for (int c2 = 0; c2 < nchunks; c2++) {
-          if (c2 == c) continue;
-          const uint64_t* chunk = sb + c2 * 64;
-          const int len = c2 == nchunks - 1 ? last_real : 64;
-          int lo = 0, hi = len;
-#pragma unroll
-          for (int step = 0; step < 7; step++) {
-            if (lo < hi) {
-              const int mid = (lo + hi) >> 1;
-              if (chunk[mid] < key)
-                lo = mid + 1;
-              else
-                hi = mid;
-            }
-          }
-          pos += (uint32_t)lo;
-        }
-        list[r0 + pos] = (uint32_t)key;
-      }
-    }
+      mine[e] = i < n ? pairs[r0 + i] : ~0ull;
+    }
+    gcr_rank_merge(s, n, mine, pos, tid);
+#pragma unroll
+    for (int e = 0; e < RANK_MERGE_MAX / 256; e++)
+      if (tid + e * 256 < n) list[r0 + pos[e]] = (uint32_t)mine[e];
     return;
   }
   int N2 = 2;
@@ -708,11 +671,11 @@
   if (tile_table_wide(T))
     k_tile_table<false, 1024><<<NG, 1024, (size_t)T * sizeof(uint32_t), s>>>(
         T, gx, tile_table_G(G), nblocks_k1, chunk, vis_rec, vis_count, table, nullptr, nullptr, nullptr, nullptr, nullptr,
-        frame, 0ull, 0ull, host_R, seq, block_tiles, banded, banded_capacity);
+        frame, 0ull, 0ull, host_R, seq, block_tiles, banded, banded_capacity, 0);
   else
     k_tile_table<false, 512><<<NG, 512, (size_t)T * sizeof(uint32_t), s>>>(
         T, gx, tile_table_G(G), nblocks_k1, chunk, vis_rec, vis_count, table, nullptr, nullptr, nullptr, nullptr, nullptr,
-        frame, 0ull, 0ull, host_R, seq, block_tiles, banded, banded_capacity);
+        frame, 0ull, 0ull, host_R, seq, block_tiles, banded, banded_capacity, 0);
   k_table_colscan<<<(T + 63) / 64, 1024, 0, s>>>(table, NG, T, tile_total, tile_local, blk_total, frame);
   return hipGetLastError();
 }
@@ -723,17 +686,17 @@
                                    const uint32_t* blk_total, uint32_t* ranges, uint64_t* pairs,
                                    unsigned long long* frame, unsigned long long cap_instances,
                                    unsigned long long cap_list, unsigned long long* host_longest,
-                                   const uint4* banded, int banded_capacity, hipStream_t s) {
+                                   const uint4* banded, int banded_capacity, bool tile_ids, hipStream_t s) {
   hipError_t e = tile_table_attr();
   if (e != hipSuccess) return e;
   if (tile_table_wide(T))
     k_tile_table<true, 1024><<<NG, 1024, (size_t)T * sizeof(uint32_t), s>>>(
         T, gx, tile_table_G(G), nblocks_k1, chunk, vis_rec, vis_count, table, tile_total, tile_local, blk_total, ranges, pairs,
-        frame, cap_instances, cap_list, host_longest, 0u, nullptr, banded, banded_capacity);
+        frame, cap_instances, cap_list, host_longest, 0u, nullptr, banded, banded_capacity, tile_ids ? 1 : 0);
   else
     k_tile_table<true, 512><<<NG, 512, (size_t)T * sizeof(uint32_t), s>>>(
         T, gx, tile_table_G(G), nblocks_k1, chunk, vis_rec, vis_count, table, tile_total, tile_local, blk_total, ranges, pairs,
-        frame, cap_instances, cap_list, host_longest, 0u, nullptr, banded, banded_capacity);
+        frame, cap_instances, cap_list, host_longest, 0u, nullptr, banded, banded_capacity, tile_ids ? 1 : 0);
   return hipGetLastError();
 }
 
diff --git a/gaussiancity_amd/csrc/gcr_blend.hip b/gaussiancity_amd/csrc/gcr_blend.hip
--- a/gaussiancity_amd/csrc/gcr_blend.hip
+++ b/gaussiancity_amd/csrc/gcr_blend.hip
@@ -11,6 +11,13 @@
 constexpr int K6_LIST_STRIDE = 232;
 static_assert(GCR_PIECE_MAX <= K6_SENT_SLOT, "a K6 chunk must leave slot 255 to the sentinel");
 constexpr uint32_t NO_ENTRY = 0xFFFFFFFFu;
+constexpr int K6_LDS_MASK = (K6_SENT_SLOT + 1) * (int)ENTRY_BYTES;
+constexpr int K6_LDS_LIST = K6_LDS_MASK + CHUNK * 4;
+constexpr int K6_LDS_BYTES = K6_LDS_LIST + 4 * 8 * K6_LIST_STRIDE;
+static_assert(K6_LDS_MASK % 16 == 0 && K6_LDS_LIST % 16 == 0, "K6's LDS arrays are read and filled as quads");
+static_assert(GCR_BLEND_RANKS_MAX == GCR_RANK_MERGE_MAX, "the host sends frames with lists up to here to the SORT kernels");
+static_assert(2 * GCR_RANK_MERGE_MAX * 8 <= K6_LDS_BYTES, "k6_rank_ids ranks up to GCR_RANK_MERGE_MAX keys in K6's LDS");
+static_assert(2 * CHUNK * 8 <= 4 * 8 * K6_LIST_STRIDE, "a one-chunk tile is ranked in the list area while its records are staged");
 
 struct __attribute__((aligned(16))) StagedEntry {
   float4 a, b, c;
@@ -143,6 +150,41 @@
   return ns;
 }
 
+GCR_DEV void k6_rank_ids(uint64_t* s, const uint32_t* __restrict__ ids, const float4* __restrict__ rec,
+                                         uint64_t* __restrict__ scratch, uint32_t n, uint32_t* __restrict__ out) {
+  const int tid = threadIdx.x;
+  if (n <= (uint32_t)GCR_RANK_MERGE_MAX) {
+    uint64_t key[GCR_RANK_MERGE_MAX / 256];
+    uint32_t pos[GCR_RANK_MERGE_MAX / 256];
+#pragma unroll
+    for (int e = 0; e < GCR_RANK_MERGE_MAX / 256; e++) {
+      const uint32_t i = (uint32_t)tid + (uint32_t)e * 256u;
+      key[e] = ~0ull;
+      if (i < n) {
+        const uint32_t id = ids[i];
+        key[e] = ((uint64_t)__float_as_uint(rec[(size_t)id * GCR_REC_QUADS + 2].y) << 32) | id;
+      }
+    }
+    gcr_rank_merge(s, (int)n, key, pos, tid);
+#pragma unroll
+    for (int e = 0; e < GCR_RANK_MERGE_MAX / 256; e++)
+      if ((uint32_t)tid + (uint32_t)e * 256u < n) out[pos[e]] = (uint32_t)key[e];
+  } else {
+    for (uint32_t i = tid; i < n; i += 256u) {
+      const uint32_t id = ids[i];
+      scratch[i] = ((uint64_t)__float_as_uint(rec[(size_t)id * GCR_REC_QUADS + 2].y) << 32) | id;
+    }
+    __syncthreads();
+    for (uint32_t i = tid; i < n; i += 256u) {
+      const uint64_t mine = scratch[i];
+      uint32_t rank = 0;
+      for (uint32_t j = 0; j < n; j++) rank += scratch[j] < mine ? 1u : 0u;
+      out[rank] = (uint32_t)mine;
+    }
+  }
+  __syncthreads();
+}
+
 __device__ __noinline__ void k6_frame_gate(unsigned long long* words, unsigned int seq, unsigned int max_polls) {
   gcr_store_to_host(words + 3, (unsigned long long)seq);
   for (unsigned int i = 0; i < max_polls; i++) {
@@ -165,9 +207,25 @@
 
 template <bool SORT, bool STATE, bool PIXSTATE>
 __global__ __launch_bounds__(256) __attribute__((amdgpu_waves_per_eu(8, 8))) void k_blend_fwd(const GcrBlendArgs a) {
-  __shared__ StagedEntry sE[K6_SENT_SLOT + 1];
-  __shared__ uint32_t sMask[CHUNK];
-  __shared__ __attribute__((aligned(16))) uint8_t sList[4][8][K6_LIST_STRIDE];
+  StagedEntry* sE;
+  uint32_t* sMask;
+  uint8_t(*sList)[8][K6_LIST_STRIDE];
+  unsigned char* k6_lds;
+  if constexpr (SORT) {
+    __shared__ __attribute__((aligned(16))) unsigned char lds_block[K6_LDS_BYTES];
+    k6_lds = lds_block;
+    sE = reinterpret_cast<StagedEntry*>(lds_block);
+    sMask = reinterpret_cast<uint32_t*>(lds_block + K6_LDS_MASK);
+    sList = reinterpret_cast<uint8_t(*)[8][K6_LIST_STRIDE]>(lds_block + K6_LDS_LIST);
+  } else {
+    __shared__ StagedEntry lds_E[K6_SENT_SLOT + 1];
+    __shared__ uint32_t lds_mask[CHUNK];
+    __shared__ __attribute__((aligned(16))) uint8_t lds_list[4][8][K6_LIST_STRIDE];
+    k6_lds = reinterpret_cast<unsigned char*>(lds_E);
+    sE = lds_E;
+    sMask = lds_mask;
+    sList = lds_list;
+  }
 
   if (a.frame != nullptr && a.frame[2] == 0ull) {
     if (a.gate_words != nullptr && blockIdx.x == 0 && threadIdx.x == 0) k6_frame_gate(a.gate_words, a.gate_seq, a.gate_polls);
@@ -178,6 +236,8 @@
   const int tid = threadIdx.x;
   const float tile_x0 = (float)(tx * GCR_TILE_X), tile_y0 = (float)(ty * GCR_TILE_Y);
   const uint32_t r0 = a.ranges[2 * tile], r1 = a.ranges[2 * tile + 1];
+  if (SORT && PIXSTATE && a.lazy != nullptr && tid == 0)
+    a.lazy[tile] = make_uint4(gcr_tile_in_window(a, tx, ty) ? r1 - r0 : 0u, 0u, ~0u, ~0u);
   if (!gcr_tile_in_window(a, tx, ty)) {
     if (STATE && a.work != nullptr) {
       const uint32_t P0 = (uint32_t)a.piece, sb = r0 / P0 + (uint32_t)tile, ns = r1 / P0 + 1u - r0 / P0;
@@ -204,7 +264,7 @@
     o[10] = __builtin_readcyclecounter();
   }
 #endif
-  if (tid == 0) {
+  if (!SORT && tid == 0) {
     sE[K6_SENT_SLOT].a = make_float4(0.0f, 0.0f, 0.0f, 0.0f);
     sE[K6_SENT_SLOT].b = make_float4(0.0f, 0.0f, 0.0f, 0.0f);
     sE[K6_SENT_SLOT].c = make_float4(0.0f, __builtin_inff(), 0.0f, 0.0f);
@@ -227,38 +287,14 @@
   uint32_t lz_sorted = (uint32_t)max(total, 0);
   if (!SORT && a.lazy != nullptr) lz_sorted = a.lazy[tile].x;
 
-  uint32_t sorted_id = 0;
-  if (SORT && total > 0) {
-    const uint64_t* __restrict__ seg = a.pairs + r0;
-    uint32_t* __restrict__ out = a.list_out + r0;
-    if (total <= K6_SENT_SLOT) {
-      uint64_t* sKey = reinterpret_cast<uint64_t*>(sE);
-      const uint64_t mine = tid < total ? seg[tid] : ~0ull;
-      sKey[tid] = mine;
-      __syncthreads();
-      const ulonglong2* k2 = reinterpret_cast<const ulonglong2*>(sKey);
-      uint32_t rank = 0;
-      for (int j = 0; j < (total + 1) / 2; j++) {
-        const ulonglong2 kk = k2[j];
-        rank += (kk.x < mine ? 1u : 0u) + (kk.y < mine ? 1u : 0u);
-      }
-      __syncthreads();
-      if (tid < total) {
-        sMask[rank] = (uint32_t)mine;
-        out[rank] = (uint32_t)mine;
-      }
-      __syncthreads();
-      sorted_id = tid < total ? sMask[tid] : 0u;
-      __syncthreads();
-    } else {
-      for (int i = tid; i < total; i += 256) {
-        const uint64_t mine = seg[i];
-        uint32_t rank = 0;
-        for (int j = 0; j < total; j++) rank += seg[j] < mine ? 1u : 0u;
-        out[rank] = (uint32_t)mine;
-      }
-      __syncthreads();
-    }
+  const bool rank_staged = SORT && cs == total;
+  if (SORT && total > 0 && !rank_staged)
+    k6_rank_ids(reinterpret_cast<uint64_t*>(k6_lds), reinterpret_cast<const uint32_t*>(a.pairs) + r0, a.rec, a.key_scratch + r0,
+                (uint32_t)total, a.list_out + r0);
+  if (SORT && tid == 0) {
+    sE[K6_SENT_SLOT].a = make_float4(0.0f, 0.0f, 0.0f, 0.0f);
+    sE[K6_SENT_SLOT].b = make_float4(0.0f, 0.0f, 0.0f, 0.0f);
+    sE[K6_SENT_SLOT].c = make_float4(0.0f, __builtin_inff(), 0.0f, 0.0f);
   }
 
 #define GCR_BLEND_STEP(QA, QB, QC, OFF)                                                      \
@@ -325,9 +361,28 @@
     entered++;
     const int n = min(cs, total - base);
     uint32_t my_mask = 0;
+    uint32_t slot = (uint32_t)tid;
+    uint32_t id = 0;
+    if (SORT && rank_staged) {
+      int t = threadIdx.x;
+      asm volatile("" : "+v"(t));
+      uint64_t key[1] = {~0ull};
+      if (t < n) {
+        id = reinterpret_cast<const uint32_t*>(a.pairs)[r0 + t];
+        key[0] = ((uint64_t)__float_as_uint(a.rec[(size_t)id * GCR_REC_QUADS + 2].y) << 32) | id;
+      }
+      uint32_t pos[1];
+      gcr_rank_merge<1, 2>(reinterpret_cast<uint64_t*>(&sList[0][0][0]), n, key, pos, t);
+      if (t < n) {
+        slot = pos[0];
+        if (PIXSTATE) a.list_out[r0 + slot] = id;
+      }
+    }
     if (tid < n) {
-      const uint32_t id = !SORT ? a.list[r0 + base + tid]
-                                : ((total <= K6_SENT_SLOT && cs == total) ? sorted_id : a.list_out[r0 + base + tid]);
+      if (!SORT)
+        id = a.list[r0 + base + tid];
+      else if (!rank_staged)
+        id = a.list_out[r0 + base + tid];
       const float4* __restrict__ rec = a.rec + (size_t)id * GCR_REC_QUADS;
 #ifdef GCR_EXPERIMENTS
       if (a.clock_buf != nullptr && tid == 0 && base == 0) {
@@ -346,19 +401,19 @@
       my_mask = gcr_block_mask_2x4(q0.x, q0.y, q0.z, q0.w, q1.x, pmin, tile_x0, tile_y0);
       const float4 sa = make_float4(q0.x, q0.y, -0.5f * q0.z, -q0.w), sb = make_float4(-0.5f * q1.x, q1.y, q1.z, q1.w);
       const float4 sc = make_float4(q2.x, pmin, 0.0f, 0.0f);
-      sE[tid].a = sa;
-      sE[tid].b = sb;
-      sE[tid].c = sc;
+      sE[slot].a = sa;
+      sE[slot].b = sb;
+      sE[slot].c = sc;
       if (STATE && a.staged_out != nullptr) {
-        float4* __restrict__ so = a.staged_out + (size_t)(r0 + (uint32_t)base + (uint32_t)tid) * 3;
+        float4* __restrict__ so = a.staged_out + (size_t)(r0 + (uint32_t)base + slot) * 3;
         so[0] = sa;
         so[1] = sb;
         so[2] = sc;
       }
     }
-    sMask[tid] = my_mask;
+    sMask[slot] = my_mask;
     if (STATE && tid < n && a.mask_out != nullptr)
-      a.mask_out[r0 + base + tid] = (uint16_t)gcr_block_mask_4x4_of_2x4(my_mask);
+      a.mask_out[r0 + base + slot] = (uint16_t)gcr_block_mask_4x4_of_2x4(my_mask);
     __syncthreads();
 #ifdef GCR_EXPERIMENTS
     if (a.clock_buf != nullptr && tid == 0 && base == 0) a.clock_buf[(size_t)tile * 16 + 4] = __builtin_readcyclecounter();
@@ -1026,8 +1081,8 @@
 #endif
   if (a.work != nullptr)
     k_blend_fwd<SORT, true, true><<<T, 256, pad, s>>>(a);
-  else if (!SORT && a.image_only)
-    k_blend_fwd<false, false, false><<<T, 256, pad, s>>>(a);
+  else if (a.image_only)
+    k_blend_fwd<SORT, false, false><<<T, 256, pad, s>>>(a);
   else
     k_blend_fwd<SORT, false, true><<<T, 256, pad, s>>>(a);
 }
diff --git a/gaussiancity_amd/csrc/gcr_internal.h b/gaussiancity_amd/csrc/gcr_internal.h
--- a/gaussiancity_amd/csrc/gcr_internal.h
+++ b/gaussiancity_amd/csrc/gcr_internal.h
@@ -128,6 +128,8 @@
 #define GCR_FRAME_CARVE 6
 #define GCR_FRAME_STAGED_OFF 8
 #define GCR_BAND_SORT_MIN_DEFAULT 6000000
+#define GCR_BLEND_RANKS_DEFAULT 1
+#define GCR_BLEND_RANKS_MAX 1024
 #define GCR_FRAME_BANDED 9
 static inline __host__ __device__ bool gcr_frame_has_state(const unsigned long long* frame, unsigned long long binning_bytes) {
   return frame[GCR_FRAME_PIECE] != 0ull && frame[GCR_FRAME_CARVE] <= binning_bytes;
@@ -138,6 +140,7 @@
   const uint32_t* list;
   const uint64_t* pairs;
   uint32_t* list_out;
+  uint64_t* key_scratch;
   const float4* rec;
   int W, H, gx, gy;
   const float* bg;
@@ -212,7 +215,7 @@
                                    const uint32_t* blk_total, uint32_t* ranges, uint64_t* pairs,
                                    unsigned long long* frame, unsigned long long cap_instances,
                                    unsigned long long cap_list, unsigned long long* host_longest,
-                                   const uint4* banded, int banded_capacity, hipStream_t s);
+                                   const uint4* banded, int banded_capacity, bool tile_ids, hipStream_t s);
 hipError_t gcr_launch_scatter_instances(int nblocks, int chunk, const uint32_t* vis_list,
                                         const uint32_t* vis_count, const float4* rec, int gx,
                                         uint32_t* tile_cursor, uint64_t* pairs, const uint32_t* ranges, int T,
diff --git a/gaussiancity_amd/csrc/gcr_sort.h b/gaussiancity_amd/csrc/gcr_sort.h
--- a/gaussiancity_amd/csrc/gcr_sort.h
+++ b/gaussiancity_amd/csrc/gcr_sort.h
@@ -29,6 +29,64 @@
     }
   }
   __syncthreads();
+}
+
+constexpr int GCR_RANK_MERGE_MAX = 1024;
+template <int E, int UNROLL = 8>
+GCR_DEV void gcr_rank_merge(uint64_t* s, int n, const uint64_t (&key)[E], uint32_t (&pos)[E], int tid) {
+  const int nchunks = (n + 63) >> 6, npad = nchunks << 6;
+  uint64_t* sb = s + npad;
+#pragma unroll
+  for (int e = 0; e < E; e++) {
+    const int i = tid + e * 256;
+    if (i < npad) s[i] = key[e];
+  }
+  __syncthreads();
+  const ulonglong2* s2 = reinterpret_cast<const ulonglong2*>(s);
+#pragma unroll
+  for (int e = 0; e < E; e++) {
+    const int i = tid + e * 256;
+    pos[e] = 0;
+    if (i < npad) {
+      const int c = i >> 6;
+      uint32_t r = 0;
+#pragma unroll UNROLL
+      for (int j = 0; j < 32; j++) {
+        const ulonglong2 kk = s2[c * 32 + j];
+        r += (kk.x < key[e] ? 1u : 0u) + (kk.y < key[e] ? 1u : 0u);
+      }
+      pos[e] = r;
+      if (i < n) sb[c * 64 + r] = key[e];
+    }
+  }
+  __syncthreads();
+  const int last_real = n - (nchunks - 1) * 64;
+#pragma unroll
+  for (int e = 0; e < E; e++) {
+    const int i = tid + e * 256;
+    if (i < n) {
+      const int c = i >> 6;
+      uint32_t p = pos[e];
+      for (int c2 = 0; c2 < nchunks; c2++) {
+        if (c2 == c) continue;
+        const uint64_t* chunk = sb + c2 * 64;
+        const int len = c2 == nchunks - 1 ? last_real : 64;
+        int lo = 0, hi = len;
+#pragma unroll
+        for (int step = 0; step < 7; step++) {
+          if (lo < hi) {
+            const int mid = (lo + hi) >> 1;
+            if (chunk[mid] < key[e])
+              lo = mid + 1;
+            else
+              hi = mid;
+          }
+        }
+        p += (uint32_t)lo;
+      }
+      pos[e] = p;
+    }
+  }
 }
 
 GCR_DEV void gcr_tile_sort_long(uint64_t* s, uint32_t run0, uint64_t* __restrict__ A, uint64_t* __restrict__ B,
```

After: 6364 frames/s (median of 6 runs). 4.8% higher.
